# in5omnia/Image_Segmentation

Measured on AMD Instinct MI355X. Metric: images/sec (fwd+bwd) U-Net 3-class 256x256; IoU parity vs CPU ref, higher is better.
Workload: dtype bf16; 1 GPU; unet(3,3) train step (fwd + ce + bwd + grad all-reduce + AdamW), B=32/GPU 3x256x256, BASELINE config 2; global_batch=32, parallelism=dp1, rccl_ranks=0, rehearsal=False

## Files before the change

### image_segmentation_amd/_lib.py

```python
import ctypes as C
import os

_HERE = os.path.dirname(os.path.abspath(__file__))
LIB_PATH = os.path.join(_HERE, "csrc", "libsegk.so")

F32, BF16 = 0, 1
ABI_VERSION = 312
MAX_CLASSES = 8
MSE_PART_FLOATS = 1024

_vp, _fp, _i, _l, _f, _d = C.c_void_p, C.c_void_p, C.c_int, C.c_long, C.c_float, C.c_double

SIGNATURES = {
    "segk_version": (_i, []),
    "segk_entry_count": (_i, []),
    "segk_clock_probe": (_i, [_vp, _i, _i, _i, _vp]),
    "segk_debug_poison_tickets": (_i, [C.c_uint64, _vp]),
    "segk_build_id": (C.c_char_p, []),
    "segk_last_error": (C.c_char_p, []),
    "segk_nchw_to_nhwc": (_i, [_fp, _vp, _i, _i, _i, _i, _i, _i, _vp]),
    "segk_nhwc_to_nchw": (_i, [_vp, _fp, _i, _i, _i, _i, _i, _i, _vp]),
    "segk_pack_conv_weight": (_i, [_fp, _vp, _i, _i, _i, _i, _i, _i, _i, _i, _i, _vp]),
    "segk_pack_conv3x3_both": (_i, [_fp, _vp, _vp, _i, _i, _i, _i, _i, _i, _i, _vp]),
    "segk_pack_multi": (_i, [_vp, _i, _i, _i, _vp]),
    "segk_pack_convt_chunk": (_i, []),
    "segk_pack_convt_weight": (_i, [_fp, _vp, _i, _i, _i, _i, _i, _i, _vp]),
    "segk_conv_tiles": (_i, [_i, _i, _i, _i, _i, _i]),
    "segk_bn_stats_floats": (_i, [_i, _i]),
    "segk_conv3x3": (_i, [_vp, _vp, _vp, _fp, _fp, _fp, _vp, _vp, _fp, _i, _i, _i, _i, _i, _i, _i, _i, _vp]),
    "segk_conv_writes_act_q": (_i, [_i, _i, _i]),
    "segk_conv3x3_act": (_i, [_vp, _vp, _fp, _fp, _vp, _vp, _fp, _i, _i, _i, _i, _i, _i, _vp]),
    "segk_stem3x3_rows": (_i, [_i, _i, _i, _i, _i, _i]),
    "segk_stem3x3": (_i, [_fp, _fp, _vp, _vp, _fp, _i, _i, _i, _i, _i, _i, _vp]),
    "segk_stem3x3_wgrad_slabs": (_i, [_i, _i, _i, _i, _i, _i]),
    "segk_stem3x3_wgrad": (_i, [_fp, _vp, _fp, _i, _i, _i, _i, _i, _i, _vp]),
    "segk_conv1x1": (_i, [_vp, _vp, _fp, _vp, _i, _i, _i, _i, _i, _i, _vp]),
    "segk_convt2x2_fwd": (_i, [_vp, _vp, _fp, _vp, _i, _i, _i, _i, _i, _i, _vp]),
    "segk_convt2x2_dgrad": (_i, [_vp, _vp, _vp, _i, _i, _i, _i, _i, _i, _vp]),
    "segk_wgrad_tiles": (_i, [_i, _i, _i, _i, _i]),
    "segk_wgrad_split": (_i, [_i, _i, _i, _i, _i, _i]),
    "segk_wgrad": (_i, [_vp, _vp, _vp, _fp, _fp, _fp, _vp, _i, _i, _i, _i, _i, _i, _i, _i, _i, _vp]),
    "segk_wgrad_reduce": (_i, [_fp, _i, _fp, _i, _i, _i, _i, _i, _i, _i, _vp]),
    "segk_wgrad_reduce_multi": (_i, [_vp, _i, _vp]),
    "segk_bn_finalize": (_i, [_fp, _i, _i, _i, _d, _fp, _fp, _fp, _fp, _fp, _f, _f, _i, _fp, _fp, _fp, _fp, _vp]),
    "segk_bn_relu_apply": (_i, [_vp, _vp, _fp, _fp, _l, _i, _i, _vp]),
    "segk_bn_relu_apply_pool": (_i, [_vp, _vp, _vp, _fp, _fp, _i, _i, _i, _i, _i, _vp]),
    "segk_bn_bwd_blocks": (_i, [_l, _i, _i]),
    "segk_bn_relu_bwd": (_i, [_vp, _vp, _vp, _fp, _fp, _fp, _fp, _l, _i, _i, _fp, _fp, _fp, _fp, _i, _vp]),
    "segk_channel_sum": (_i, [_vp, _l, _i, _i, _fp, _fp, _i, _vp]),
    "segk_maxpool2x2_fwd": (_i, [_vp, _vp, _i, _i, _i, _i, _i, _vp]),
    "segk_maxpool2x2_bwd": (_i, [_vp, _vp, _vp, _i, _i, _i, _i, _i, _i, _vp]),
    "segk_maxpool_bwd_stat_blocks": (_i, [_i, _i, _i, _i, _i]),
    "segk_maxpool2x2_bwd_bnstat": (_i, [_vp, _vp, _vp, _i, _i, _i, _i, _i, _fp, _fp, _fp, _fp, _fp, _vp, _i, _vp]),
    "segk_bn_relu_bwd_from_part": (_i, [_vp, _vp, _vp, _fp, _fp, _fp, _fp, _l, _i, _i, _fp, _i, _fp, _fp, _fp, _i, _vp]),
    "segk_bilinear_fwd": (_i, [_vp, _vp, _i, _i, _i, _i, _i, _i, _i, _vp]),
    "segk_bilinear_bwd": (_i, [_vp, _vp, _fp, _i, _i, _i, _i, _i, _i, _i, _vp]),
    "segk_linear": (_i, [_vp, _vp, _fp, _vp, _l, _i, _i, _i, _i, _vp]),
    "segk_vit_patchify": (_i, [_fp, _vp, _i, _i, _i, _i, _i, _i, _i, _vp]),
    "segk_vit_embed_ln": (_i, [_vp, _fp, _fp, _fp, _fp, _f, _fp, _i, _i, _i, _i, _i, _vp]),
    "segk_add_layernorm": (_i, [_fp, _vp, _fp, _fp, _f, _vp, _l, _i, _i, _i, _vp]),
    "segk_linear_splitk": (_i, [_vp, _vp, _fp, _vp, _l, _i, _i, _i, _i, _vp]),
    "segk_add_layernorm_parts": (_i, [_fp, _vp, _i, _l, _fp, _fp, _f, _vp, _l, _i, _i, _i, _vp]),
    "segk_attention": (_i, [_vp, _vp, _i, _i, _i, _i, _i, _i, _f, _i, _vp]),
    "segk_vit_tokens_to_grid": (_i, [_fp, _vp, _i, _i, _i, _i, _i, _vp]),
    "segk_resize_pad": (_i, [_vp, _vp, _i, _i, _i, _i, _i, _i, _i, _i, _i, _i, _vp]),
    "segk_crop_resize": (_i, [_fp, _fp, _i, _i, _i, _i, _i, _i, _i, _i, _i, _vp]),
    "segk_resize_pad_u8": (_i, [_vp, _fp, _i, _i, _i, _i, _i, _i, _i, _i, _i, _vp]),
    "segk_predict_mask": (_i, [_vp, _vp, _vp, _vp, _vp, _vp, _vp, _i, _i, _i, _i, _i, _i, _i, _i, _i, _vp]),
    "segk_head_fwd": (_i, [_vp, _fp, _fp, _fp, _i, _i, _i, _i, _i, _i, _i, _vp]),
    "segk_head_fwd_bn": (_i, [_vp, _fp, _fp, _fp, _fp, _fp, _i, _i, _i, _i, _i, _i, _i, _vp]),
    "segk_head_bwd_bn": (_i, [_fp, _vp, _fp, _vp, _fp, _fp, _fp, _i, _i, _i, _i, _i, _i, _fp, _fp, _fp, _fp, _fp, _i, _vp]),
    "segk_head_part_floats": (_i, [_l, _i]),
    "segk_head_bwd": (_i, [_fp, _vp, _fp, _vp, _fp, _fp, _fp, _i, _i, _i, _i, _i, _i, _i, _vp]),
    "segk_head_bwd_blocks": (_i, [_l]),
    "segk_head_bwd_bnstat": (_i, [_fp, _vp, _fp, _vp, _fp, _fp, _fp, _i, _i, _i, _i, _i, _i, _fp, _fp, _fp, _fp, _fp, _i, _vp]),
    "segk_loss_part_floats": (_i, [_l]),
    "segk_loss_state_floats": (_i, []),
    "segk_loss_fwd": (_i, [_fp, _vp, _fp, _i, _i, _l, _i, _f, _f, _f, _fp, _fp, _fp, _vp]),
    "segk_loss_bwd": (_i, [_fp, _vp, _fp, _fp, _fp, _i, _i, _l, _i, _f, _f, _fp, _vp]),
    "segk_prompt_mix_fwd": (_i, [_fp, _fp, _fp, _i, _l, _vp]),
    "segk_prompt_mix_bwd": (_i, [_fp, _fp, _fp, _fp, _i, _l, _vp]),
    "segk_prob_loss_fwd": (_i, [_fp, _vp, _fp, _i, _i, _l, _i, _f, _f, _f, _i, _f, _fp, _fp, _fp, _vp]),
    "segk_prob_loss_bwd": (_i, [_fp, _vp, _fp, _fp, _fp, _i, _i, _l, _i, _f, _f, _i, _f, _fp, _vp]),
    "segk_confusion": (_i, [_fp, _vp, _i, _i, _l, _vp, _vp]),
    "segk_recon_head_fwd": (_i, [_vp, _fp, _fp, _fp, _i, _i, _i, _i, _i, _i, _i, _vp]),
    "segk_recon_sigmoid_bwd": (_i, [_fp, _fp, _vp, _i, _i, _i, _i, _i, _i, _vp]),
    "segk_mse_fwd": (_i, [_fp, _fp, _fp, _i, _fp, _l, _i, _vp]),
    "segk_mse_bwd": (_i, [_fp, _fp, _fp, _fp, _fp, _l, _i, _vp]),
}



class ReduceJob(C.Structure):
    _fields_ = [("src", C.c_void_p), ("dst", C.c_void_p), ("kind", C.c_int), ("S", C.c_int), ("N", C.c_int), ("CA", C.c_int),
                ("CB", C.c_int), ("Np", C.c_int), ("CAp", C.c_int), ("CBp", C.c_int), ("taps", C.c_int), ("pad_", C.c_int)]


_lib = None


def load():
    global _lib, LIB_PATH
    if _lib is None:
        if os.environ.get("SEGK_LIB"):
            LIB_PATH = os.path.abspath(os.environ["SEGK_LIB"])
        if not os.path.exists(LIB_PATH):
            raise RuntimeError(
                f"{LIB_PATH} not found: the HIP extension is required (no CPU/eager fallback exists). "
                "Build it with `python -m image_segmentation_amd.build`.")
        lib = C.CDLL(LIB_PATH)
        for name, (res, args) in SIGNATURES.items():
            try:
                fn = getattr(lib, name)
            except AttributeError:
                raise RuntimeError(f"{LIB_PATH} does not export {name}: it was built from another include/segk.h than "
                                   "this binding (rebuild with `python -m image_segmentation_amd.build`)") from None
            fn.restype = res
            fn.argtypes = args
        ver, nent = lib.segk_version(), lib.segk_entry_count()
        if ver != ABI_VERSION or nent != len(SIGNATURES):
            raise RuntimeError(f"{LIB_PATH}: ABI version {ver} with {nent} entries, this binding expects version "
                               f"{ABI_VERSION} with {len(SIGNATURES)} entries -- refusing to drive a library built from "
                               "another include/segk.h")
        _lib = lib
    return _lib


def call(name, *args):
    lib = load()
    rc = getattr(lib, name)(*args)
    if rc != 0:
        raise RuntimeError(f"{name} failed ({rc}): {lib.segk_last_error().decode()}")


def build_id():
    return load().segk_build_id().decode()


def query(name, *args):
    return getattr(load(), name)(*args)
```

### image_segmentation_amd/csrc/api.hip

```cpp
#include "common.hpp"
#include "segk_internal.h"
#include "../../include/segk.h"

thread_local char g_segk_err[512] = "";

int segk_bn_finalize_impl(const float*, int, int, int, double, const float*, const float*, const float*, float*, float*,
                          float, float, int, float*, float*, float*, float*, hipStream_t);
int segk_bn_relu_apply_impl(const void*, void*, const float*, const float*, long, int, int, hipStream_t);
int segk_bn_relu_apply_pool_impl(const void*, void*, void*, const float*, const float*, int, int, int, int, int, hipStream_t);
int segk_bn_bwd_impl(const void*, const void*, void*, const float*, const float*, const float*, const float*, long, int,
                     int, float*, float*, float*, float*, int, hipStream_t);
int segk_channel_sum_impl(const void*, long, int, int, float*, float*, int, hipStream_t);
int segk_maxpool_fwd_impl(const void*, void*, int, int, int, int, int, hipStream_t);
int segk_maxpool_bwd_impl(const void*, const void*, void*, int, int, int, int, int, int, hipStream_t);
int segk_maxpool_bwd_bnstat_impl(const void*, const void*, void*, int, int, int, int, int, const float*, const float*,
                                 const float*, const float*, float*, const void*, int, hipStream_t);
int segk_bn_bwd_from_part_impl(const void*, const void*, void*, const float*, const float*, const float*, const float*, long,
                               int, int, const float*, int, float*, float*, float*, int, hipStream_t);
int segk_nchw_to_nhwc_impl(const float*, void*, int, int, int, int, int, int, hipStream_t);
int segk_nhwc_to_nchw_impl(const void*, float*, int, int, int, int, int, int, hipStream_t);
int segk_pack_conv_weight_impl(const float*, void*, int, int, int, int, int, int, int, int, int, hipStream_t);
int segk_pack_convt_weight_impl(const float*, void*, int, int, int, int, int, int, hipStream_t);
int segk_pack_conv3x3_both_impl(const float*, void*, void*, int, int, int, int, int, int, int, hipStream_t);
int segk_pack_multi_impl(const void*, int, int, int, hipStream_t);
int segk_pack_convt_chunk_impl();
int segk_wgrad_reduce_impl(const float*, int, float*, int, int, int, int, int, int, int, hipStream_t);
int segk_wgrad_reduce_multi_impl(const segk_reduce_job*, int, hipStream_t);
int segk_head_fwd_impl(const void*, const float*, const float*, float*, int, int, int, int, int, int, const float*, const float*,
                       int, hipStream_t);
int segk_head_bwd_impl(const float*, const void*, const float*, void*, float*, float*, float*, int, int, int, int, int,
                       int, const float*, const float*, const float*, const float*, float*, int, int, hipStream_t);
int segk_head_blocks_q(long);
int segk_loss_fwd_impl(const float*, const long long*, const float*, int, int, long, int, float, float, float, float*,
                       float*, float*, int, int, float, hipStream_t);
int segk_loss_bwd_impl(const float*, const long long*, const float*, const float*, const float*, int, int, long, int,
                       float, float, float*, int, int, float, hipStream_t);
int segk_prompt_mix_impl(const float*, const float*, const float*, float*, int, long, hipStream_t);
int segk_confusion_impl(const float*, const long long*, int, int, long, unsigned long long*, hipStream_t);

int segk_recon_head_fwd_impl(const void*, const float*, const float*, float*, int, int, int, int, int, int, int, hipStream_t);
int segk_recon_sigmoid_bwd_impl(const float*, const float*, void*, int, int, int, int, int, int, hipStream_t);
int segk_mse_fwd_impl(const float*, const float*, float*, int, float*, long, int, hipStream_t);
int segk_mse_bwd_impl(const float*, const float*, const float*, float*, float*, long, int, hipStream_t);

int segk_clock_probe_impl(unsigned long long*, int, int, int, hipStream_t);
int segk_debug_poison_tickets_impl(unsigned long long, hipStream_t);

int segk_device_index() {
  int dev = 0;
  if (hipGetDevice(&dev) != hipSuccess || dev < 0) dev = 0;
  return dev < SEGK_MAX_DEVICES ? dev : SEGK_MAX_DEVICES - 1;
}
int segk_num_cus() {
  static int n[SEGK_MAX_DEVICES] = {};
  const int dev = segk_device_index();
  if (n[dev] == 0) {
    hipDeviceProp_t p;
    int v = 0;
    if (hipGetDeviceProperties(&p, dev) == hipSuccess) v = p.multiProcessorCount;
    n[dev] = v >= 8 ? v : 256;
  }
  return n[dev];
}

static void fill_tiles(ConvArgs&) {}

extern "C" {

#ifndef SEGK_BUILD_ID
#define SEGK_BUILD_ID "unknown"
#endif
int segk_version(void) { return SEGK_ABI_VERSION; }
int segk_entry_count(void) { return SEGK_ENTRY_COUNT; }
int segk_debug_poison_tickets(uint64_t pattern, segk_stream_t s) {
  return segk_debug_poison_tickets_impl((unsigned long long)pattern, (hipStream_t)s);
}
int segk_clock_probe(uint64_t* out, int blocks, int iters, int shape, segk_stream_t s) {
  return segk_clock_probe_impl((unsigned long long*)out, blocks, iters, shape, (hipStream_t)s);
}
const char* segk_build_id(void) { return SEGK_BUILD_ID; }
const char* segk_last_error(void) { return g_segk_err; }

int segk_nchw_to_nhwc(const float* src, void* dst, int B, int C, int H, int W, int Cp, int dtype, segk_stream_t s) {
  SEGK_REQUIRE(dtype == SEGK_DT_F32 || dtype == SEGK_DT_BF16, "nchw_to_nhwc: bad dtype %d", dtype);
  return segk_nchw_to_nhwc_impl(src, dst, B, C, H, W, Cp, dtype, (hipStream_t)s);
}
int segk_nhwc_to_nchw(const void* src, float* dst, int B, int C, int H, int W, int Cp, int dtype, segk_stream_t s) {
  SEGK_REQUIRE(dtype == SEGK_DT_F32 || dtype == SEGK_DT_BF16, "nhwc_to_nchw: bad dtype %d", dtype);
  return segk_nhwc_to_nchw_impl(src, dst, B, C, H, W, Cp, dtype, (hipStream_t)s);
}
int segk_pack_conv_weight(const float* w, void* dst, int Cout, int CA, int CB, int Coutp, int CAp, int CBp, int taps,
                          int mode, int dtype, segk_stream_t s) {
  SEGK_REQUIRE(dtype == SEGK_DT_F32 || dtype == SEGK_DT_BF16, "pack_conv_weight: bad dtype %d", dtype);
  return segk_pack_conv_weight_impl(w, dst, Cout, CA, CB, Coutp, CAp, CBp, taps, mode, dtype, (hipStream_t)s);
}
int segk_pack_conv3x3_both(const float* w, void* dst_fwd, void* dst_dgrad, int Cout, int CA, int CB, int Coutp, int CAp,
                            int CBp, int dtype, segk_stream_t s) {
  SEGK_REQUIRE(dtype == SEGK_DT_F32 || dtype == SEGK_DT_BF16, "pack_conv3x3_both: bad dtype %d", dtype);
  return segk_pack_conv3x3_both_impl(w, dst_fwd, dst_dgrad, Cout, CA, CB, Coutp, CAp, CBp, dtype, (hipStream_t)s);
}
int segk_pack_convt_chunk(void) { return segk_pack_convt_chunk_impl(); }
int segk_pack_multi(const void* table, int n, int total_blocks, int dtype, segk_stream_t s) {
  return segk_pack_multi_impl(table, n, total_blocks, dtype, (hipStream_t)s);
}
int segk_pack_convt_weight(const float* w, void* dst, int Cin, int Cout, int Cinp, int Coutp, int mode, int dtype,
                           segk_stream_t s) {
  SEGK_REQUIRE(dtype == SEGK_DT_F32 || dtype == SEGK_DT_BF16, "pack_convt_weight: bad dtype %d", dtype);
  return segk_pack_convt_weight_impl(w, dst, Cin, Cout, Cinp, Coutp, mode, dtype, (hipStream_t)s);
}

int segk_conv_tiles(int B, int H, int W, int Cin, int Cout, int dtype) {
  if (B <= 0 || H <= 0 || W <= 0 || Cin <= 0 || Cout <= 0 || (long long)B * H * W > 0x1fffffffLL) return 0;
  if (segk_conv_use_rs(Cin, Cout, dtype, W)) return segk_conv_rs_rows(B, H, W, Cout);
  const int pk = segk_conv_use_pipe(Cin, Cout, dtype);
  const int bm = segk_conv_use_ws(Cin, Cout, dtype) ? 256 : pk ? 32768 / pk : segk_conv_bm(0, Cout);
  const int twl = segk_conv_twl(bm, W);
  return B * cdiv(W, 1 << twl) * cdiv(H, bm >> twl);
}

int segk_conv3x3(const void* srcA, const void* srcB, const void* wpacked, const float* bias, const float* scale,
                 const float* shift, void* out, void* out2, float* stats, int B, int H, int W, int CA, int CB, int CO1,
                 int CO2, int dtype, segk_stream_t s) {
  SEGK_REQUIRE(dtype == SEGK_DT_F32 || dtype == SEGK_DT_BF16, "conv3x3: bad dtype %d", dtype);
  ConvArgs a{};
  a.srcA = srcA; a.srcB = srcB; a.w = wpacked; a.bias = bias; a.scale = scale; a.shift = shift;
  a.out = out; a.out2 = out2; a.stats = stats;
  a.B = B; a.H = H; a.W = W; a.CA = CA; a.CB = CB; a.Ntot = CO1 + CO2; a.CO1 = CO1; a.CO2 = CO2;
  fill_tiles(a);
  return segk_conv_igemm_launch(a, 0, dtype, (hipStream_t)s);
}

int segk_conv_writes_act_q(int Cin, int Cout, int dtype) { return segk_conv_writes_act(Cin, Cout, dtype); }

int segk_stem3x3_rows(int B, int H, int W, int Cin, int Cout, int dtype) { return segk_stem_rows(B, H, W, Cin, Cout, dtype); }
int segk_stem3x3_wgrad_slabs(int B, int H, int W, int Cin, int Cout, int dtype) {
  return segk_stem_wgrad_slabs(B, H, W, Cin, Cout, dtype);
}
int segk_stem3x3_wgrad(const float* x_nchw, const void* dz, float* slabs, int B, int H, int W, int Cin, int Cout, int dtype,
                       segk_stream_t s) {
  SEGK_REQUIRE(dtype == SEGK_DT_BF16, "stem3x3_wgrad: bf16 only (dtype %d)", dtype);
  return segk_stem_wgrad_launch(x_nchw, dz, slabs, B, H, W, Cin, Cout, (hipStream_t)s);
}
int segk_stem3x3(const float* x_nchw, const float* w_oihw, void* z, void* x_nhwc, float* stats, int B, int H, int W, int Cin,
                 int Cout, int dtype, segk_stream_t s) {
  SEGK_REQUIRE(dtype == SEGK_DT_BF16, "stem3x3: bf16 only (dtype %d)", dtype);
  return segk_stem_launch(x_nchw, w_oihw, z, x_nhwc, stats, B, H, W, Cin, Cout, (hipStream_t)s);
}

int segk_conv3x3_act(const void* srcA, const void* wpacked, const float* scale, const float* shift, void* out,
                     void* act_out, float* stats, int B, int H, int W, int CA, int CO, int dtype, segk_stream_t s) {
  SEGK_REQUIRE(dtype == SEGK_DT_F32 || dtype == SEGK_DT_BF16, "conv3x3_act: bad dtype %d", dtype);
  ConvArgs a{};
  a.srcA = srcA; a.w = wpacked; a.scale = scale; a.shift = shift; a.out = out; a.act_out = act_out; a.stats = stats;
  a.B = B; a.H = H; a.W = W; a.CA = CA; a.Ntot = CO; a.CO1 = CO;
  fill_tiles(a);
  return segk_conv_igemm_launch(a, 0, dtype, (hipStream_t)s);
}

int segk_conv1x1(const void* srcA, const void* wpacked, const float* bias, void* out, int B, int H, int W, int CA,
                 int CO, int dtype, segk_stream_t s) {
  SEGK_REQUIRE(dtype == SEGK_DT_F32 || dtype == SEGK_DT_BF16, "conv1x1: bad dtype %d", dtype);
  ConvArgs a{};
  a.srcA = srcA; a.w = wpacked; a.bias = bias; a.out = out;
  a.B = B; a.H = H; a.W = W; a.CA = CA; a.Ntot = CO; a.CO1 = CO;
  fill_tiles(a);
  return segk_conv_igemm_launch(a, 1, dtype, (hipStream_t)s);
}

int segk_linear(const void* rows, const void* wpacked, const float* bias, void* out, long M, int K, int N, int act,
                int dtype, segk_stream_t s) {
  SEGK_REQUIRE(dtype == SEGK_DT_F32 || dtype == SEGK_DT_BF16, "linear: bad dtype %d", dtype);
  SEGK_REQUIRE(M > 0 && M % 16 == 0 && M / 16 < (1 << 24), "linear: M=%ld must be a positive multiple of 16", M);
  SEGK_REQUIRE(act == 0 || act == 1, "linear: bad activation %d", act);
  ConvArgs a{};
  a.srcA = rows; a.w = wpacked; a.bias = bias; a.out = out;
  a.B = 1; a.H = (int)(M / 16); a.W = 16; a.CA = K; a.Ntot = N; a.CO1 = N; a.act = act;
  fill_tiles(a);
  return segk_conv_igemm_launch(a, 1, dtype, (hipStream_t)s);
}

int segk_linear_splitk(const void* rows, const void* wpacked, const float* bias, void* out_parts, long M, int K, int N,
                       int ksplit, int dtype, segk_stream_t s) {
  SEGK_REQUIRE(dtype == SEGK_DT_F32 || dtype == SEGK_DT_BF16, "linear_splitk: bad dtype %d", dtype);
  SEGK_REQUIRE(dtype == SEGK_DT_BF16, "linear_splitk: bf16 only");
  SEGK_REQUIRE(M > 0 && M % 16 == 0 && K > 0 && K % 64 == 0 && N > 0 && ksplit >= 1, "linear_splitk: bad shape");
  SEGK_REQUIRE(segk_gemm_dma_ok(M, K / 32, K / 32, N, N, K, 0) && (K / 64) % ksplit == 0 && K / 64 / ksplit >= 1,
               "linear_splitk: K=%d does not split %d ways into 64-element stages (or the shape is not served)", K, ksplit);
  GemmArgs g{};
  g.A = rows; g.w = (const char*)wpacked; g.bias = bias; g.out = out_parts;
  g.M = M; g.N = N; g.nchunks = K / 32; g.nchA = K / 32; g.lda = K; g.H = 1; g.W = 1; g.Cout = N;
  g.ksplit = ksplit; g.split_stride = M * (long)N;
  return segk_gemm_dma_launch(g, 0, (hipStream_t)s);
}

int segk_convt2x2_fwd(const void* in, const void* wpacked, const float* bias4, void* out, int B, int H, int W, int Cin,
                      int Cout, int dtype, segk_stream_t s) {
  SEGK_REQUIRE(dtype == SEGK_DT_F32 || dtype == SEGK_DT_BF16, "convt2x2_fwd: bad dtype %d", dtype);
  SEGK_REQUIRE(in && wpacked && out && B > 0 && H > 0 && W > 0 && Cin > 0 && Cout > 0, "convt2x2_fwd: bad arguments");
  if (segk_convt_stream_ok(B, H, W, Cin, Cout, dtype))
    return segk_convt_stream_launch(in, wpacked, bias4, out, B, H, W, Cin, Cout, (hipStream_t)s);
  ConvArgs a{};
  a.srcA = in; a.w = wpacked; a.bias = bias4; a.out = out;
  a.B = B; a.H = H; a.W = W; a.CA = Cin; a.Ntot = 4 * Cout; a.CO1 = Cout; a.shuffle = 1;
  fill_tiles(a);
  return segk_conv_igemm_launch(a, 1, dtype, (hipStream_t)s);
}

int segk_convt2x2_dgrad(const void* dout, const void* wpacked, void* din, int B, int H, int W, int Cin, int Cout,
                        int dtype, segk_stream_t s) {
  SEGK_REQUIRE(dtype == SEGK_DT_F32 || dtype == SEGK_DT_BF16, "convt2x2_dgrad: bad dtype %d", dtype);
  SEGK_REQUIRE(dout && wpacked && din && B > 0 && H > 0 && W > 0 && Cin > 0 && Cout > 0, "convt2x2_dgrad: bad arguments");
  if (segk_convt_stream_dgrad_ok(B, H, W, Cin, Cout, dtype))
    return segk_convt_stream_dgrad_launch(dout, wpacked, din, B, H, W, Cin, Cout, (hipStream_t)s);
  ConvArgs a{};
  a.srcA = dout; a.w = wpacked; a.out = din;
  a.B = B; a.H = H; a.W = W; a.CA = Cout; a.Ntot = Cin; a.CO1 = Cin; a.unshuf = 1;
  fill_tiles(a);
  return segk_conv_igemm_launch(a, 1, dtype, (hipStream_t)s);
}

int segk_wgrad(const void* dz, const void* srcA, const void* srcB, const float* scale, const float* shift, float* slabs,
               const void* zeros, int S, int B, int H, int W, int CD, int CA, int CB, int geo, int dtype,
               segk_stream_t s) {
  SEGK_REQUIRE(dtype == SEGK_DT_F32 || dtype == SEGK_DT_BF16, "wgrad: bad dtype %d", dtype);
  WgradArgs a{};
  a.dz = dz; a.srcA = srcA; a.srcB = srcB; a.scale = scale; a.shift = shift; a.slabs = slabs; a.zeros = zeros;
  a.B = B; a.H = H; a.W = W; a.CD = CD; a.CA = CA; a.CB = CB; a.S = S;
  return segk_wgrad_launch(a, geo, dtype, (hipStream_t)s);
}
int segk_wgrad_reduce(const float* slabs, int S, float* grad, int N, int CA, int CB, int Np, int CAp, int CBp, int taps,
                      segk_stream_t s) {
  return segk_wgrad_reduce_impl(slabs, S, grad, N, CA, CB, Np, CAp, CBp, taps, (hipStream_t)s);
}
int segk_wgrad_reduce_multi(const segk_reduce_job* jobs, int n, segk_stream_t s) {
  return segk_wgrad_reduce_multi_impl(jobs, n, (hipStream_t)s);
}

int segk_bn_finalize(const float* stats, int tiles, int Cp, int C, double count, const float* conv_bias,
                     const float* gamma, const float* beta, float* running_mean, float* running_var, float momentum,
                     float eps, int training, float* scale, float* shift, float* mean, float* rstd, segk_stream_t s) {
  return segk_bn_finalize_impl(stats, tiles, Cp, C, count, conv_bias, gamma, beta, running_mean, running_var, momentum,
                               eps, training, scale, shift, mean, rstd, (hipStream_t)s);
}
int segk_bn_relu_apply(const void* z, void* y, const float* scale, const float* shift, long P, int Cp, int dtype,
                       segk_stream_t s) {
  SEGK_REQUIRE(dtype == SEGK_DT_F32 || dtype == SEGK_DT_BF16, "bn_relu_apply: bad dtype %d", dtype);
  return segk_bn_relu_apply_impl(z, y, scale, shift, P, Cp, dtype, (hipStream_t)s);
}
int segk_bn_relu_apply_pool(const void* z, void* y, void* pooled, const float* scale, const float* shift, int B, int H, int W,
                            int Cp, int dtype, segk_stream_t s) {
  SEGK_REQUIRE(dtype == SEGK_DT_F32 || dtype == SEGK_DT_BF16, "bn_relu_apply_pool: bad dtype %d", dtype);
  return segk_bn_relu_apply_pool_impl(z, y, pooled, scale, shift, B, H, W, Cp, dtype, (hipStream_t)s);
}
int segk_bn_relu_bwd(const void* dy, const void* z, void* dz, const float* scale, const float* shift, const float* mean,
                     const float* rstd, long P, int Cp, int C, float* part, float* dgamma, float* dbeta, float* coef,
                     int dtype, segk_stream_t s) {
  SEGK_REQUIRE(dtype == SEGK_DT_F32 || dtype == SEGK_DT_BF16, "bn_relu_bwd: bad dtype %d", dtype);
  return segk_bn_bwd_impl(dy, z, dz, scale, shift, mean, rstd, P, Cp, C, part, dgamma, dbeta, coef, dtype,
                          (hipStream_t)s);
}
int segk_channel_sum(const void* x, long P, int Cp, int C, float* part, float* out, int dtype, segk_stream_t s) {
  SEGK_REQUIRE(dtype == SEGK_DT_F32 || dtype == SEGK_DT_BF16, "channel_sum: bad dtype %d", dtype);
  return segk_channel_sum_impl(x, P, Cp, C, part, out, dtype, (hipStream_t)s);
}
int segk_maxpool2x2_fwd(const void* x, void* y, int B, int H, int W, int Cp, int dtype, segk_stream_t s) {
  SEGK_REQUIRE(dtype == SEGK_DT_F32 || dtype == SEGK_DT_BF16, "maxpool2x2_fwd: bad dtype %d", dtype);
  return segk_maxpool_fwd_impl(x, y, B, H, W, Cp, dtype, (hipStream_t)s);
}
int segk_maxpool2x2_bwd(const void* x, const void* dy, void* dx, int B, int H, int W, int Cp, int accumulate, int dtype,
                        segk_stream_t s) {
  SEGK_REQUIRE(dtype == SEGK_DT_F32 || dtype == SEGK_DT_BF16, "maxpool2x2_bwd: bad dtype %d", dtype);
  return segk_maxpool_bwd_impl(x, dy, dx, B, H, W, Cp, accumulate, dtype, (hipStream_t)s);
}
int segk_maxpool2x2_bwd_bnstat(const void* x, const void* dy, void* dx, int B, int H, int W, int Cp, int accumulate,
                               const float* scale, const float* shift, const float* mean, const float* rstd, float* part,
                               const void* z, int dtype, segk_stream_t s) {
  SEGK_REQUIRE(dtype == SEGK_DT_F32 || dtype == SEGK_DT_BF16, "maxpool2x2_bwd_bnstat: bad dtype %d", dtype);
  return segk_maxpool_bwd_bnstat_impl(x, dy, dx, B, H, W, Cp, accumulate, scale, shift, mean, rstd, part, z, dtype,
                                      (hipStream_t)s);
}
int segk_bn_relu_bwd_from_part(const void* dy, const void* z, void* dz, const float* scale, const float* shift,
                               const float* mean, const float* rstd, long P, int Cp, int C, const float* part, int nb,
                               float* dgamma, float* dbeta, float* coef, int dtype, segk_stream_t s) {
  SEGK_REQUIRE(dtype == SEGK_DT_F32 || dtype == SEGK_DT_BF16, "bn_relu_bwd_from_part: bad dtype %d", dtype);
  return segk_bn_bwd_from_part_impl(dy, z, dz, scale, shift, mean, rstd, P, Cp, C, part, nb, dgamma, dbeta, coef, dtype,
                                    (hipStream_t)s);
}
int segk_head_fwd(const void* y, const float* w, const float* bias, float* logits, int B, int H, int W, int Cp, int C,
                  int ncls, int dtype, segk_stream_t s) {
  SEGK_REQUIRE(dtype == SEGK_DT_F32 || dtype == SEGK_DT_BF16, "head_fwd: bad dtype %d", dtype);
  return segk_head_fwd_impl(y, w, bias, logits, B, H, W, Cp, C, ncls, nullptr, nullptr, dtype, (hipStream_t)s);
}
int segk_head_fwd_bn(const void* z, const float* scale, const float* shift, const float* w, const float* bias, float* logits,
                     int B, int H, int W, int Cp, int C, int ncls, int dtype, segk_stream_t s) {
  SEGK_REQUIRE(scale && shift, "head_fwd_bn: null scale/shift");
  return segk_head_fwd_impl(z, w, bias, logits, B, H, W, Cp, C, ncls, scale, shift, dtype, (hipStream_t)s);
}
int segk_head_bwd(const float* dlogits, const void* y, const float* w, void* dy, float* part, float* dw, float* db,
                  int B, int H, int W, int Cp, int C, int ncls, int dtype, segk_stream_t s) {
  SEGK_REQUIRE(dtype == SEGK_DT_F32 || dtype == SEGK_DT_BF16, "head_bwd: bad dtype %d", dtype);
  return segk_head_bwd_impl(dlogits, y, w, dy, part, dw, db, B, H, W, Cp, C, ncls, nullptr, nullptr, nullptr, nullptr, nullptr,
                            0, dtype, (hipStream_t)s);
}
int segk_head_bwd_blocks(long P) { return segk_head_blocks_q(P); }
int segk_head_bwd_bnstat(const float* dlogits, const void* y, const float* w, void* dy, float* part, float* dw, float* db,
                         int B, int H, int W, int Cp, int C, int ncls, const float* scale, const float* shift,
                         const float* mean, const float* rstd, float* bnpart, int dtype, segk_stream_t s) {
  SEGK_REQUIRE(dtype == SEGK_DT_F32 || dtype == SEGK_DT_BF16, "head_bwd_bnstat: bad dtype %d", dtype);
  SEGK_REQUIRE(bnpart, "head_bwd_bnstat: null partials");
  return segk_head_bwd_impl(dlogits, y, w, dy, part, dw, db, B, H, W, Cp, C, ncls, scale, shift, mean, rstd, bnpart, 0, dtype,
                            (hipStream_t)s);
}
int segk_head_bwd_bn(const float* dlogits, const void* z, const float* w, void* dy, float* part, float* dw, float* db,
                     int B, int H, int W, int Cp, int C, int ncls, const float* scale, const float* shift,
                     const float* mean, const float* rstd, float* bnpart, int dtype, segk_stream_t s) {
  SEGK_REQUIRE(scale && shift && mean && rstd, "head_bwd_bn: null BatchNorm vectors");
  return segk_head_bwd_impl(dlogits, z, w, dy, part, dw, db, B, H, W, Cp, C, ncls, scale, shift, mean, rstd, bnpart, 1, dtype,
                            (hipStream_t)s);
}
int segk_loss_fwd(const float* logits, const int64_t* labels, const float* cw, int N, int C, long HW, int ignore_index,
                  float smooth, float dice_weight, float ce_weight, float* part, float* state, float* loss_out,
                  segk_stream_t s) {
  return segk_loss_fwd_impl(logits, (const long long*)labels, cw, N, C, HW, ignore_index, smooth, dice_weight, ce_weight,
                            part, state, loss_out, 0, 0, 0.f, (hipStream_t)s);
}
int segk_prob_loss_fwd(const float* probs, const int64_t* labels, const float* cw, int N, int C, long HW, int ignore_index,
                       float smooth, float dice_weight, float nll_weight, int nll_log, float eps, float* part, float* state,
                       float* loss_out, segk_stream_t s) {
  return segk_loss_fwd_impl(probs, (const long long*)labels, cw, N, C, HW, ignore_index, smooth, dice_weight, nll_weight,
                            part, state, loss_out, 1, nll_log, eps, (hipStream_t)s);
}
int segk_prob_loss_bwd(const float* probs, const int64_t* labels, const float* cw, const float* state, const float* gout,
                       int N, int C, long HW, int ignore_index, float dice_weight, float nll_weight, int nll_log, float eps,
                       float* dprobs, segk_stream_t s) {
  return segk_loss_bwd_impl(probs, (const long long*)labels, cw, state, gout, N, C, HW, ignore_index, dice_weight,
                            nll_weight, dprobs, 1, nll_log, eps, (hipStream_t)s);
}
int segk_prompt_mix_fwd(const float* clip_logits, const float* mask_logit, float* final_probs, int N, long HW,
                        segk_stream_t s) {
  return segk_prompt_mix_impl(clip_logits, mask_logit, nullptr, final_probs, N, HW, (hipStream_t)s);
}
int segk_prompt_mix_bwd(const float* clip_logits, const float* mask_logit, const float* dfinal, float* dmask_logit, int N,
                        long HW, segk_stream_t s) {
  SEGK_REQUIRE(dfinal, "prompt_mix_bwd: null gradient");
  return segk_prompt_mix_impl(clip_logits, mask_logit, dfinal, dmask_logit, N, HW, (hipStream_t)s);
}
int segk_loss_bwd(const float* logits, const int64_t* labels, const float* cw, const float* state, const float* gout,
                  int N, int C, long HW, int ignore_index, float dice_weight, float ce_weight, float* dlogits,
                  segk_stream_t s) {
  return segk_loss_bwd_impl(logits, (const long long*)labels, cw, state, gout, N, C, HW, ignore_index, dice_weight,
                            ce_weight, dlogits, 0, 0, 0.f, (hipStream_t)s);
}
int segk_recon_head_fwd(const void* x, const float* w, const float* bias, float* rec, int B, int H, int W, int Cp, int Cin,
                        int Cout, int dtype, segk_stream_t s) {
  return segk_recon_head_fwd_impl(x, w, bias, rec, B, H, W, Cp, Cin, Cout, dtype, (hipStream_t)s);
}
int segk_recon_sigmoid_bwd(const float* drec, const float* rec, void* dz, int B, int H, int W, int C, int Cp, int dtype,
                           segk_stream_t s) {
  return segk_recon_sigmoid_bwd_impl(drec, rec, dz, B, H, W, C, Cp, dtype, (hipStream_t)s);
}
int segk_mse_fwd(const float* a, const float* b, float* part, int part_floats, float* out, long n, int mean, segk_stream_t s) {
  return segk_mse_fwd_impl(a, b, part, part_floats, out, n, mean, (hipStream_t)s);
}
int segk_mse_bwd(const float* a, const float* b, const float* grad_out, float* da, float* db, long n, int mean,
                 segk_stream_t s) {
  return segk_mse_bwd_impl(a, b, grad_out, da, db, n, mean, (hipStream_t)s);
}
int segk_confusion(const float* logits, const int64_t* labels, int N, int C, long HW, uint64_t* M, segk_stream_t s) {
  return segk_confusion_impl(logits, (const long long*)labels, N, C, HW, (unsigned long long*)M, (hipStream_t)s);
}

}
```

### image_segmentation_amd/csrc/bn_pool.hip

```cpp
#include <atomic>
#include "common.hpp"
#include "segk_internal.h"
#include "ticket.hpp"
#include "../../include/segk.h"

namespace {
__device__ unsigned g_tickets[TICKET_SLOTS * TICKET_GROUPS];

struct Lanes {
  int cx, ry, cv;
  bool active;
};
__device__ __forceinline__ Lanes lanes(int cvb, int cvec) {
  Lanes l;
  l.cx = threadIdx.x % cvb;
  l.ry = threadIdx.x / cvb;
  l.cv = blockIdx.y * cvb + l.cx;
  l.active = l.cv < cvec;
  return l;
}

constexpr int NCH = 32;
__device__ __forceinline__ void stats_chunk(const float* __restrict__ part, int MT, int C, double* __restrict__ out,
                                            double (&sh)[8][32][2]) {
  const int cx = threadIdx.x & 31, ry = threadIdx.x >> 5;
  const int c = blockIdx.x * 32 + cx;
  const int chunk = (MT + NCH - 1) / NCH;
  const int m0 = blockIdx.y * chunk, m1 = min(MT, m0 + chunk);
  double s1 = 0.0, s2 = 0.0;
  for (int m = m0 + ry; m < m1; m += 8) {
    const float2 v = ((const float2*)part)[(size_t)m * C + c];
    s1 += (double)v.x;
    s2 += (double)v.y;
  }
  sh[ry][cx][0] = s1;
  sh[ry][cx][1] = s2;
  __syncthreads();
  if (ry == 0) {
    s1 = 0.0; s2 = 0.0;
    for (int r = 0; r < 8; ++r) { s1 += sh[r][cx][0]; s2 += sh[r][cx][1]; }
    out[((size_t)blockIdx.y * C + c) * 2 + 0] = s1;
    out[((size_t)blockIdx.y * C + c) * 2 + 1] = s2;
  }
}

__device__ __forceinline__ void finalize_channels(const double* __restrict__ part, int MT, int C, int C_real,
                                                  double count, const float* conv_bias,
                                                  const float* gamma, const float* beta, float* rmean,
                                                  float* rvar, float momentum, float eps, int training,
                                                  float* scale, float* shift, float* mean_out,
                                                  float* rstd_out, double (&sh)[8][32][2]) {
  const int cx = threadIdx.x & 31, ry = threadIdx.x >> 5;
  const int c = blockIdx.x * 32 + cx;
  double s1 = 0.0, s2 = 0.0;
  if (training && c < C)
    for (int m = ry; m < MT; m += 8) {
      s1 += part[((size_t)m * C + c) * 2 + 0];
      s2 += part[((size_t)m * C + c) * 2 + 1];
    }
  sh[ry][cx][0] = s1;
  sh[ry][cx][1] = s2;
  __syncthreads();
  if (ry != 0 || c >= C) return;
  if (c >= C_real) {
    scale[c] = 0.f; shift[c] = 0.f;
    if (mean_out) { mean_out[c] = 0.f; rstd_out[c] = 0.f; }
    return;
  }
  const float g = gamma[c], be = beta[c];
  const float cb = conv_bias ? conv_bias[c] : 0.f;
  if (training) {
    s1 = 0.0; s2 = 0.0;
    for (int r = 0; r < 8; ++r) { s1 += sh[r][cx][0]; s2 += sh[r][cx][1]; }
    const double mean = s1 / count;
    double var = s2 / count - mean * mean;
    if (var < 0.0) var = 0.0;
    const float rstd = (float)(1.0 / sqrt(var + (double)eps));
    const float sc = g * rstd;
    scale[c] = sc;
    shift[c] = be - (float)mean * sc;
    mean_out[c] = (float)mean;
    rstd_out[c] = rstd;
    if (rmean) {
      const double unb = count > 1.0 ? var * count / (count - 1.0) : var;
      rmean[c] = (1.f - momentum) * rmean[c] + momentum * ((float)mean + cb);
      rvar[c] = (1.f - momentum) * rvar[c] + momentum * (float)unb;
    }
  } else {
    const float rstd = 1.f / sqrtf(rvar[c] + eps);
    const float sc = g * rstd;
    scale[c] = sc;
    shift[c] = be + (cb - rmean[c]) * sc;
    if (mean_out) { mean_out[c] = rmean[c] - cb; rstd_out[c] = rstd; }
  }
}

__global__ __launch_bounds__(256) void bn_finalize_kernel(const double* __restrict__ part, int MT, int C, int C_real,
                                                          double count, const float* conv_bias,
                                                          const float* gamma, const float* beta, float* rmean,
                                                          float* rvar, float momentum, float eps, int training,
                                                          float* scale, float* shift, float* mean_out,
                                                          float* rstd_out) {
  __shared__ double sh[8][32][2];
  finalize_channels(part, MT, C, C_real, count, conv_bias, gamma, beta, rmean, rvar, momentum, eps, training, scale, shift,
                    mean_out, rstd_out, sh);
}

__global__ __launch_bounds__(1024) void bn_stats_finalize_small_kernel(const float* __restrict__ part, int MT, int C,
                                                                       int C_real, double count, const float* conv_bias,
                                                                       const float* gamma, const float* beta, float* rmean,
                                                                       float* rvar, float momentum, float eps, float* scale,
                                                                       float* shift, float* mean_out, float* rstd_out) {
  __shared__ double sh[32][32][2];
  const int cx = threadIdx.x & 31, ry = threadIdx.x >> 5;
  const int c = blockIdx.x * 32 + cx;
  double s1 = 0.0, s2 = 0.0;
#pragma unroll 1
  for (int m = ry; m < MT; m += 512) {
    float2 v[16];
#pragma unroll
    for (int u = 0; u < 16; ++u) {
      const int r = m + 32 * u < MT ? m + 32 * u : MT - 1;
      v[u] = ((const float2*)part)[(unsigned)r * (unsigned)C + (unsigned)c];
    }
#pragma unroll
    for (int u = 0; u < 16; ++u) {
      const bool ok = m + 32 * u < MT;
      s1 += ok ? (double)v[u].x : 0.0;
      s2 += ok ? (double)v[u].y : 0.0;
    }
  }
  sh[ry][cx][0] = s1;
  sh[ry][cx][1] = s2;
  __syncthreads();
  if (ry != 0) return;
  s1 = 0.0; s2 = 0.0;
#pragma unroll 8
  for (int r = 0; r < 32; ++r) { s1 += sh[r][cx][0]; s2 += sh[r][cx][1]; }
  if (c >= C_real) {
    scale[c] = 0.f; shift[c] = 0.f; mean_out[c] = 0.f; rstd_out[c] = 0.f;
    return;
  }
  const float g = gamma[c], be = beta[c];
  const float cb = conv_bias ? conv_bias[c] : 0.f;
  const double mean = s1 / count;
  double var = s2 / count - mean * mean;
  if (var < 0.0) var = 0.0;
  const float rstd = (float)(1.0 / sqrt(var + (double)eps));
  const float sc = g * rstd;
  scale[c] = sc;
  shift[c] = be - (float)mean * sc;
  mean_out[c] = (float)mean;
  rstd_out[c] = rstd;
  if (rmean) {
    const double unb = count > 1.0 ? var * count / (count - 1.0) : var;
    rmean[c] = (1.f - momentum) * rmean[c] + momentum * ((float)mean + cb);
    rvar[c] = (1.f - momentum) * rvar[c] + momentum * (float)unb;
  }
}

__global__ __launch_bounds__(256) void bn_stats_finalize_kernel(const float* __restrict__ part, int MT, int C, int C_real,
                                                                double count, const float* conv_bias,
                                                                const float* gamma, const float* beta, float* rmean,
                                                                float* rvar, float momentum, float eps,
                                                                float* scale, float* shift, float* mean_out,
                                                                float* rstd_out, double* __restrict__ scratch,
                                                                unsigned* __restrict__ tickets) {
  __shared__ double sh[8][32][2];
  __shared__ int last;
  stats_chunk(part, MT, C, scratch, sh);
  if (!last_arriver(tickets + blockIdx.x, gridDim.y, &last)) return;
  finalize_channels(scratch, (int)gridDim.y, C, C_real, count, conv_bias, gamma, beta, rmean, rvar, momentum, eps, 1, scale,
                    shift, mean_out, rstd_out, sh);
}

template <typename T>
__global__ __launch_bounds__(256) void bn_relu_apply_kernel(const T* __restrict__ z, T* __restrict__ y,
                                                            const float* scale, const float* shift, long P, int C,
                                                            int cvb, int rows) {
  using E = ET<T>;
  const Lanes l = lanes(cvb, C / E::VEC);
  if (!l.active || l.ry >= rows) return;
  float sc[E::VEC], sh[E::VEC];
#pragma unroll
  for (int j = 0; j < E::VEC; ++j) { sc[j] = scale[l.cv * E::VEC + j]; sh[j] = shift[l.cv * E::VEC + j]; }
  auto one = [&](const uint4 raw, const size_t off) {
    float f[E::VEC];
    unpack16<T>(raw, f);
#pragma unroll
    for (int j = 0; j < E::VEC; ++j) f[j] = fmaxf(fmaf(f[j], sc[j], sh[j]), 0.f);
    *(uint4*)(y + off) = pack16<T>(f);
  };
  for (long p = (long)blockIdx.x * rows + l.ry; p < P; p += (long)gridDim.x * rows) {
    const size_t off = (size_t)p * C + (size_t)l.cv * E::VEC;
    one(*(const uint4*)(z + off), off);
  }
}

template <typename T>
__global__ __launch_bounds__(256) void bn_bwd_reduce_kernel(const T* __restrict__ dy, const T* __restrict__ z,
                                                            const float* scale, const float* shift,
                                                            const float* mean, const float* rstd, long P, int C,
                                                            int cvb, int rows, float* part) {
  using E = ET<T>;
  extern __shared__ __attribute__((aligned(16))) char smem[];
  float* red = (float*)smem;
  const Lanes l = lanes(cvb, C / E::VEC);
  float sg[E::VEC], sgx[E::VEC];
#pragma unroll
  for (int j = 0; j < E::VEC; ++j) { sg[j] = 0.f; sgx[j] = 0.f; }
  if (l.active && l.ry < rows) {
    float sc[E::VEC], sh[E::VEC], mu[E::VEC], rs[E::VEC];
#pragma unroll
    for (int j = 0; j < E::VEC; ++j) {
      const int c = l.cv * E::VEC + j;
      sc[j] = scale[c]; sh[j] = shift[c]; mu[j] = mean[c]; rs[j] = rstd[c];
    }
    auto one = [&](const uint4 rz, const uint4 rd) {
      float fz[E::VEC], fd[E::VEC];
      unpack16<T>(rz, fz);
      unpack16<T>(rd, fd);
#pragma unroll
      for (int j = 0; j < E::VEC; ++j) {
        const float g = (fmaf(fz[j], sc[j], sh[j]) > 0.f) ? fd[j] : 0.f;
        sg[j] += g;
        sgx[j] = fmaf(g, (fz[j] - mu[j]) * rs[j], sgx[j]);
      }
    };
    const long step = (long)gridDim.x * rows;
    const size_t cofs = (size_t)l.cv * E::VEC;
    long p = (long)blockIdx.x * rows + l.ry;
    for (; p + 3 * step < P; p += 4 * step) {
      uint4 rz[4], rd[4];
#pragma unroll
      for (int u = 0; u < 4; ++u) {
        const size_t off = (size_t)(p + u * step) * C + cofs;
        rz[u] = *(const uint4*)(z + off);
        rd[u] = *(const uint4*)(dy + off);
      }
      __builtin_amdgcn_sched_barrier(0);
#pragma unroll
      for (int u = 0; u < 4; ++u) one(rz[u], rd[u]);
    }
    for (; p < P; p += step) {
      const size_t off = (size_t)p * C + cofs;
      one(*(const uint4*)(z + off), *(const uint4*)(dy + off));
    }
  }
  if (l.ry < rows) {
    float* r = red + ((size_t)l.ry * cvb + l.cx) * (2 * E::VEC);
#pragma unroll
    for (int j = 0; j < E::VEC; ++j) { r[j] = sg[j]; r[E::VEC + j] = sgx[j]; }
  }
  __syncthreads();
  if (l.ry == 0 && l.active) {
#pragma unroll
    for (int j = 0; j < E::VEC; ++j) {
      float a = 0.f, b = 0.f;
      for (int r = 0; r < rows; ++r) {
        const float* q = red + ((size_t)r * cvb + l.cx) * (2 * E::VEC);
        a += q[j];
        b += q[E::VEC + j];
      }
      float2* dst = (float2*)part + (size_t)blockIdx.x * C + l.cv * E::VEC + j;
      *dst = make_float2(a, b);
    }
  }
}

__global__ __launch_bounds__(1024) void bn_bwd_finalize_kernel(const float* __restrict__ part, int NB, int C,
                                                               int C_real, double count, float* dgamma, float* dbeta,
                                                               float* coef) {
  __shared__ double sh[32][32][2];
  const int cx = threadIdx.x & 31, ry = threadIdx.x >> 5;
  const int c = blockIdx.x * 32 + cx;
  double s1 = 0.0, s2 = 0.0;
  if (c < C) {
    for (int m = ry; m < NB; m += 512) {
      float2 v[16];
#pragma unroll
      for (int u = 0; u < 16; ++u) {
        const int r = m + 32 * u < NB ? m + 32 * u : NB - 1;
        v[u] = ((const float2*)part)[(unsigned)r * (unsigned)C + (unsigned)c];
      }
#pragma unroll
      for (int u = 0; u < 16; ++u) {
        const bool ok = m + 32 * u < NB;
        s1 += ok ? (double)v[u].x : 0.0;
        s2 += ok ? (double)v[u].y : 0.0;
      }
    }
  }
  sh[ry][cx][0] = s1;
  sh[ry][cx][1] = s2;
  __syncthreads();
  if (ry != 0 || c >= C) return;
  s1 = 0.0; s2 = 0.0;
  for (int r = 0; r < 32; ++r) { s1 += sh[r][cx][0]; s2 += sh[r][cx][1]; }
  if (c < C_real) { dbeta[c] = (float)s1; dgamma[c] = (float)s2; }
  coef[2 * c] = (float)(s1 / count);
  coef[2 * c + 1] = (float)(s2 / count);
}

template <typename T>
__global__ __launch_bounds__(256) void bn_bwd_apply_kernel(const T* __restrict__ dy, const T* __restrict__ z,
                                                           T* __restrict__ dz, const float* scale,
                                                           const float* shift, const float* mean, const float* rstd,
                                                           const float* coef, long P, int C, int cvb, int rows) {
  using E = ET<T>;
  const Lanes l = lanes(cvb, C / E::VEC);
  if (!l.active || l.ry >= rows) return;
  float sc[E::VEC], sh[E::VEC], mu[E::VEC], rs[E::VEC], c1[E::VEC], c2[E::VEC];
#pragma unroll
  for (int j = 0; j < E::VEC; ++j) {
    const int c = l.cv * E::VEC + j;
    sc[j] = scale[c]; sh[j] = shift[c]; mu[j] = mean[c]; rs[j] = rstd[c];
    c1[j] = coef[2 * c]; c2[j] = coef[2 * c + 1];
  }
  auto one = [&](const uint4 rz, const uint4 rd, const size_t off) {
    float fz[E::VEC], fd[E::VEC];
    unpack16<T>(rz, fz);
    unpack16<T>(rd, fd);
#pragma unroll
    for (int j = 0; j < E::VEC; ++j) {
      const float g = (fmaf(fz[j], sc[j], sh[j]) > 0.f) ? fd[j] : 0.f;
      const float xh = (fz[j] - mu[j]) * rs[j];
      fd[j] = sc[j] * (g - c1[j] - xh * c2[j]);
    }
    *(uint4*)(dz + off) = pack16<T>(fd);
  };
#ifndef SEGK_BN_APPLY_FLIGHT
#define SEGK_BN_APPLY_FLIGHT 1
#endif
  constexpr int APF = SEGK_BN_APPLY_FLIGHT;
  const long step = (long)gridDim.x * rows;
  const size_t cofs = (size_t)l.cv * E::VEC;
  long p = (long)blockIdx.x * rows + l.ry;
  for (; p + (APF - 1) * step < P; p += APF * step) {
    size_t o[APF];
    uint4 rz[APF], rd[APF];
#pragma unroll
    for (int u = 0; u < APF; ++u) {
      o[u] = (size_t)(p + u * step) * C + cofs;
      rz[u] = *(const uint4*)(z + o[u]);
      rd[u] = *(const uint4*)(dy + o[u]);
    }
#pragma unroll
    for (int u = 0; u < APF; ++u) one(rz[u], rd[u], o[u]);
  }
  for (; p < P; p += step) {
    const size_t o0 = (size_t)p * C + cofs;
    one(*(const uint4*)(z + o0), *(const uint4*)(dy + o0), o0);
  }
}

template <typename T>
__global__ __launch_bounds__(256) void bn_relu_apply_pool_kernel(const T* __restrict__ z, T* __restrict__ y,
                                                                 T* __restrict__ pooled, const float* __restrict__ scale,
                                                                 const float* __restrict__ shift, int B, int H, int W, int C) {
  using E = ET<T>;
  const int Ho = H >> 1, Wo = W >> 1, CV = C / E::VEC;
  const int Hc = (H + 1) >> 1, Wc = (W + 1) >> 1;
  const long total = (long)B * Hc * Wc * CV;
  for (unsigned i = blockIdx.x * 256u + threadIdx.x; i < (unsigned)total; i += gridDim.x * 256u) {
    const Idx4 ix = split4(i, (unsigned)CV, (unsigned)Wc, (unsigned)Hc);
    const int cv = ix.cv, xo = ix.x, yo = ix.y, b = ix.b;
    float sc[E::VEC], sh[E::VEC], mx[E::VEC];
#pragma unroll
    for (int j = 0; j < E::VEC; ++j) { sc[j] = scale[cv * E::VEC + j]; sh[j] = shift[cv * E::VEC + j]; mx[j] = 0.f; }
    size_t offs[4];
    uint4 raw[4];
#pragma unroll
    for (int k = 0; k < 4; ++k) {
      const int yy = 2 * yo + (k >> 1), xx = 2 * xo + (k & 1);
      offs[k] = (((size_t)(b * H + (yy < H ? yy : H - 1))) * W + (xx < W ? xx : W - 1)) * C + cv * E::VEC;
      raw[k] = *(const uint4*)(z + offs[k]);
    }
#pragma unroll
    for (int k = 0; k < 4; ++k) {
      const int yy = 2 * yo + (k >> 1), xx = 2 * xo + (k & 1);
      if (yy >= H || xx >= W) continue;
      const size_t off = offs[k];
      float f[E::VEC];
      unpack16<T>(raw[k], f);
#pragma unroll
      for (int j = 0; j < E::VEC; ++j) f[j] = fmaxf(fmaf(f[j], sc[j], sh[j]), 0.f);
      const uint4 pk = pack16<T>(f);
      *(uint4*)(y + off) = pk;
      unpack16<T>(pk, f);
#pragma unroll
      for (int j = 0; j < E::VEC; ++j) mx[j] = fmaxf(mx[j], f[j]);
    }
    if (yo < Ho && xo < Wo) *(uint4*)(pooled + (((size_t)(b * Ho + yo)) * Wo + xo) * C + cv * E::VEC) = pack16<T>(mx);
  }
}

template <typename T>
__global__ __launch_bounds__(256) void maxpool_fwd_kernel(const T* __restrict__ x, T* __restrict__ y, int B, int H,
                                                          int W, int C) {
  using E = ET<T>;
  const int Ho = H >> 1, Wo = W >> 1, CV = C / E::VEC;
  const long total = (long)B * Ho * Wo * CV;
  for (unsigned i = blockIdx.x * 256u + threadIdx.x; i < (unsigned)total; i += gridDim.x * 256u) {
    const Idx4 ix = split4(i, (unsigned)CV, (unsigned)Wo, (unsigned)Ho);
    const int cv = ix.cv, xo = ix.x, yo = ix.y, b = ix.b;
    const T* src = x + (((size_t)(b * H + 2 * yo)) * W + 2 * xo) * C + cv * E::VEC;
    float f0[E::VEC], f1[E::VEC], f2[E::VEC], f3[E::VEC];
    unpack16<T>(*(const uint4*)src, f0);
    unpack16<T>(*(const uint4*)(src + C), f1);
    unpack16<T>(*(const uint4*)(src + (size_t)W * C), f2);
    unpack16<T>(*(const uint4*)(src + (size_t)W * C + C), f3);
#pragma unroll
    for (int j = 0; j < E::VEC; ++j) f0[j] = fmaxf(fmaxf(f0[j], f1[j]), fmaxf(f2[j], f3[j]));
    *(uint4*)(y + (((size_t)(b * Ho + yo)) * Wo + xo) * C + cv * E::VEC) = pack16<T>(f0);
  }
}

template <typename T, bool STAT>
__global__ __launch_bounds__(256) void maxpool_bwd_kernel(const T* __restrict__ x, const T* __restrict__ dy,
                                                          T* __restrict__ dx, int B, int H, int W, int C,
                                                          int accumulate, const float* __restrict__ scale,
                                                          const float* __restrict__ shift, const float* __restrict__ mean,
                                                          const float* __restrict__ rstd, float* __restrict__ part,
                                                          const T* __restrict__ z) {
  using E = ET<T>;
  const int Ho = H >> 1, Wo = W >> 1, CV = C / E::VEC;
  const int Hc = (H + 1) >> 1, Wc = (W + 1) >> 1;
  const long total = (long)B * Hc * Wc * CV;
  float xa[E::VEC], xb[E::VEC], sg[E::VEC], sgx[E::VEC];
  bool from_z = false;
  if (STAT) {
    const int cv0 = threadIdx.x % CV;
#pragma unroll
    for (int j = 0; j < E::VEC; ++j) {
      const int c = cv0 * E::VEC + j;
      const float sc = scale[c], rs = rstd[c], sh = shift[c];
      from_z = from_z || (z != nullptr && (sc == 0.f || fabsf(sc) * 16.f < fabsf(sh)));
      xa[j] = sc != 0.f ? rs / sc : 0.f;
      xb[j] = -sh * xa[j] - mean[c] * rs;
      sg[j] = 0.f; sgx[j] = 0.f;
    }
  }
  for (unsigned i = blockIdx.x * 256u + threadIdx.x; i < (unsigned)total; i += gridDim.x * 256u) {
    const Idx4 ix = split4(i, (unsigned)CV, (unsigned)Wc, (unsigned)Hc);
    const int cv = ix.cv, xo = ix.x, yo = ix.y, b = ix.b;
    const bool inwin = (yo < Ho) && (xo < Wo);
    const int yoc = yo < Ho ? yo : Ho - 1, xoc = xo < Wo ? xo : Wo - 1;
    const uint4 rg = *(const uint4*)(dy + (((size_t)(b * Ho + yoc)) * Wo + xoc) * C + cv * E::VEC);
    uint4 rv[4], ro[4];
    size_t off[4];
#pragma unroll
    for (int k = 0; k < 4; ++k) {
      const int yy = 2 * yo + (k >> 1), xx = 2 * xo + (k & 1);
      off[k] = (((size_t)(b * H + (yy < H ? yy : H - 1))) * W + (xx < W ? xx : W - 1)) * C + cv * E::VEC;
      rv[k] = *(const uint4*)(x + off[k]);
    }
    if (accumulate) {
#pragma unroll
      for (int k = 0; k < 4; ++k) ro[k] = *(const uint4*)(dx + off[k]);
    }
    float g[E::VEC];
    float v[4][E::VEC];
    unpack16<T>(rg, g);
#pragma unroll
    for (int k = 0; k < 4; ++k) unpack16<T>(rv[k], v[k]);
    int sel[E::VEC];
#pragma unroll
    for (int j = 0; j < E::VEC; ++j) {
      sel[j] = 0;
      float m = v[0][j];
#pragma unroll
      for (int k = 1; k < 4; ++k)
        if (v[k][j] > m) { m = v[k][j]; sel[j] = k; }
    }
#pragma unroll
    for (int k = 0; k < 4; ++k) {
      const int yy = 2 * yo + (k >> 1), xx = 2 * xo + (k & 1);
      if (yy >= H || xx >= W) continue;
      float o[E::VEC];
      if (accumulate) unpack16<T>(ro[k], o);
#pragma unroll
      for (int j = 0; j < E::VEC; ++j) {
        const float r = (inwin && sel[j] == k) ? g[j] : 0.f;
        o[j] = accumulate ? o[j] + r : r;
        if (STAT) {
          const float gg = v[k][j] > 0.f ? o[j] : 0.f;
          sg[j] += gg;
          sgx[j] = fmaf(gg, fmaf(v[k][j], xa[j], xb[j]), sgx[j]);
        }
      }
      *(uint4*)(dx + off[k]) = pack16<T>(o);
    }
  }
  if (STAT) {
    __shared__ float red[256][2 * E::VEC + 1];
    if (from_z) {
#pragma unroll
      for (int j = 0; j < E::VEC; ++j) sgx[j] = 0.f;
      for (unsigned i = blockIdx.x * 256u + threadIdx.x; i < (unsigned)total; i += gridDim.x * 256u) {
        const Idx4 ix = split4(i, (unsigned)CV, (unsigned)Wc, (unsigned)Hc);
        const int cv = ix.cv, xo = ix.x, yo = ix.y, b = ix.b;
        for (int k = 0; k < 4; ++k) {
          const int yy = 2 * yo + (k >> 1), xx = 2 * xo + (k & 1);
          if (yy >= H || xx >= W) continue;
          const size_t off = (((size_t)(b * H + yy)) * W + xx) * C + cv * E::VEC;
          float fy[E::VEC], fd[E::VEC], fz[E::VEC];
          unpack16<T>(*(const uint4*)(x + off), fy);
          unpack16<T>(*(const uint4*)(dx + off), fd);
          unpack16<T>(*(const uint4*)(z + off), fz);
#pragma unroll
          for (int j = 0; j < E::VEC; ++j) {
            const int c = cv * E::VEC + j;
            const float gg = fy[j] > 0.f ? fd[j] : 0.f;
            sgx[j] = fmaf(gg, (fz[j] - mean[c]) * rstd[c], sgx[j]);
          }
        }
      }
    }
#pragma unroll
    for (int j = 0; j < E::VEC; ++j) { red[threadIdx.x][j] = sg[j]; red[threadIdx.x][E::VEC + j] = sgx[j]; }
    __syncthreads();
    for (int q = threadIdx.x; q < CV * E::VEC; q += 256) {
      const int cv = q / E::VEC, j = q - cv * E::VEC;
      float a = 0.f, bsum = 0.f;
      for (int t = cv; t < 256; t += CV) {
        a += red[t][j];
        bsum += red[t][E::VEC + j];
      }
      ((float2*)part)[(size_t)blockIdx.x * C + q] = make_float2(a, bsum);
    }
  }
}

template <typename T>
__global__ __launch_bounds__(256) void channel_sum_kernel(const T* __restrict__ x, long P, int C, int cvb, int rows,
                                                          float* part) {
  using E = ET<T>;
  extern __shared__ __attribute__((aligned(16))) char smem[];
  float* red = (float*)smem;
  const Lanes l = lanes(cvb, C / E::VEC);
  float s[E::VEC];
#pragma unroll
  for (int j = 0; j < E::VEC; ++j) s[j] = 0.f;
  if (l.active && l.ry < rows) {
    auto one = [&](const uint4 raw) {
      float f[E::VEC];
      unpack16<T>(raw, f);
#pragma unroll
      for (int j = 0; j < E::VEC; ++j) s[j] += f[j];
    };
    const long step = (long)gridDim.x * rows;
    const size_t cofs = (size_t)l.cv * E::VEC;
    long p = (long)blockIdx.x * rows + l.ry;
    for (; p + 3 * step < P; p += 4 * step) {
      uint4 r[4];
#pragma unroll
      for (int u = 0; u < 4; ++u) r[u] = *(const uint4*)(x + (size_t)(p + u * step) * C + cofs);
      __builtin_amdgcn_sched_barrier(0);
#pragma unroll
      for (int u = 0; u < 4; ++u) one(r[u]);
    }
    for (; p < P; p += step) one(*(const uint4*)(x + (size_t)p * C + cofs));
  }
  if (l.ry < rows) {
    float* r = red + ((size_t)l.ry * cvb + l.cx) * E::VEC;
#pragma unroll
    for (int j = 0; j < E::VEC; ++j) r[j] = s[j];
  }
  __syncthreads();
  if (l.ry == 0 && l.active)
#pragma unroll
    for (int j = 0; j < E::VEC; ++j) {
      float a = 0.f;
      for (int r = 0; r < rows; ++r) a += red[((size_t)r * cvb + l.cx) * E::VEC + j];
      part[(size_t)blockIdx.x * C + l.cv * E::VEC + j] = a;
    }
}
__global__ __launch_bounds__(1024) void channel_sum_finalize_kernel(const float* __restrict__ part, int NB, int C,
                                                                    int C_real, float* out) {
  __shared__ double sh[32][32];
  const int cx = threadIdx.x & 31, ry = threadIdx.x >> 5;
  const int c = blockIdx.x * 32 + cx;
  double s = 0.0;
  if (c < C) {
    for (int m = ry; m < NB; m += 512) {
      float v[16];
#pragma unroll
      for (int u = 0; u < 16; ++u) {
        const int r = m + 32 * u < NB ? m + 32 * u : NB - 1;
        v[u] = part[(unsigned)r * (unsigned)C + (unsigned)c];
      }
#pragma unroll
      for (int u = 0; u < 16; ++u) s += (m + 32 * u < NB) ? (double)v[u] : 0.0;
    }
  }
  sh[ry][cx] = s;
  __syncthreads();
  if (ry != 0 || c >= C_real) return;
  s = 0.0;
#pragma unroll 8
  for (int r = 0; r < 32; ++r) s += sh[r][cx];
  out[c] = (float)s;
}

static inline void lane_geometry(int C, int vec, int* cvb, int* rows, int* gy) {
  const int cvec = C / vec;
  *cvb = cvec < 128 ? cvec : 128;
  *rows = 256 / *cvb;
  *gy = cdiv(cvec, *cvb);
}

}

unsigned* segk_ticket_slot(int groups, hipStream_t st) {
  static std::atomic<unsigned> n{0};
  static unsigned* base[SEGK_MAX_DEVICES] = {};
  const int dev = segk_device_index();
  if (groups < 1 || groups > TICKET_GROUPS) return nullptr;
  if (!base[dev] && hipGetSymbolAddress((void**)&base[dev], HIP_SYMBOL(g_tickets)) != hipSuccess) return nullptr;
  unsigned* const p = base[dev] + (size_t)(n.fetch_add(1, std::memory_order_relaxed) % TICKET_SLOTS) * TICKET_GROUPS;
  if (hipMemsetAsync(p, 0, (size_t)groups * sizeof(unsigned), st) != hipSuccess) return nullptr;
  return p;
}

int segk_debug_poison_tickets_impl(unsigned long long pattern, hipStream_t st) {
  unsigned* base = nullptr;
  SEGK_REQUIRE(hipGetSymbolAddress((void**)&base, HIP_SYMBOL(g_tickets)) == hipSuccess, "poison_tickets: no ticket array");
  static unsigned host[TICKET_SLOTS * TICKET_GROUPS];
  for (int i = 0; i < TICKET_SLOTS * TICKET_GROUPS; ++i) host[i] = (unsigned)pattern;
  SEGK_REQUIRE(hipMemcpyAsync(base, host, sizeof(host), hipMemcpyHostToDevice, st) == hipSuccess, "poison_tickets: copy failed");
  SEGK_REQUIRE(hipStreamSynchronize(st) == hipSuccess, "poison_tickets: sync failed");
  return 0;
}

int segk_bn_finalize_impl(const float* part, int MT, int C, int C_real, double count, const float* conv_bias,
                          const float* gamma, const float* beta, float* rmean, float* rvar, float momentum, float eps,
                          int training, float* scale, float* shift, float* mean, float* rstd, hipStream_t st) {
  SEGK_REQUIRE(C > 0 && C % 32 == 0 && C_real > 0 && C_real <= C, "bn_finalize: bad channels C=%d real=%d", C, C_real);
  SEGK_REQUIRE(gamma && beta && scale && shift, "bn_finalize: null pointer");
  if (training) SEGK_REQUIRE(part && MT > 0 && count > 0 && mean && rstd, "bn_finalize: training needs partials");
  else SEGK_REQUIRE(rmean && rvar, "bn_finalize: eval needs running statistics");
  double* scratch = part ? (double*)(const_cast<float*>(part) + (size_t)MT * C * 2) : nullptr;
  if (training && MT <= 1024) {
    hipLaunchKernelGGL(bn_stats_finalize_small_kernel, dim3(C / 32), dim3(1024), 0, st, part, MT, C, C_real, count, conv_bias,
                       gamma, beta, rmean, rvar, momentum, eps, scale, shift, mean, rstd);
    SEGK_CHECK_LAUNCH("bn_stats_finalize_small");
    return 0;
  }
  if (training) {
    SEGK_REQUIRE(C / 32 <= TICKET_GROUPS, "bn_finalize: at most %d channels", 32 * TICKET_GROUPS);
    unsigned* const tickets = segk_ticket_slot(C / 32, st);
    SEGK_REQUIRE(tickets != nullptr, "bn_finalize: no ticket array");
    hipLaunchKernelGGL(bn_stats_finalize_kernel, dim3(C / 32, NCH), dim3(256), 0, st, part, MT, C, C_real, count, conv_bias,
                       gamma, beta, rmean, rvar, momentum, eps, scale, shift, mean, rstd, scratch, tickets);
    SEGK_CHECK_LAUNCH("bn_stats_finalize");
    return 0;
  }
  hipLaunchKernelGGL(bn_finalize_kernel, dim3(C / 32), dim3(256), 0, st, scratch, NCH, C, C_real, count, conv_bias,
                     gamma, beta, rmean, rvar, momentum, eps, training, scale, shift, mean, rstd);
  SEGK_CHECK_LAUNCH("bn_finalize");
  return 0;
}
int segk_bn_stats_floats(int tiles, int Cp) {
  if (tiles <= 0 || Cp <= 0) return 0;
  const long long n = (long long)tiles * Cp * 2 + (long long)NCH * Cp * 4;
  return n > 0x7fffffffLL ? 0 : (int)n;
}

template <typename T>
static int bn_relu_apply_t(const void* z, void* y, const float* scale, const float* shift, long P, int C, hipStream_t st) {
  int cvb, rows, gy;
  lane_geometry(C, ET<T>::VEC, &cvb, &rows, &gy);
  long gx = (P + rows - 1) / rows;
  if (gx > 4096) gx = 4096;
  hipLaunchKernelGGL(bn_relu_apply_kernel<T>, dim3((int)gx, gy), dim3(256), 0, st, (const T*)z, (T*)y, scale, shift, P,
                     C, cvb, rows);
  SEGK_CHECK_LAUNCH("bn_relu_apply");
  return 0;
}
int segk_bn_relu_apply_impl(const void* z, void* y, const float* scale, const float* shift, long P, int C, int dtype,
                            hipStream_t st) {
  SEGK_REQUIRE(z && y && scale && shift && P > 0 && C > 0 && C % 32 == 0, "bn_relu_apply: bad arguments");
  return dtype == SEGK_DT_BF16 ? bn_relu_apply_t<bf16_t>(z, y, scale, shift, P, C, st)
                               : bn_relu_apply_t<float>(z, y, scale, shift, P, C, st);
}

int segk_bn_relu_apply_pool_impl(const void* z, void* y, void* pooled, const float* scale, const float* shift, int B, int H,
                                  int W, int C, int dtype, hipStream_t st) {
  SEGK_REQUIRE(z && y && pooled && scale && shift && B > 0 && H >= 2 && W >= 2 && C > 0 && C % 32 == 0,
               "bn_relu_apply_pool: bad arguments");
  const int vec = dtype == SEGK_DT_BF16 ? 8 : 4;
  long total = (long)B * ((H + 1) / 2) * ((W + 1) / 2) * (C / vec);
  SEGK_REQUIRE(total < (1L << 31), "bn_relu_apply_pool: more than 2^31 windows x channel vectors");
  long g = (total + 255) / 256;
  if (g > 8192) g = 8192;
  if (dtype == SEGK_DT_BF16)
    hipLaunchKernelGGL(bn_relu_apply_pool_kernel<bf16_t>, dim3((int)g), dim3(256), 0, st, (const bf16_t*)z, (bf16_t*)y,
                       (bf16_t*)pooled, scale, shift, B, H, W, C);
  else
    hipLaunchKernelGGL(bn_relu_apply_pool_kernel<float>, dim3((int)g), dim3(256), 0, st, (const float*)z, (float*)y,
                       (float*)pooled, scale, shift, B, H, W, C);
  SEGK_CHECK_LAUNCH("bn_relu_apply_pool");
  return 0;
}

int segk_bn_bwd_blocks(long P, int C, int dtype) {
  if (P <= 0 || C <= 0 || C % 32 != 0) return 0;
  const int vec = dtype == SEGK_DT_BF16 ? 8 : 4;
  int cvb, rows, gy;
  lane_geometry(C, vec, &cvb, &rows, &gy);
  long gx = (P + rows - 1) / rows;
  if (gx > 512) gx = 512;
  return (int)gx;
}

template <typename T>
static int bn_bwd_t(const void* dy, const void* z, void* dz, const float* scale, const float* shift, const float* mean,
                    const float* rstd, long P, int C, int C_real, float* part, float* dgamma, float* dbeta,
                    float* coef, hipStream_t st) {
  using E = ET<T>;
  int cvb, rows, gy;
  lane_geometry(C, E::VEC, &cvb, &rows, &gy);
  const int gx = segk_bn_bwd_blocks(P, C, sizeof(T) == 2 ? SEGK_DT_BF16 : SEGK_DT_F32);
  const size_t lds = (size_t)rows * cvb * 2 * E::VEC * sizeof(float);
  hipLaunchKernelGGL(bn_bwd_reduce_kernel<T>, dim3(gx, gy), dim3(256), lds, st, (const T*)dy, (const T*)z, scale, shift,
                     mean, rstd, P, C, cvb, rows, part);
  SEGK_CHECK_LAUNCH("bn_bwd_reduce");
  hipLaunchKernelGGL(bn_bwd_finalize_kernel, dim3(C / 32), dim3(1024), 0, st, part, gx, C, C_real, (double)P, dgamma,
                     dbeta, coef);
  SEGK_CHECK_LAUNCH("bn_bwd_finalize");
  long ga = (P + rows - 1) / rows;
  if (ga > 4096) ga = 4096;
  hipLaunchKernelGGL(bn_bwd_apply_kernel<T>, dim3((int)ga, gy), dim3(256), 0, st, (const T*)dy, (const T*)z, (T*)dz,
                     scale, shift, mean, rstd, coef, P, C, cvb, rows);
  SEGK_CHECK_LAUNCH("bn_bwd_apply");
  return 0;
}
template <typename T>
static int bn_bwd_from_part_t(const void* dy, const void* z, void* dz, const float* scale, const float* shift, const float* mean,
                              const float* rstd, long P, int C, int C_real, const float* part, int nb, float* dgamma,
                              float* dbeta, float* coef, hipStream_t st) {
  using E = ET<T>;
  int cvb, rows, gy;
  lane_geometry(C, E::VEC, &cvb, &rows, &gy);
  hipLaunchKernelGGL(bn_bwd_finalize_kernel, dim3(C / 32), dim3(1024), 0, st, part, nb, C, C_real, (double)P, dgamma,
                     dbeta, coef);
  SEGK_CHECK_LAUNCH("bn_bwd_finalize");
  long ga = (P + rows - 1) / rows;
  if (ga > 4096) ga = 4096;
  hipLaunchKernelGGL(bn_bwd_apply_kernel<T>, dim3((int)ga, gy), dim3(256), 0, st, (const T*)dy, (const T*)z, (T*)dz,
                     scale, shift, mean, rstd, coef, P, C, cvb, rows);
  SEGK_CHECK_LAUNCH("bn_bwd_apply");
  return 0;
}
int segk_bn_bwd_from_part_impl(const void* dy, const void* z, void* dz, const float* scale, const float* shift,
                               const float* mean, const float* rstd, long P, int C, int C_real, const float* part, int nb,
                               float* dgamma, float* dbeta, float* coef, int dtype, hipStream_t st) {
  SEGK_REQUIRE(dy && z && dz && scale && shift && mean && rstd && part && dgamma && dbeta && coef && nb > 0,
               "bn_bwd_from_part: bad arguments");
  SEGK_REQUIRE(P > 0 && C > 0 && C % 32 == 0 && C_real > 0 && C_real <= C, "bn_bwd_from_part: bad shape");
  return dtype == SEGK_DT_BF16
             ? bn_bwd_from_part_t<bf16_t>(dy, z, dz, scale, shift, mean, rstd, P, C, C_real, part, nb, dgamma, dbeta, coef, st)
             : bn_bwd_from_part_t<float>(dy, z, dz, scale, shift, mean, rstd, P, C, C_real, part, nb, dgamma, dbeta, coef, st);
}

int segk_bn_bwd_impl(const void* dy, const void* z, void* dz, const float* scale, const float* shift, const float* mean,
                     const float* rstd, long P, int C, int C_real, float* part, float* dgamma, float* dbeta, float* coef,
                     int dtype, hipStream_t st) {
  SEGK_REQUIRE(dy && z && dz && scale && shift && mean && rstd && part && dgamma && dbeta && coef,
               "bn_bwd: null pointer");
  SEGK_REQUIRE(P > 0 && C > 0 && C % 32 == 0 && C_real > 0 && C_real <= C, "bn_bwd: bad shape");
  return dtype == SEGK_DT_BF16
             ? bn_bwd_t<bf16_t>(dy, z, dz, scale, shift, mean, rstd, P, C, C_real, part, dgamma, dbeta, coef, st)
             : bn_bwd_t<float>(dy, z, dz, scale, shift, mean, rstd, P, C, C_real, part, dgamma, dbeta, coef, st);
}

int segk_maxpool_fwd_impl(const void* x, void* y, int B, int H, int W, int C, int dtype, hipStream_t st) {
  SEGK_REQUIRE(x && y && B > 0 && H >= 2 && W >= 2 && C > 0 && C % 32 == 0, "maxpool_fwd: bad arguments");
  const int vec = dtype == SEGK_DT_BF16 ? 8 : 4;
  long total = (long)B * (H / 2) * (W / 2) * (C / vec);
  SEGK_REQUIRE(total < (1L << 31), "maxpool_fwd: more than 2^31 windows x channel vectors");
  long g = (total + 255) / 256;
  if (g > 8192) g = 8192;
  if (dtype == SEGK_DT_BF16)
    hipLaunchKernelGGL(maxpool_fwd_kernel<bf16_t>, dim3((int)g), dim3(256), 0, st, (const bf16_t*)x, (bf16_t*)y, B, H, W, C);
  else
    hipLaunchKernelGGL(maxpool_fwd_kernel<float>, dim3((int)g), dim3(256), 0, st, (const float*)x, (float*)y, B, H, W, C);
  SEGK_CHECK_LAUNCH("maxpool_fwd");
  return 0;
}

int segk_maxpool_bwd_impl(const void* x, const void* dy, void* dx, int B, int H, int W, int C, int accumulate, int dtype,
                          hipStream_t st) {
  SEGK_REQUIRE(x && dy && dx && B > 0 && H >= 2 && W >= 2 && C > 0 && C % 32 == 0, "maxpool_bwd: bad arguments");
  const int vec = dtype == SEGK_DT_BF16 ? 8 : 4;
  long total = (long)B * ((H + 1) / 2) * ((W + 1) / 2) * (C / vec);
  SEGK_REQUIRE(total < (1L << 31), "maxpool_bwd: more than 2^31 windows x channel vectors");
  long g = (total + 255) / 256;
  if (g > 8192) g = 8192;
  if (dtype == SEGK_DT_BF16)
    hipLaunchKernelGGL((maxpool_bwd_kernel<bf16_t, false>), dim3((int)g), dim3(256), 0, st, (const bf16_t*)x, (const bf16_t*)dy,
                       (bf16_t*)dx, B, H, W, C, accumulate, nullptr, nullptr, nullptr, nullptr, nullptr, nullptr);
  else
    hipLaunchKernelGGL((maxpool_bwd_kernel<float, false>), dim3((int)g), dim3(256), 0, st, (const float*)x, (const float*)dy,
                       (float*)dx, B, H, W, C, accumulate, nullptr, nullptr, nullptr, nullptr, nullptr, nullptr);
  SEGK_CHECK_LAUNCH("maxpool_bwd");
  return 0;
}

int segk_maxpool_bwd_stat_blocks(int B, int H, int W, int C, int dtype) {
  const int vec = dtype == SEGK_DT_BF16 ? 8 : 4;
  if (B <= 0 || H < 2 || W < 2 || C <= 0 || C % 32 != 0) return 0;
  const int cv = C / vec;
  if ((cv & (cv - 1)) != 0 || cv > 256) return 0;
  long total = (long)B * ((H + 1) / 2) * ((W + 1) / 2) * cv;
  if (total >= (1L << 31)) return 0;
  long g = (total + 255) / 256;
  return (int)(g > 1024 ? 1024 : g);
}

int segk_maxpool_bwd_bnstat_impl(const void* x, const void* dy, void* dx, int B, int H, int W, int C, int accumulate,
                                 const float* scale, const float* shift, const float* mean, const float* rstd, float* part,
                                 const void* z, int dtype, hipStream_t st) {
  SEGK_REQUIRE(x && dy && dx && scale && shift && mean && rstd && part, "maxpool_bwd_bnstat: null pointer");
  const int g = segk_maxpool_bwd_stat_blocks(B, H, W, C, dtype);
  SEGK_REQUIRE(g > 0, "maxpool_bwd_bnstat: shape not served (channel vectors must be a power of two)");
  if (dtype == SEGK_DT_BF16)
    hipLaunchKernelGGL((maxpool_bwd_kernel<bf16_t, true>), dim3(g), dim3(256), 0, st, (const bf16_t*)x, (const bf16_t*)dy,
                       (bf16_t*)dx, B, H, W, C, accumulate, scale, shift, mean, rstd, part, (const bf16_t*)z);
  else
    hipLaunchKernelGGL((maxpool_bwd_kernel<float, true>), dim3(g), dim3(256), 0, st, (const float*)x, (const float*)dy,
                       (float*)dx, B, H, W, C, accumulate, scale, shift, mean, rstd, part, (const float*)z);
  SEGK_CHECK_LAUNCH("maxpool_bwd_bnstat");
  return 0;
}

int segk_channel_sum_impl(const void* x, long P, int C, int C_real, float* part, float* out, int dtype, hipStream_t st) {
  SEGK_REQUIRE(x && part && out && P > 0 && C > 0 && C % 32 == 0 && C_real > 0 && C_real <= C, "channel_sum: bad arguments");
  const int vec = dtype == SEGK_DT_BF16 ? 8 : 4;
  int cvb, rows, gy;
  lane_geometry(C, vec, &cvb, &rows, &gy);
  const int gx = segk_bn_bwd_blocks(P, C, dtype);
  const size_t lds = (size_t)rows * cvb * vec * sizeof(float);
  if (dtype == SEGK_DT_BF16)
    hipLaunchKernelGGL(channel_sum_kernel<bf16_t>, dim3(gx, gy), dim3(256), lds, st, (const bf16_t*)x, P, C, cvb, rows, part);
  else
    hipLaunchKernelGGL(channel_sum_kernel<float>, dim3(gx, gy), dim3(256), lds, st, (const float*)x, P, C, cvb, rows, part);
  SEGK_CHECK_LAUNCH("channel_sum");
  hipLaunchKernelGGL(channel_sum_finalize_kernel, dim3(C / 32), dim3(1024), 0, st, part, gx, C, C_real, out);
  SEGK_CHECK_LAUNCH("channel_sum_finalize");
  return 0;
}
```

### image_segmentation_amd/csrc/common.hpp

```cpp
#pragma once
#include <hip/hip_runtime.h>
#include <stdint.h>
#include <stdio.h>
#include <string.h>

typedef __bf16 bf16_t;
typedef __attribute__((ext_vector_type(8))) __bf16 bf16x8;
typedef __attribute__((ext_vector_type(4))) __bf16 bf16x4;
typedef __attribute__((ext_vector_type(4))) short s16x4;
typedef __attribute__((ext_vector_type(4))) float f32x4;
typedef __attribute__((ext_vector_type(16))) float f32x16;

#define SEGK_DT_F32 0
#define SEGK_DT_BF16 1

extern thread_local char g_segk_err[512];
#define SEGK_FAIL(code, ...)                                   \
  do {                                                         \
    snprintf(g_segk_err, sizeof(g_segk_err), __VA_ARGS__);     \
    return (code);                                             \
  } while (0)
#define SEGK_REQUIRE(cond, ...)                                \
  do {                                                         \
    if (!(cond)) SEGK_FAIL(-2, __VA_ARGS__);                   \
  } while (0)
#define SEGK_CHECK_LAUNCH(name)                                                        \
  do {                                                                                 \
    hipError_t e_ = hipGetLastError();                                                 \
    if (e_ != hipSuccess) SEGK_FAIL(-3, "%s: launch failed: %s", name, hipGetErrorString(e_)); \
  } while (0)

template <typename T> struct ET;
template <> struct ET<float> {
  static constexpr int VEC = 4;
  static constexpr int ES = 4;
  static constexpr int CH = 16;
};
template <> struct ET<bf16_t> {
  static constexpr int VEC = 8;
  static constexpr int ES = 2;
  static constexpr int CH = 32;
};

__device__ __forceinline__ float bf2f(uint32_t lo16) { return __uint_as_float(lo16 << 16); }

template <typename T> __device__ __forceinline__ void unpack16(const uint4& v, float* f);
template <> __device__ __forceinline__ void unpack16<float>(const uint4& v, float* f) {
  f[0] = __uint_as_float(v.x); f[1] = __uint_as_float(v.y);
  f[2] = __uint_as_float(v.z); f[3] = __uint_as_float(v.w);
}
template <> __device__ __forceinline__ void unpack16<bf16_t>(const uint4& v, float* f) {
  f[0] = bf2f(v.x & 0xffffu); f[1] = __uint_as_float(v.x & 0xffff0000u);
  f[2] = bf2f(v.y & 0xffffu); f[3] = __uint_as_float(v.y & 0xffff0000u);
  f[4] = bf2f(v.z & 0xffffu); f[5] = __uint_as_float(v.z & 0xffff0000u);
  f[6] = bf2f(v.w & 0xffffu); f[7] = __uint_as_float(v.w & 0xffff0000u);
}
typedef float f32x2v __attribute__((ext_vector_type(2)));
typedef __bf16 bf16x2v __attribute__((ext_vector_type(2)));
__device__ __forceinline__ uint32_t cvt_pk_bf16(float lo, float hi) {
  return __builtin_bit_cast(uint32_t, __builtin_convertvector((f32x2v){lo, hi}, bf16x2v));
}
__device__ __forceinline__ uint32_t pack_bf16x2(float lo, float hi) { return cvt_pk_bf16(lo, hi); }
template <typename T> __device__ __forceinline__ uint4 pack16(const float* f);
template <> __device__ __forceinline__ uint4 pack16<float>(const float* f) {
  return make_uint4(__float_as_uint(f[0]), __float_as_uint(f[1]), __float_as_uint(f[2]), __float_as_uint(f[3]));
}
template <> __device__ __forceinline__ uint4 pack16<bf16_t>(const float* f) {
  return make_uint4(pack_bf16x2(f[0], f[1]), pack_bf16x2(f[2], f[3]), pack_bf16x2(f[4], f[5]),
                    pack_bf16x2(f[6], f[7]));
}
template <typename T> __device__ __forceinline__ T from_float(float f);
template <> __device__ __forceinline__ float from_float<float>(float f) { return f; }
template <> __device__ __forceinline__ bf16_t from_float<bf16_t>(float f) { return (bf16_t)f; }
template <typename T> __device__ __forceinline__ float to_float(T v);
template <> __device__ __forceinline__ float to_float<float>(float v) { return v; }
template <> __device__ __forceinline__ float to_float<bf16_t>(bf16_t v) { return (float)v; }

typedef float f32x2_t __attribute__((ext_vector_type(2)));
template <typename T>
__device__ __forceinline__ void stage_frag(const float (&v)[16], char* obase, int OP, float& s1, float& s2) {
  f32x2_t p1 = {0.f, 0.f}, p2 = {0.f, 0.f};
#pragma unroll
  for (int r = 0; r < 16; r += 2) {
    const int dm = (r & 3) + 8 * (r >> 2);
    const f32x2_t x = {v[r], v[r + 1]};
    p1 += x;
    p2 = __builtin_elementwise_fma(x, x, p2);
    if constexpr (sizeof(T) == 2) {
      const uint32_t pk = cvt_pk_bf16(x.x, x.y);
      *(uint16_t*)(obase + dm * OP) = (uint16_t)(pk & 0xffffu);
      *(uint16_t*)(obase + (dm + 1) * OP) = (uint16_t)(pk >> 16);
    } else {
      *(float*)(obase + dm * OP) = x.x;
      *(float*)(obase + (dm + 1) * OP) = x.y;
    }
  }
  s1 += p1.x + p1.y;
  s2 += p2.x + p2.y;
}

__device__ __forceinline__ int xcd_remap(int bid, int nblk) {
  const int q = nblk >> 3, r = nblk & 7, x = bid & 7, i = bid >> 3;
  return (x < r ? x * (q + 1) : r * (q + 1) + (x - r) * q) + i;
}

struct Idx4 { int cv, x, y, b; };
__device__ __forceinline__ Idx4 split4(unsigned i, unsigned CV, unsigned Wc, unsigned Hc) {
  const unsigned p = i / CV, q = p / Wc, b = q / Hc;
  Idx4 r;
  r.cv = (int)(i - p * CV); r.x = (int)(p - q * Wc); r.y = (int)(q - b * Hc); r.b = (int)b;
  return r;
}
static inline int cdiv(int a, int b) { return (a + b - 1) / b; }
```

### image_segmentation_amd/csrc/segk_internal.h

```cpp
#pragma once
#include <hip/hip_runtime.h>
#include <stdint.h>

struct ConvArgs {
  const void* srcA;
  const void* srcB;
  const void* w;
  const float* bias;
  const float* scale;
  const float* shift;
  void* out;
  void* out2;
  float* stats;
  void* act_out;
  int B, H, W;
  int CA, CB;
  int Ntot, CO1, CO2;
  int twl, tiles_x, tiles_y;
  int unshuf, shuffle;
  int persistent;
  int act;
};
int segk_conv_igemm_launch(const ConvArgs& a, int geo, int dtype, hipStream_t st);

#define SEGK_MAX_DEVICES 64
int segk_device_index();
int segk_num_cus();

int segk_conv_use_rs(int cin_p, int n_p, int dtype, int W);
int segk_conv_rs_rows(int B, int H, int W, int n_p);
void segk_conv_rs_grid(int B, int H, int W, int NT, int* gw_out, int* GW_out);
int segk_conv_rs_launch(const ConvArgs& a, hipStream_t st);
int segk_stem_rows(int B, int H, int W, int Cin, int Cout, int dtype);
int segk_stem_launch(const float* x, const float* w, void* z, void* xn, float* stats, int B, int H, int W, int Cin, int Cout,
                     hipStream_t st);
int segk_stem_wgrad_slabs(int B, int H, int W, int Cin, int Cout, int dtype);
int segk_stem_wgrad_launch(const float* x, const void* dz, float* slabs, int B, int H, int W, int Cin, int Cout,
                           hipStream_t st);
int segk_convt_stream_ok(int B, int H, int W, int Cin, int Cout, int dtype);
int segk_convt_stream_launch(const void* x, const void* wp, const float* bias4, void* out, int B, int H, int W, int Cin,
                             int Cout, hipStream_t st);
int segk_convt_stream_dgrad_ok(int B, int H, int W, int Cin, int Cout, int dtype);
int segk_convt_stream_dgrad_launch(const void* dout, const void* wd, void* din, int B, int H, int W, int Cin, int Cout,
                                   hipStream_t st);
int segk_conv_use_ws(int cin_p, int n_p, int dtype);
int segk_conv_use_pipe(int cin_p, int n_p, int dtype);
int segk_conv_writes_act(int cin_p, int n_p, int dtype);
int segk_conv_bm(int geo, int unit);
int segk_conv_twl(int bm, int W);

struct SegkPackEntry {
  const float* w;
  void* dst_fwd;
  void* dst_dgrad;
  int Cout, CA, CB, Coutp, CAp, CBp;
  int block0;
  int kind;
  int pad_[2];
};
static_assert(sizeof(SegkPackEntry) == 64, "SegkPackEntry is 64 bytes");

struct WgradArgs {
  const void* dz;
  const void* srcA;
  const void* srcB;
  const float* scale;
  const float* shift;
  float* slabs;
  const void* zeros;
  int B, H, W;
  int CD, CA, CB;
  int S;
};
int segk_wgrad_launch(const WgradArgs& a, int geo, int dtype, hipStream_t st);
int segk_wgrad_wc(int CD, int CA, int CB, int geo, int dtype);

struct GemmArgs {
  const void* A;
  const char* w;
  const float* bias;
  void* out;
  long M;
  int N;
  int nchunks;
  int nchA;
  int lda;
  int H, W;
  int Cout;
  int act;
  int ksplit;
  long split_stride;
};
int segk_gemm_dma_ok(long M, int nchunks, int nchA, int N, int cout_shuffle, int lda, int mode);
int segk_gemm_dma_launch(const GemmArgs& g, int mode, hipStream_t st);
```

### image_segmentation_amd/csrc/stem.hip

```cpp
#include "common.hpp"
#include "segk_internal.h"

namespace {

typedef unsigned u32x4 __attribute__((ext_vector_type(4)));

template <int CTRL> __device__ __forceinline__ float dpp_add(float v) {
  const int x = __builtin_amdgcn_update_dpp(0, __float_as_int(v), CTRL, 0xf, 0xf, true);
  return v + __int_as_float(x);
}
__device__ __forceinline__ float row16_sum(float v) {
  v = dpp_add<0xB1>(v);
  v = dpp_add<0x4E>(v);
  v = dpp_add<0x141>(v);
  v = dpp_add<0x140>(v);
  return v;
}
__device__ __forceinline__ unsigned pk_bf16(float a, float b) {
  return cvt_pk_bf16(a, b);
}

constexpr int STEM_WAVES = 8;
#ifndef STEM_WG_PER_CU
#define STEM_WG_PER_CU 2
#endif

__global__ __launch_bounds__(STEM_WAVES * 64, 4) void stem_stream_kernel(const float* __restrict__ x, const float* __restrict__ w,
                                                                         bf16_t* __restrict__ z, bf16_t* __restrict__ xn,
                                                                         float* __restrict__ stats, int B, int H, int W,
                                                                         int Cin, long nblk) {
  __shared__ float red[STEM_WAVES][64][2];
  const int lane = threadIdx.x & 63, lc = lane & 15, lq = lane >> 4;
  const int wave = __builtin_amdgcn_readfirstlane(threadIdx.x >> 6);
  const int K = Cin * 9;
  const long HW = (long)H * W;

  u32x4 wf[4];
#pragma unroll
  for (int g = 0; g < 4; ++g) {
    const int p = g >> 1, half = g & 1;
    const int n_row = p * 32 + 8 * (lc >> 2) + 4 * half + (lc & 3);
    float f[8];
#pragma unroll
    for (int e = 0; e < 8; ++e) {
      const int k = lq * 8 + e;
      f[e] = k < K ? w[(size_t)n_row * K + k] : 0.f;
    }
    wf[g] = (u32x4){pk_bf16(f[0], f[1]), pk_bf16(f[2], f[3]), pk_bf16(f[4], f[5]), pk_bf16(f[6], f[7])};
  }
  unsigned gpk[2] = {0u, 0u};
#pragma unroll
  for (int e = 0; e < 8; ++e) {
    const int k = lq * 8 + e;
    const int ci = k / 9, tap = k - ci * 9;
    const int dy = tap / 3 - 1, dx = tap % 3 - 1;
    const unsigned bits = k < K ? (unsigned)((dy + 1) | ((dx + 1) << 2) | (ci << 4) | (1 << 6)) : 0x05u;
    gpk[e >> 2] |= bits << (8 * (e & 3));
  }

  float s1[2][8], s2[2][8];
#pragma unroll
  for (int p = 0; p < 2; ++p)
#pragma unroll
    for (int j = 0; j < 8; ++j) { s1[p][j] = 0.f; s2[p][j] = 0.f; }

  const int W16 = W / 16;
  const unsigned step = gridDim.x * STEM_WAVES;
  struct Blk { unsigned row; int xx; unsigned ok; float g[8]; };
  auto fetch = [&](unsigned blk, Blk& k) {
    k.row = blk / (unsigned)W16;
    k.xx = (int)(blk - k.row * W16) * 16 + lc;
    const unsigned b = k.row / (unsigned)H;
    const int y = (int)(k.row - b * H);
    const unsigned base = (b * (unsigned)Cin) * (unsigned)HW + (unsigned)y * (unsigned)W + (unsigned)k.xx;
    unsigned ok = 0;
#pragma unroll
    for (int e = 0; e < 8; ++e) {
      const unsigned bits = gpk[e >> 2] >> (8 * (e & 3));
      const int dy = (int)(bits & 3u) - 1, dx = (int)((bits >> 2) & 3u) - 1, ci = (int)((bits >> 4) & 3u);
      const bool v = ((bits >> 6) & 1u) & ((unsigned)(y + dy) < (unsigned)H) & ((unsigned)(k.xx + dx) < (unsigned)W);
      ok |= (v ? 1u : 0u) << e;
      const int off = ci * (int)HW + dy * W + dx;
      k.g[e] = x[base + (unsigned)(v ? off : 0)];
    }
    k.ok = ok;
  };
  auto work = [&](const Blk& k) {
    float v[8];
#pragma unroll
    for (int e = 0; e < 8; ++e) v[e] = ((k.ok >> e) & 1u) ? k.g[e] : 0.f;
    const u32x4 bf = {pk_bf16(v[0], v[1]), pk_bf16(v[2], v[3]), pk_bf16(v[4], v[5]), pk_bf16(v[6], v[7])};
    f32x4 acc[4];
#pragma unroll
    for (int g = 0; g < 4; ++g)
      acc[g] = __builtin_amdgcn_mfma_f32_16x16x32_bf16(__builtin_bit_cast(bf16x8, wf[g]), __builtin_bit_cast(bf16x8, bf),
                                                       (f32x4){0.f, 0.f, 0.f, 0.f}, 0, 0, 0);
    const size_t opix = (size_t)k.row * W + k.xx;
#pragma unroll
    for (int p = 0; p < 2; ++p) {
      const f32x4 a0 = acc[2 * p], a1 = acc[2 * p + 1];
      const float o[8] = {a0[0], a0[1], a0[2], a0[3], a1[0], a1[1], a1[2], a1[3]};
#pragma unroll
      for (int j = 0; j < 8; ++j) { s1[p][j] += o[j]; s2[p][j] = fmaf(o[j], o[j], s2[p][j]); }
      const u32x4 ov = {pk_bf16(o[0], o[1]), pk_bf16(o[2], o[3]), pk_bf16(o[4], o[5]), pk_bf16(o[6], o[7])};
      *(u32x4*)(z + opix * 64 + p * 32 + lq * 8) = ov;
    }
    if (xn != nullptr) {
      u32x4 c = {0u, 0u, 0u, 0u};
      if (lq == 0) {
        const unsigned b = k.row / (unsigned)H;
        const float* px = x + (size_t)b * Cin * HW + (size_t)(k.row - b * H) * W + k.xx;
        const float c0 = px[0], c1 = Cin > 1 ? px[HW] : 0.f, c2 = Cin > 2 ? px[2 * HW] : 0.f;
        c.x = pk_bf16(c0, c1);
        c.y = pk_bf16(c2, 0.f);
      }
      *(u32x4*)(xn + opix * 32 + lq * 8) = c;
    }
  };
  {
    const unsigned nb = (unsigned)nblk;
    unsigned blk = blockIdx.x * STEM_WAVES + wave;
    for (; blk < nb; blk += 2 * step) {
      const bool two = blk + step < nb;
      Blk ka, kb;
      fetch(blk, ka);
      fetch(two ? blk + step : blk, kb);
      __builtin_amdgcn_sched_barrier(0);
      work(ka);
      if (two) work(kb);
    }
  }
  if (stats == nullptr) return;
#pragma unroll
  for (int p = 0; p < 2; ++p)
#pragma unroll
    for (int j = 0; j < 8; ++j) {
      const float a = row16_sum(s1[p][j]), q = row16_sum(s2[p][j]);
      if (lc == 0) {
        red[wave][p * 32 + lq * 8 + j][0] = a;
        red[wave][p * 32 + lq * 8 + j][1] = q;
      }
    }
  __syncthreads();
  if (threadIdx.x < 64) {
    float a = 0.f, q = 0.f;
#pragma unroll
    for (int wv = 0; wv < STEM_WAVES; ++wv) { a += red[wv][threadIdx.x][0]; q += red[wv][threadIdx.x][1]; }
    ((float2*)stats)[(size_t)blockIdx.x * 64 + threadIdx.x] = make_float2(a, q);
  }
}

struct __attribute__((packed, aligned(4))) F4U { float v[4]; };

__global__ __launch_bounds__(STEM_WAVES * 64, 2) void stem_wgrad_kernel(const float* __restrict__ x, const bf16_t* __restrict__ dz,
                                                                        float* __restrict__ slabs, int B, int H, int W, int Cin,
                                                                        long nblk) {
  __shared__ __attribute__((aligned(16))) char lds[4 * 64 * 32 * 4];
  typedef __attribute__((address_space(3))) s16x4* lds_v4;
  const int lane = threadIdx.x & 63;
  const int wave = __builtin_amdgcn_readfirstlane(threadIdx.x >> 6);
  const int K = Cin * 9;
  const long HW = (long)H * W;
  char* const slot = lds + wave * 2048;

  const int j = lane & 31, hh = lane >> 5;
  const int ci = j / 9, tap = j - ci * 9;
  const int dy = tap / 3 - 1, dx = tap % 3 - 1;
  const bool jok = j < K;
  const int g = lane >> 4, i16 = lane & 15, q = i16 >> 2, p = i16 & 3;
  const int coff = (16 * (g & 1) + 4 * p) * 2, xa = 8 * (g >> 1) + q;
  const int lp = lane >> 2, lc4 = lane & 3;

  f32x16 acc[2];
#pragma unroll
  for (int nh = 0; nh < 2; ++nh)
#pragma unroll
    for (int r = 0; r < 16; ++r) acc[nh][r] = 0.f;

  const int W16 = W / 16;
  const long step = (long)gridDim.x * STEM_WAVES;
  for (long blk = (long)blockIdx.x * STEM_WAVES + wave; blk < nblk; blk += step) {
    const long row = blk / W16;
    const int x0 = (int)(blk - row * W16) * 16;
    const long b = row / H;
    const int y = (int)(row - b * H);
    const bf16_t* dp = dz + ((size_t)row * W + x0 + lp) * 64 + lc4 * 8;
    const uint4 d0 = *(const uint4*)dp, d1 = *(const uint4*)(dp + 32);
    float v[8];
    const int xs = x0 + 8 * hh + dx;
    const bool rok = jok & ((unsigned)(y + dy) < (unsigned)H);
    const float* src = x + ((size_t)(b * Cin + ci) * H + (y + dy)) * W + xs;
    if (rok && xs >= 0 && xs + 8 <= W) {
      const F4U a = *(const F4U*)src, c = *(const F4U*)(src + 4);
#pragma unroll
      for (int e = 0; e < 4; ++e) { v[e] = a.v[e]; v[4 + e] = c.v[e]; }
    } else {
#pragma unroll
      for (int e = 0; e < 8; ++e) v[e] = (rok && (unsigned)(xs + e) < (unsigned)W) ? src[e] : 0.f;
    }
    *(uint4*)(slot + lp * 64 + lc4 * 16) = d0;
    *(uint4*)(slot + 1024 + lp * 64 + lc4 * 16) = d1;
    const u32x4 fbv = {pk_bf16(v[0], v[1]), pk_bf16(v[2], v[3]), pk_bf16(v[4], v[5]), pk_bf16(v[6], v[7])};
    const bf16x8 fb = __builtin_bit_cast(bf16x8, fbv);
    __builtin_amdgcn_fence(__ATOMIC_RELEASE, "wavefront");
#pragma unroll
    for (int nh = 0; nh < 2; ++nh) {
      const s16x4 a0 = __builtin_amdgcn_ds_read_tr16_b64_v4i16((lds_v4)(slot + nh * 1024 + xa * 64 + coff));
      const s16x4 a1 = __builtin_amdgcn_ds_read_tr16_b64_v4i16((lds_v4)(slot + nh * 1024 + (xa + 4) * 64 + coff));
      const bf16x8 fa = __builtin_bit_cast(bf16x8, __builtin_shufflevector(a0, a1, 0, 1, 2, 3, 4, 5, 6, 7));
      acc[nh] = __builtin_amdgcn_mfma_f32_32x32x16_bf16(fa, fb, acc[nh], 0, 0, 0);
    }
  }

  float* const red = (float*)lds;
  const int col = lane & 31, lh = lane >> 5;
  auto put = [&](int slot_i) {
#pragma unroll
    for (int nh = 0; nh < 2; ++nh)
#pragma unroll
      for (int r = 0; r < 16; ++r) {
        const int n = 32 * nh + (r & 3) + 8 * (r >> 2) + 4 * lh;
        red[(slot_i * 64 + n) * 32 + col] = acc[nh][r];
      }
  };
  auto add = [&](int slot_i) {
#pragma unroll
    for (int nh = 0; nh < 2; ++nh)
#pragma unroll
      for (int r = 0; r < 16; ++r) {
        const int n = 32 * nh + (r & 3) + 8 * (r >> 2) + 4 * lh;
        acc[nh][r] += red[(slot_i * 64 + n) * 32 + col];
      }
  };
  __syncthreads();
  if (wave >= 4) put(wave - 4);
  __syncthreads();
  if (wave < 4) add(wave);
  __syncthreads();
  if (wave == 2 || wave == 3) put(wave - 2);
  __syncthreads();
  if (wave < 2) add(wave);
  __syncthreads();
  if (wave == 1) put(0);
  __syncthreads();
  if (wave == 0) {
    add(0);
    float* const slab = slabs + (size_t)blockIdx.x * 64 * 32;
#pragma unroll
    for (int nh = 0; nh < 2; ++nh)
#pragma unroll
      for (int r = 0; r < 16; ++r) {
        const int n = 32 * nh + (r & 3) + 8 * (r >> 2) + 4 * lh;
        slab[n * 32 + col] = acc[nh][r];
      }
  }
}

}

int segk_stem_wgrad_slabs(int B, int H, int W, int Cin, int Cout, int dtype) {
  const int rows = segk_stem_rows(B, H, W, Cin, Cout, dtype);
  if (rows <= 0) return 0;
  const long nblk = (long)B * H * (W / 16);
  long g = (nblk + STEM_WAVES - 1) / STEM_WAVES;
  const long cap = (long)segk_num_cus() * 2;
  if (g > cap) g = cap;
  return (int)g;
}

int segk_stem_wgrad_launch(const float* x, const void* dz, float* slabs, int B, int H, int W, int Cin, int Cout,
                           hipStream_t st) {
  SEGK_REQUIRE(x && dz && slabs, "stem_wgrad: null pointer");
  const int g = segk_stem_wgrad_slabs(B, H, W, Cin, Cout, SEGK_DT_BF16);
  SEGK_REQUIRE(g > 0, "stem_wgrad: shape not served (bf16, 1..3 input channels, 64 output channels, W a multiple of 16)");
  const long nblk = (long)B * H * (W / 16);
  hipLaunchKernelGGL(stem_wgrad_kernel, dim3(g), dim3(STEM_WAVES * 64), 0, st, x, (const bf16_t*)dz, slabs, B, H, W, Cin, nblk);
  SEGK_CHECK_LAUNCH("stem_wgrad");
  return 0;
}

int segk_stem_rows(int B, int H, int W, int Cin, int Cout, int dtype) {
  if (dtype != SEGK_DT_BF16 || B <= 0 || H <= 0 || W <= 0 || W % 16 != 0 || Cin < 1 || Cin > 3 || Cout != 64) return 0;
  if ((long long)B * H * W * 64 >= 2147483647LL * 16 || (long long)B * Cin * H * W >= 2147483647LL) return 0;
  const long nblk = (long)B * H * (W / 16);
  long g = (nblk + STEM_WAVES - 1) / STEM_WAVES;
  const long cap = (long)segk_num_cus() * STEM_WG_PER_CU;
  if (g > cap) g = cap;
  return (int)(g > 1024 ? 1024 : g);
}

int segk_stem_launch(const float* x, const float* w, void* z, void* xn, float* stats, int B, int H, int W, int Cin, int Cout,
                     hipStream_t st) {
  SEGK_REQUIRE(x && w && z, "stem3x3: null pointer");
  const int g = segk_stem_rows(B, H, W, Cin, Cout, SEGK_DT_BF16);
  SEGK_REQUIRE(g > 0, "stem3x3: shape not served (bf16, 1..3 input channels, 64 output channels, W a multiple of 16)");
  const long nblk = (long)B * H * (W / 16);
  hipLaunchKernelGGL(stem_stream_kernel, dim3(g), dim3(STEM_WAVES * 64), 0, st, x, w, (bf16_t*)z, (bf16_t*)xn, stats, B, H, W, Cin,
                     nblk);
  SEGK_CHECK_LAUNCH("stem3x3");
  return 0;
}
```

### image_segmentation_amd/ops.py

```python
import os
import sys
import weakref

import torch

from . import _lib

_DT = {torch.float32: _lib.F32, torch.bfloat16: _lib.BF16}
_compute_dtype = torch.bfloat16


def set_compute_dtype(dtype):
    global _compute_dtype
    if dtype not in _DT:
        raise ValueError("compute dtype must be torch.float32 or torch.bfloat16")
    _compute_dtype = dtype


def get_compute_dtype():
    return _compute_dtype


def pad32(c):
    return (c + 31) // 32 * 32


_raw_stream = getattr(torch._C, "_cuda_getCurrentRawStream", None)
_raw_device = getattr(torch._C, "_cuda_getDevice", None)


def _stream():
    if _raw_stream is not None and _raw_device is not None:
        return _raw_stream(_raw_device())
    return torch.cuda.current_stream().cuda_stream


def _require_cuda(t, what):
    if not t.is_cuda:
        raise RuntimeError(f"{what}: expected a CUDA/HIP tensor -- image_segmentation_amd has no CPU path "
                           "(the CPU oracle lives in oracle/ and is test infrastructure only)")


def _p(t):
    return 0 if t is None else t.data_ptr()


def new_act(B, C, H, W, dtype, device):
    Cp = pad32(C)
    buf = torch.empty((B, H, W, Cp), dtype=dtype, device=device)
    if Cp != C:
        buf[..., C:].zero_()
    return buf.permute(0, 3, 1, 2)[:, :C]


def act_view(buf, C):
    return buf.permute(0, 3, 1, 2)[:, :C]


def act_info(t, dtype):
    if t.dim() != 4 or t.dtype != dtype or not t.is_cuda:
        return None
    B, C, H, W = t.shape
    sb, sc, sh, sw = t.stride()
    Cp = sw if W > 1 else (sh if H > 1 else pad32(C))
    if sc != 1 or Cp < C or Cp % 32 != 0 or Cp != pad32(C):
        return None
    if (W > 1 and sw != Cp) or (H > 1 and sh != W * Cp) or (B > 1 and sb != H * W * Cp):
        return None
    if (t.storage_offset() * t.element_size()) % 16 != 0:
        return None
    return t.data_ptr(), Cp


def to_act(x, dtype):
    _require_cuda(x, "to_act")
    if act_info(x, dtype) is not None:
        return x
    B, C, H, W = x.shape
    src = x.detach()
    if C % 32 == 0 and src.stride(1) == 1 and src.permute(0, 2, 3, 1).is_contiguous():
        return act_view(src.permute(0, 2, 3, 1).to(dtype), C)
    if src.dtype != torch.float32 or not src.is_contiguous():
        src = src.float().contiguous()
    out = torch.empty((B, H, W, pad32(C)), dtype=dtype, device=x.device)
    _lib.call("segk_nchw_to_nhwc", src.data_ptr(), out.data_ptr(), B, C, H, W, pad32(C), _DT[dtype], _stream())
    return act_view(out, C)


def act_to_nchw(t):
    info = act_info(t, t.dtype)
    if info is None:
        return t.float().contiguous()
    B, C, H, W = t.shape
    out = torch.empty((B, C, H, W), dtype=torch.float32, device=t.device)
    _lib.call("segk_nhwc_to_nchw", info[0], out.data_ptr(), B, C, H, W, info[1], _DT[t.dtype], _stream())
    return out


def _private_act_copy(t, dtype):
    ptr, Cp = act_info(t, dtype)
    B, C, H, W = t.shape
    n = B * H * W * Cp
    out = torch.empty((B, H, W, Cp), dtype=dtype, device=t.device)
    out.view(-1).copy_(torch.as_strided(t, (n,), (1,), t.storage_offset()))
    return out


def _raw(t, dtype):
    t = to_act(t, dtype)
    ptr, Cp = act_info(t, dtype)
    return t, ptr, Cp


INPLACE_SKIP_GRAD = True
FUSE_BN_REDUCE = True
HEAD_ON_Z = os.environ.get("SEGK_HEAD_ON_Z", "1") != "0"
_OPT_EPOCH = [0]


def _on_optimizer_step(optimizer, args, kwargs):
    _OPT_EPOCH[0] += 1


from torch.optim.optimizer import register_optimizer_step_post_hook as _register_step_hook

_register_step_hook(_on_optimizer_step)


def invalidate_packed_weights():
    _OPT_EPOCH[0] += 1


class PackCache:

    def __init__(self):
        self._c = {}
        self.multi = {}

    def get_pair(self, key_a, key_b, param, builder, meta=None):
        ver = (param._version, param.data_ptr(), param.device, _OPT_EPOCH[0] if param.requires_grad else -1)
        hit = self._c.get(key_a)
        if hit is None or hit[0] != ver:
            a, b = builder()
            hit = (ver, a)
            self._c[key_a] = hit
            self._c[key_b] = (ver, b)
            if meta is not None:
                self.multi[key_a] = (meta[0], key_b, param) + tuple(meta[1:])
        return hit[1]

    def get_registered(self, key, param, builder, meta):
        self.multi[key] = (meta[0], None, param) + tuple(meta[1:])
        return self.get(key, param, builder)

    def get(self, key, param, builder):
        ver = (param._version, param.data_ptr(), param.device, _OPT_EPOCH[0] if param.requires_grad else -1)
        hit = self._c.get(key)
        if hit is None or hit[0] != ver:
            hit = (ver, builder())
            self._c[key] = hit
        return hit[1]


def pack_conv(w, CA, CB, dtype, mode, taps=9):
    Cout = w.shape[0]
    Coutp, CAp, CBp = pad32(Cout), pad32(CA), (pad32(CB) if CB else 0)
    dst = torch.empty(((CAp + CBp) * taps * Coutp,), dtype=dtype, device=w.device)
    wf = w.detach()
    if wf.dtype != torch.float32 or not wf.is_contiguous():
        wf = wf.float().contiguous()
    _lib.call("segk_pack_conv_weight", wf.data_ptr(), dst.data_ptr(), Cout, CA, CB, Coutp, CAp, CBp, taps, mode,
              _DT[dtype], _stream())
    return dst


def pack_conv_both(w, CA, CB, dtype):
    Cout = w.shape[0]
    Coutp, CAp, CBp = pad32(Cout), pad32(CA), (pad32(CB) if CB else 0)
    n = (CAp + CBp) * 9 * Coutp
    both = torch.empty((2 * n,), dtype=dtype, device=w.device)
    wf = w.detach()
    if wf.dtype != torch.float32 or not wf.is_contiguous():
        wf = wf.float().contiguous()
    _lib.call("segk_pack_conv3x3_both", wf.data_ptr(), both.data_ptr(), both[n:].data_ptr(), Cout, CA, CB, Coutp, CAp, CBp,
              _DT[dtype], _stream())
    return both[:n], both[n:]


_PACK_CONVT_CHUNK = [0]


def _entry_geometry(kind, param, d0, d1):
    if kind == 0:
        Cout = param.shape[0]
        Coutp, CAp, CBp = pad32(Cout), pad32(d0), (pad32(d1) if d1 else 0)
        return (CAp + CBp) * 9 * Coutp, (Cout, d0, d1, Coutp, CAp, CBp), (CAp + CBp) // 32 * (Coutp // 32)
    if kind == 1:
        Cin, Cout = param.shape[0], param.shape[1]
        Cinp, Coutp = pad32(Cin), pad32(Cout)
        if not _PACK_CONVT_CHUNK[0]:
            _PACK_CONVT_CHUNK[0] = _lib.query("segk_pack_convt_chunk")
        n = Cinp * 4 * Coutp
        return n, (Cout, Cin, 0, Coutp, Cinp, 0), (n + _PACK_CONVT_CHUNK[0] - 1) // _PACK_CONVT_CHUNK[0]
    if kind == 3:
        Cout = param.shape[0]
        Coutp, CAp = pad32(Cout), pad32(d0)
        if not _PACK_CONVT_CHUNK[0]:
            _PACK_CONVT_CHUNK[0] = _lib.query("segk_pack_convt_chunk")
        n = CAp * Coutp
        return n, (Cout, d0, 0, Coutp, CAp, 0), (n + _PACK_CONVT_CHUNK[0] - 1) // _PACK_CONVT_CHUNK[0]
    Cout = param.shape[0]
    reps = d0 if d0 > 0 else 4
    return reps * pad32(Cout), (Cout, d0, 0, pad32(Cout), 0, 0), 1


def _pack_caches(model):
    seen, out, stack = set(), [], list(model.modules())
    while stack:
        m = stack.pop()
        if id(m) in seen:
            continue
        seen.add(id(m))
        c = getattr(m, "cache", None)
        if isinstance(c, PackCache):
            out.append(c)
        for v in vars(m).values():
            if isinstance(v, torch.nn.Module) and id(v) not in seen:
                stack.extend(v.modules())
    return out


def repack_stale(model):
    st = model.__dict__.get("_segk_pack_state")
    if st is None:
        st = model.__dict__["_segk_pack_state"] = {"epoch": _OPT_EPOCH[0], "caches": None, "tables": {}}
        return
    if st["epoch"] == _OPT_EPOCH[0]:
        return
    st["epoch"] = _OPT_EPOCH[0]
    if st["caches"] is None:
        st["caches"] = _pack_caches(model)
    groups = {}
    for cache in st["caches"]:
        for key_a, (kind, key_b, param, d0, d1, dtype) in cache.multi.items():
            ha = cache._c.get(key_a)
            hb = cache._c.get(key_b) if key_b is not None else None
            if ha is None or (key_b is not None and hb is None):
                continue
            if not param.is_cuda or param.dtype != torch.float32 or not param.is_contiguous():
                continue
            ver = (param._version, param.data_ptr(), param.device, _OPT_EPOCH[0] if param.requires_grad else -1)
            if ha[0] == ver and (hb is None or hb[0] == ver):
                continue
            n, _, _ = _entry_geometry(kind, param, d0, d1)
            want = torch.float32 if kind == 2 else dtype
            if ha[1].numel() != n or ha[1].dtype != want or not ha[1].is_contiguous():
                continue
            if hb is not None and (hb[1].numel() != n or hb[1].dtype != want or not hb[1].is_contiguous()):
                continue
            groups.setdefault((dtype, param.device), []).append(
                (cache, key_a, key_b, ver, param, ha[1], None if hb is None else hb[1], kind, d0, d1))
    for (dtype, dev), items in groups.items():
        if len(items) < 2:
            continue
        for c0 in range(0, len(items), 64):
            chunk = items[c0:c0 + 64]
            sig = tuple((it[4].data_ptr(), it[5].data_ptr(), 0 if it[6] is None else it[6].data_ptr(), it[7], it[8], it[9])
                        for it in chunk)
            tab = st["tables"].get((dtype, dev, c0))
            if tab is None or tab[0] != sig:
                import numpy as np
                words = np.zeros((len(chunk), 8), dtype=np.int64)
                ints = words.view(np.int32).reshape(len(chunk), 16)
                blk = 0
                for i, (_, _, _, _, param, a, b, kind, d0, d1) in enumerate(chunk):
                    _, dims, nblk = _entry_geometry(kind, param, d0, d1)
                    words[i, 0], words[i, 1], words[i, 2] = param.data_ptr(), a.data_ptr(), 0 if b is None else b.data_ptr()
                    ints[i, 6:12] = dims
                    ints[i, 12], ints[i, 13] = blk, kind
                    blk += nblk
                tab = (sig, torch.from_numpy(words).to(dev), blk)
                st["tables"][(dtype, dev, c0)] = tab
            with torch.cuda.device(dev):
                _lib.call("segk_pack_multi", tab[1].data_ptr(), len(chunk), tab[2], _DT[dtype], _stream())
            for cache, key_a, key_b, ver, _, a, b, _, _, _ in chunk:
                cache._c[key_a] = (ver, a)
                if key_b is not None:
                    cache._c[key_b] = (ver, b)


def pack_convt(w, dtype, mode):
    Cin, Cout = w.shape[0], w.shape[1]
    dst = torch.empty((pad32(Cin) * 4 * pad32(Cout),), dtype=dtype, device=w.device)
    wf = w.detach()
    if wf.dtype != torch.float32 or not wf.is_contiguous():
        wf = wf.float().contiguous()
    _lib.call("segk_pack_convt_weight", wf.data_ptr(), dst.data_ptr(), Cin, Cout, pad32(Cin), pad32(Cout), mode,
              _DT[dtype], _stream())
    return dst


class KernelTimer:

    def __init__(self):
        self.rows = {}
        self.levels = {}

    def span(self, tag, flops=0.0, nbytes=0.0):
        return _Span(self, tag, flops, nbytes)

    @staticmethod
    def _sum(rows):
        out = {}
        for key, r in rows.items():
            ms = sum(a.elapsed_time(b) for a, b in r["ev"])
            out[key] = {"launches": len(r["ev"]), "ms": ms, "flops": r["flops"], "bytes": r["bytes"]}
        return out

    def summary(self):
        torch.cuda.synchronize()
        return self._sum(self.rows)

    def level_summary(self):
        torch.cuda.synchronize()
        return self._sum(self.levels)


class _Span:
    def __init__(self, timer, tag, flops, nbytes):
        self.t, self.tag, self.flops, self.nbytes = timer, tag, flops, nbytes

    def __enter__(self):
        self.a = torch.cuda.Event(enable_timing=True)
        self.a.record()

    def __exit__(self, *exc):
        b = torch.cuda.Event(enable_timing=True)
        b.record()
        r = self.t.rows.setdefault(self.tag, {"ev": [], "flops": 0.0, "bytes": 0.0})
        r["ev"].append((self.a, b))
        r["flops"] += self.flops
        r["bytes"] += self.nbytes
        if _LEVEL is not None:
            phase = {"conv3x3_igemm": "dgrad" if _LEVEL[1] else "fwd", "wgrad3x3": "wgrad"}.get(self.tag, "other")
            r = self.t.levels.setdefault((_LEVEL[0], phase), {"ev": [], "flops": 0.0, "bytes": 0.0})
            r["ev"].append((self.a, b))
            r["flops"] += self.flops
            r["bytes"] += self.nbytes


class _NoSpan:
    def __enter__(self):
        return None

    def __exit__(self, *exc):
        return False


_NOSPAN = _NoSpan()
TIMER = None
_LEVEL = None


def name_levels(model):
    for name, m in model.named_modules():
        if hasattr(m, "bn_modules") and hasattr(m, "cache"):
            m.__dict__["_segk_level"] = name or "block"


class _level_scope:
    def __init__(self, mod, backward):
        self.v = (mod.__dict__.get("_segk_level"), backward) if TIMER is not None else None

    def __enter__(self):
        global _LEVEL
        self.prev = _LEVEL
        if self.v is not None and self.v[0] is not None:
            _LEVEL = self.v

    def __exit__(self, *exc):
        global _LEVEL
        _LEVEL = self.prev
        return False


def clock_probe(launches=4, blocks=256, iters=20000, device=None):
    dev = torch.device("cuda", torch.cuda.current_device()) if device is None else torch.device(device)
    res = {"method": f"s_memtime / s_memrealtime (100 MHz) around {iters} rounds of 16 v_mfma_f32_32x32x16_bf16 (or 32 "
                     f"v_mfma_f32_16x16x32_bf16: the same matrix work) per wave, one wave per SIMD on {blocks} workgroups, "
                     f"launch {launches} of {launches} back to back; pseudo-random register operands"}
    for shape, name in ((0, "mfma_32x32x16"), (1, "mfma_16x16x32")):
        out = torch.zeros((blocks * 4 * 2,), dtype=torch.int64, device=dev)
        with torch.cuda.device(dev):
            for _ in range(launches):
                _lib.call("segk_clock_probe", out.data_ptr(), blocks, iters, shape, _stream())
            torch.cuda.synchronize(dev)
        t = out.view(-1, 2).double().cpu()
        ghz = (t[:, 0] / t[:, 1].clamp(min=1.0)) * 0.1
        ms = float(t[:, 1].median()) / 1e5
        res[name] = {"median_ghz": round(float(ghz.median()), 4), "min_ghz": round(float(ghz.min()), 4),
                     "max_ghz": round(float(ghz.max()), 4), "probe_ms": round(ms, 3),
                     "probe_pflops": round(blocks * 4 * iters * 16 * 32768.0 / (ms * 1e-3) / 1e15, 3)}
    res["median_ghz"] = res["mfma_32x32x16"]["median_ghz"]
    return res


def _span(tag, flops=0.0, nbytes=0.0):
    return _NOSPAN if TIMER is None else TIMER.span(tag, flops, nbytes)


def _es(dtype):
    return 2 if dtype == torch.bfloat16 else 4


def _f32(n, dev):
    return torch.empty((n,), dtype=torch.float32, device=dev)


_ZERO_PAGES = {}


def _zero_page(dev):
    key = torch.device(dev)
    if key.type == "cuda" and key.index is None:
        key = torch.device("cuda", torch.cuda.current_device())
    z = _ZERO_PAGES.get(key)
    if z is None:
        z = torch.zeros(256, dtype=torch.uint8, device=key)
        _ZERO_PAGES[key] = z
    return z


def conv3x3(srcA, ptrA, CAp, ptrB, CBp, wpacked, out_ptr, CO1p, out2_ptr, CO2p, B, H, W, dtype, scale=None,
            shift=None, stats=None, alg=None, tag="conv3x3_igemm"):
    cin, cout = alg if alg else (CAp + CBp, CO1p + CO2p)
    P, e = B * H * W, _es(dtype)
    with _span(tag, 2.0 * P * 9 * cin * cout, P * (cin + cout) * e + 9.0 * cin * cout * e):
        _lib.call("segk_conv3x3", ptrA, ptrB, wpacked.data_ptr(), 0, _p(scale), _p(shift), out_ptr, out2_ptr,
                  _p(stats), B, H, W, CAp, CBp, CO1p, CO2p, _DT[dtype], _stream())


def wgrad(dz_ptr, CDp, ptrA, CAp, ptrB, CBp, B, H, W, geo, dtype, dev, scale=None, shift=None, alg=None):
    taps = {0: 9, 1: 1, 2: 4}[geo]
    cd, ck = alg if alg else (CDp, CAp + CBp)
    P, e = B * H * W, _es(dtype)
    pk = P * (4 if geo == 2 else 1)
    tiles = _lib.query("segk_wgrad_tiles", B, H, W, geo, _DT[dtype])
    S = _lib.query("segk_wgrad_split", tiles, CDp, CAp, CBp, geo, _DT[dtype])
    slabs = _f32(S * CDp * taps * (CAp + CBp), dev)
    tag = {0: "wgrad3x3", 1: "wgrad1x1", 2: "wgrad_convt"}[geo]
    with _span(tag, 2.0 * P * taps * cd * ck, (P * cd + pk * ck) * e + 4.0 * taps * cd * ck):
        _lib.call("segk_wgrad", dz_ptr, ptrA, ptrB, _p(scale), _p(shift), slabs.data_ptr(), _zero_page(dev).data_ptr(),
                  S, B, H, W, CDp, CAp, CBp, geo, _DT[dtype], _stream())
    return slabs, S


_GRAD_DEST = None
_GRAD_DEST_USED = set()


def grad_destination_begin(callback):
    global _GRAD_DEST
    _GRAD_DEST = callback
    _GRAD_DEST_USED.clear()


def grad_destination_end():
    global _GRAD_DEST
    _GRAD_DEST = None
    _GRAD_DEST_USED.clear()


def _grad_buffer(param, shape, dev):
    if _GRAD_DEST is not None and param is not None and param.data_ptr() not in _GRAD_DEST_USED:
        d = _GRAD_DEST(param)
        if d is not None and tuple(d.shape) == tuple(shape) and d.dtype == torch.float32:
            _GRAD_DEST_USED.add(param.data_ptr())
            return d
    return torch.empty(shape, dtype=torch.float32, device=dev)


def wgrad_to_param(slabs, S, shape, N, CA, CB, taps, dev, param=None):
    grad = _grad_buffer(param, shape, dev)
    with _span("wgrad_reduce", 0.0, 4.0 * (S + 1) * grad.numel()):
        _lib.call("segk_wgrad_reduce", slabs.data_ptr(), S, grad.data_ptr(), N, CA, CB, pad32(N), pad32(CA),
                  pad32(CB) if CB else 0, taps, _stream())
    return grad


class ReduceBatch:

    def __init__(self, dev):
        self.dev, self.jobs, self.keep, self.nbytes = dev, [], [], 0.0

    def add_weight(self, slabs, S, shape, N, CA, CB, taps, param=None):
        grad = _grad_buffer(param, shape, self.dev)
        self.jobs.append(_lib.ReduceJob(slabs.data_ptr(), grad.data_ptr(), 0, S, N, CA, CB, pad32(N), pad32(CA),
                                        pad32(CB) if CB else 0, taps, 0))
        self.keep.append(slabs)
        self.nbytes += 4.0 * (S + 1) * grad.numel()
        return grad

    def add_colsum(self, part, rows, ntot, col0, ncols):
        out = _f32(ncols, self.dev)
        self.jobs.append(_lib.ReduceJob(part.data_ptr(), out.data_ptr(), 1, rows, ntot, col0, ncols, 0, 0, 0, 0, 0))
        self.keep.append(part)
        self.nbytes += 8.0 * rows * ncols
        return out

    def flush(self):
        for i in range(0, len(self.jobs), 4):
            chunk = self.jobs[i:i + 4]
            arr = (_lib.ReduceJob * len(chunk))(*chunk)
            with _span("wgrad_reduce", 0.0, self.nbytes * len(chunk) / len(self.jobs)):
                _lib.call("segk_wgrad_reduce_multi", arr, len(chunk), _stream())
        self.jobs, self.keep, self.nbytes = [], [], 0.0


def bn_finalize(stats, tiles, C, count, conv_bias, bn_w, bn_b, rmean, rvar, momentum, eps, training, dev):
    Cp = pad32(C)
    scale, shift = _f32(Cp, dev), _f32(Cp, dev)
    mean, rstd = _f32(Cp, dev), _f32(Cp, dev)
    with _span("bn_finalize", 0.0, 8.0 * tiles * Cp if training else 0.0):
        _lib.call("segk_bn_finalize", _p(stats), tiles, Cp, C, float(count), _p(conv_bias), bn_w.data_ptr(),
                  bn_b.data_ptr(), _p(rmean), _p(rvar), float(momentum), float(eps), int(training), scale.data_ptr(),
                  shift.data_ptr(), mean.data_ptr(), rstd.data_ptr(), _stream())
    return scale, shift, mean, rstd


def bn_relu_bwd(dy_ptr, z_ptr, dz_ptr, scale, shift, mean, rstd, P, C, dtype, dev, ready=None, frozen=False):
    Cp = pad32(C)
    dgamma, dbeta = _f32(C, dev), _f32(C, dev)
    if frozen:
        nb = _lib.query("segk_bn_bwd_blocks", P, Cp, _DT[dtype])
        part, coef = _f32(nb * Cp * 2, dev), _f32(2 * Cp, dev)
        scratch = torch.empty((P * Cp,), dtype=dtype, device=dev)
        _lib.call("segk_bn_relu_bwd", dy_ptr, z_ptr, scratch.data_ptr(), scale.data_ptr(), shift.data_ptr(), mean.data_ptr(),
                  rstd.data_ptr(), P, Cp, C, part.data_ptr(), dgamma.data_ptr(), dbeta.data_ptr(), coef.data_ptr(),
                  _DT[dtype], _stream())
        zero_part = torch.zeros((Cp * 2,), dtype=torch.float32, device=dev)
        unused_g, unused_b = _f32(C, dev), _f32(C, dev)
        _lib.call("segk_bn_relu_bwd_from_part", dy_ptr, z_ptr, dz_ptr, scale.data_ptr(), shift.data_ptr(),
                  mean.data_ptr(), rstd.data_ptr(), P, Cp, C, zero_part.data_ptr(), 1, unused_g.data_ptr(), unused_b.data_ptr(),
                  coef.data_ptr(), _DT[dtype], _stream())
        return dgamma, dbeta
    if ready is not None:
        part, nb = ready
        coef = _f32(2 * Cp, dev)
        with _span("bn_relu_bwd", 0.0, 3.0 * P * C * _es(dtype)):
            _lib.call("segk_bn_relu_bwd_from_part", dy_ptr, z_ptr, dz_ptr, scale.data_ptr(), shift.data_ptr(),
                      mean.data_ptr(), rstd.data_ptr(), P, Cp, C, part.data_ptr(), nb, dgamma.data_ptr(), dbeta.data_ptr(),
                      coef.data_ptr(), _DT[dtype], _stream())
        return dgamma, dbeta
    nb = _lib.query("segk_bn_bwd_blocks", P, Cp, _DT[dtype])
    part, coef = _f32(nb * Cp * 2, dev), _f32(2 * Cp, dev)
    with _span("bn_relu_bwd", 0.0, 5.0 * P * C * _es(dtype)):
        _lib.call("segk_bn_relu_bwd", dy_ptr, z_ptr, dz_ptr, scale.data_ptr(), shift.data_ptr(), mean.data_ptr(),
                  rstd.data_ptr(), P, Cp, C, part.data_ptr(), dgamma.data_ptr(), dbeta.data_ptr(), coef.data_ptr(),
                  _DT[dtype], _stream())
    return dgamma, dbeta


def channel_sum(ptr, P, C, dtype, dev):
    Cp = pad32(C)
    nb = _lib.query("segk_bn_bwd_blocks", P, Cp, _DT[dtype])
    part, out = _f32(nb * Cp, dev), _f32(C, dev)
    _lib.call("segk_channel_sum", ptr, P, Cp, C, part.data_ptr(), out.data_ptr(), _DT[dtype], _stream())
    return out


_ZERO_POOL = {}


def _zero_grad_like(n, dev):
    key = torch.device(dev)
    if key.type == "cuda" and key.index is None:
        key = torch.device("cuda", torch.cuda.current_device())
    pool = _ZERO_POOL.get(key)
    if pool is None or pool[0] != _OPT_EPOCH[0] or pool[2] + n > pool[1].numel():
        pool = [_OPT_EPOCH[0], torch.zeros(max(16384, 4 * n), dtype=torch.float32, device=key), 0]
        _ZERO_POOL[key] = pool
    off = pool[2]
    pool[2] = off + (n + 3) // 4 * 4
    return pool[1][off:off + n]


_NBT_DEFER = None


class defer_batch_counters:

    def __enter__(self):
        global _NBT_DEFER
        self.prev, _NBT_DEFER = _NBT_DEFER, []
        return self

    def __exit__(self, *exc):
        global _NBT_DEFER
        pending, _NBT_DEFER = _NBT_DEFER, self.prev
        if pending and exc[0] is None:
            torch._foreach_add_(pending, 1)
        return False


def _bump_batch_counters(*bns):
    for bn in bns:
        if bn.num_batches_tracked is None:
            continue
        if _NBT_DEFER is not None:
            _NBT_DEFER.append(bn.num_batches_tracked)
        else:
            bn.num_batches_tracked.add_(1)


def _param_f32(p):
    t = p.detach()
    if t.dtype != torch.float32 or not t.is_contiguous():
        t = t.float().contiguous()
    return t


def _bn_momentum(bn):
    if bn.momentum is None:
        raise NotImplementedError("BatchNorm2d(momentum=None) (cumulative moving average) is not supported by the fused "
                                  "DoubleConv kernels; the reference uses the default momentum 0.1 (unet/unet.py:17,20)")
    return bn.momentum


def _convt_fwd(mod, x_t, px, w, b, B, H, W, Cin, Cout, dtype, dev, both=False):
    Cinp, Coutp = pad32(Cin), pad32(Cout)
    if both:
        wp = mod.cache.get_pair(("tf", dtype), ("td", dtype), w, lambda: (pack_convt(w, dtype, 0), pack_convt(w, dtype, 1)),
                                meta=(1, 0, 0, dtype))
    else:
        wp = mod.cache.get(("tf", dtype), w, lambda: pack_convt(w, dtype, 0))

    def bias4():
        t = torch.zeros((4, Coutp), dtype=torch.float32, device=dev)
        t[:, :Cout] = _param_f32(b)
        return t
    b4 = None if b is None else mod.cache.get_registered(("tb", dtype), b, bias4, meta=(2, 0, 0, dtype))
    out = torch.empty((B, 2 * H, 2 * W, Coutp), dtype=dtype, device=dev)
    with _span("convt_fwd", 2.0 * B * H * W * Cin * 4 * Cout, B * H * W * (Cin + 4 * Cout) * _es(dtype)):
        _lib.call("segk_convt2x2_fwd", px, wp.data_ptr(), _p(b4), out.data_ptr(), B, H, W, Cinp, Coutp, _DT[dtype],
                  _stream())
    return out


def _convt_bwd(mod, x_t, w, pd, B, H, W, Cin, Cout, dtype, dev, need_dx, has_bias, chan_sum=None, batch=None):
    Cinp, Coutp = pad32(Cin), pad32(Cout)
    px = act_info(x_t, dtype)[0]
    dx = None
    if need_dx:
        wd = mod.cache.get(("td", dtype), w, lambda: pack_convt(w, dtype, 1))
        dxb = torch.empty((B, H, W, Cinp), dtype=dtype, device=dev)
        with _span("convt_dgrad", 2.0 * B * H * W * Cin * 4 * Cout, B * H * W * (Cin + 4 * Cout) * _es(dtype)):
            _lib.call("segk_convt2x2_dgrad", pd, wd.data_ptr(), dxb.data_ptr(), B, H, W, Cinp, Coutp, _DT[dtype],
                      _stream())
        dx = act_view(dxb, Cin)
    slabs, S = wgrad(px, Cinp, pd, Coutp, 0, 0, B, H, W, 2, dtype, dev, alg=(Cin, Cout))
    if batch is not None:
        dw = batch.add_weight(slabs, S, w.shape, Cin, Cout, 0, 4, param=w)
    else:
        dw = wgrad_to_param(slabs, S, w.shape, Cin, Cout, 0, 4, dev, param=w)
    db = None
    if has_bias:
        db = chan_sum if chan_sum is not None else channel_sum(pd, B * 4 * H * W, Cout, dtype, dev)
    return dx, dw, db


def _head_fwd(px, Cp, w, b, B, C, H, W, dtype, dev, bn=None):
    ncls = w.shape[0]
    if ncls > _lib.MAX_CLASSES:
        raise RuntimeError(f"output head supports up to {_lib.MAX_CLASSES} classes, got {ncls}")
    w2 = _param_f32(w).reshape(ncls, C)
    logits = torch.empty((B, ncls, H, W), dtype=torch.float32, device=dev)
    with _span("head_fwd", 2.0 * B * H * W * C * ncls, B * H * W * (C * _es(dtype) + 4 * ncls)):
        if bn is not None:
            _lib.call("segk_head_fwd_bn", px, bn[0].data_ptr(), bn[1].data_ptr(), w2.data_ptr(), _param_f32(b).data_ptr(),
                      logits.data_ptr(), B, H, W, Cp, C, ncls, _DT[dtype], _stream())
        else:
            _lib.call("segk_head_fwd", px, w2.data_ptr(), _param_f32(b).data_ptr(), logits.data_ptr(), B, H, W, Cp, C,
                      ncls, _DT[dtype], _stream())
    return logits


def _head_bwd(dlogits, px, Cp, w, B, C, H, W, dtype, dev, bn=None, on_z=False):
    ncls = w.shape[0]
    dl = dlogits
    if dl.dtype != torch.float32 or not dl.is_contiguous():
        dl = dl.float().contiguous()
    w2 = _param_f32(w).reshape(ncls, C)
    dy = torch.empty((B, H, W, Cp), dtype=dtype, device=dev)
    part = _f32(_lib.query("segk_head_part_floats", B * H * W, Cp), dev)
    dw = _grad_buffer(w, w.shape, dev)
    db = _f32(ncls, dev)
    ready = None
    with _span("head_bwd", 4.0 * B * H * W * C * ncls, B * H * W * (2 * C * _es(dtype) + 4 * ncls)):
        if on_z:
            sc, sh, mu, rs = bn
            bnpart, nb = None, 0
            if FUSE_BN_REDUCE:
                nb = _lib.query("segk_head_bwd_blocks", B * H * W)
                bnpart = _f32(nb * Cp * 2, dev)
                ready = (bnpart, nb)
            _lib.call("segk_head_bwd_bn", dl.data_ptr(), px, w2.data_ptr(), dy.data_ptr(), part.data_ptr(),
                      dw.data_ptr(), db.data_ptr(), B, H, W, Cp, C, ncls, sc.data_ptr(), sh.data_ptr(), mu.data_ptr(),
                      rs.data_ptr(), _p(bnpart), _DT[dtype], _stream())
        elif bn is not None and FUSE_BN_REDUCE:
            sc, sh, mu, rs = bn
            nb = _lib.query("segk_head_bwd_blocks", B * H * W)
            bnpart = _f32(nb * Cp * 2, dev)
            _lib.call("segk_head_bwd_bnstat", dl.data_ptr(), px, w2.data_ptr(), dy.data_ptr(), part.data_ptr(),
                      dw.data_ptr(), db.data_ptr(), B, H, W, Cp, C, ncls, sc.data_ptr(), sh.data_ptr(), mu.data_ptr(),
                      rs.data_ptr(), bnpart.data_ptr(), _DT[dtype], _stream())
            ready = (bnpart, nb)
        else:
            _lib.call("segk_head_bwd", dl.data_ptr(), px, w2.data_ptr(), dy.data_ptr(), part.data_ptr(), dw.data_ptr(),
                      db.data_ptr(), B, H, W, Cp, C, ncls, _DT[dtype], _stream())
    return dy, dw, db, ready


class BlockCfg:
    __slots__ = ("mod", "up_mod", "emit_pool")

    def __init__(self, mod, up_mod=None, emit_pool=False):
        self.mod, self.up_mod, self.emit_pool = mod, up_mod, emit_pool


class DoubleConvFn(torch.autograd.Function):

    @staticmethod
    def forward(ctx, cfg, xa, xb, w1, b1, g1, be1, w2, b2, g2, be2, up_x, up_w, up_b, head_w, head_b):
        with _level_scope(cfg.mod, False):
            return DoubleConvFn._forward(ctx, cfg, xa, xb, w1, b1, g1, be1, w2, b2, g2, be2, up_x, up_w, up_b, head_w, head_b)

    @staticmethod
    def _forward(ctx, cfg, xa, xb, w1, b1, g1, be1, w2, b2, g2, be2, up_x, up_w, up_b, head_w, head_b):
        mod = cfg.mod
        dtype = mod.compute_dtype or _compute_dtype
        _require_cuda(xa, "DoubleConvReLU")
        dev = xa.device
        B, CA, H, W = xa.shape
        up_t, up_dims = None, None
        if up_x is not None:
            if xb is not None:
                raise ValueError("DoubleConvFn: give either xb or up_x")
            _require_cuda(up_x, "ConvTranspose2d")
            Bu, Cin_u, Hu, Wu = up_x.shape
            Cout_u = up_w.shape[1]
            if (2 * Hu, 2 * Wu) != (H, W):
                raise RuntimeError(f"Sizes of tensors must match except in dimension 1: {tuple(xa.shape)} vs "
                                   f"{(Bu, Cout_u, 2 * Hu, 2 * Wu)} (H and W must be multiples of 16)")
            up_t, pux, _ = _raw(up_x, dtype)
            ubuf = _convt_fwd(cfg.up_mod, up_t, pux, up_w, up_b, Bu, Hu, Wu, Cin_u, Cout_u, dtype, dev,
                              both=any(ctx.needs_input_grad))
            xb = act_view(ubuf, Cout_u)
            up_dims = (Bu, Hu, Wu, Cin_u, Cout_u)
        CB = 0 if xb is None else xb.shape[1]
        Cout = w1.shape[0]
        Coutp = pad32(Cout)
        training = mod.training
        bn1, bn2 = mod.bn_modules()
        want_grad = any(ctx.needs_input_grad)
        stem_rows = 0
        if (xb is None and act_info(xa, dtype) is None and xa.dtype == torch.float32 and xa.is_contiguous()
                and w1.dtype == torch.float32 and w1.is_contiguous()):
            stem_rows = _lib.query("segk_stem3x3_rows", B, H, W, CA, Cout, _DT[dtype])
        stem_raw = False
        if stem_rows:
            xa_t, pA, CAp = None, 0, pad32(CA)
            if want_grad and _lib.query("segk_stem3x3_wgrad_slabs", B, H, W, CA, Cout, _DT[dtype]):
                xa_t, stem_raw = xa.detach(), True
            elif want_grad:
                xbuf = torch.empty((B, H, W, CAp), dtype=dtype, device=dev)
                xa_t, pA = act_view(xbuf, CA), xbuf.data_ptr()
        else:
            xa_t, pA, CAp = _raw(xa, dtype)
        xb_t, pB, CBp = (None, 0, 0) if xb is None else _raw(xb, dtype)
        if training and want_grad:
            w1p = mod.cache.get_pair(("w1f", dtype), ("w1d", dtype), w1, lambda: pack_conv_both(w1, CA, CB, dtype),
                                     meta=(0, CA, CB, dtype))
            w2p = mod.cache.get_pair(("w2f", dtype), ("w2d", dtype), w2, lambda: pack_conv_both(w2, Cout, 0, dtype),
                                     meta=(0, Cout, 0, dtype))
        else:
            w1p = mod.cache.get(("w1f", dtype), w1, lambda: pack_conv(w1, CA, CB, dtype, 0))
            w2p = mod.cache.get(("w2f", dtype), w2, lambda: pack_conv(w2, Cout, 0, dtype, 0))
        tiles1 = stem_rows or _lib.query("segk_conv_tiles", B, H, W, CAp + CBp, Coutp, _DT[dtype])
        tiles2 = _lib.query("segk_conv_tiles", B, H, W, Coutp, Coutp, _DT[dtype])
        P = B * H * W

        z1 = torch.empty((B, H, W, Coutp), dtype=dtype, device=dev)
        st1 = _f32(_lib.query("segk_bn_stats_floats", tiles1, Coutp), dev) if training else None
        if stem_rows:
            e = _es(dtype)
            with _span("conv3x3_igemm", 2.0 * P * 9 * CA * Cout, P * (4 * CA + Cout * e) + 9.0 * CA * Cout * 4):
                _lib.call("segk_stem3x3", xa.data_ptr(), w1.data_ptr(), z1.data_ptr(), pA, _p(st1), B, H, W, CA, Cout,
                          _DT[dtype], _stream())
        else:
            conv3x3(xa_t, pA, CAp, pB, CBp, w1p, z1.data_ptr(), Coutp, 0, 0, B, H, W, dtype, stats=st1, alg=(CA + CB, Cout))
        sc1, sh1, mu1, rs1 = bn_finalize(st1, tiles1, Cout, P, None if b1 is None else _param_f32(b1), _param_f32(g1),
                                         _param_f32(be1), bn1.running_mean, bn1.running_var, _bn_momentum(bn1), bn1.eps,
                                         training, dev)
        z2 = torch.empty((B, H, W, Coutp), dtype=dtype, device=dev)
        st2 = _f32(_lib.query("segk_bn_stats_floats", tiles2, Coutp), dev) if training else None
        a1 = None
        if training and want_grad and _lib.query("segk_conv_writes_act_q", Coutp, Coutp, _DT[dtype]):
            a1 = torch.empty((B, H, W, Coutp), dtype=dtype, device=dev)
            with _span("conv3x3_igemm", 2.0 * P * 9 * Cout * Cout, (P * 2 * Cout + 9.0 * Cout * Cout) * _es(dtype)):
                _lib.call("segk_conv3x3_act", z1.data_ptr(), w2p.data_ptr(), sc1.data_ptr(), sh1.data_ptr(), z2.data_ptr(),
                          a1.data_ptr(), _p(st2), B, H, W, Coutp, Coutp, _DT[dtype], _stream())
        else:
            conv3x3(z1, z1.data_ptr(), Coutp, 0, 0, w2p, z2.data_ptr(), Coutp, 0, 0, B, H, W, dtype, scale=sc1,
                    shift=sh1, stats=st2, alg=(Cout, Cout))
        sc2, sh2, mu2, rs2 = bn_finalize(st2, tiles2, Cout, P, None if b2 is None else _param_f32(b2), _param_f32(g2),
                                         _param_f32(be2), bn2.running_mean, bn2.running_var, _bn_momentum(bn2), bn2.eps,
                                         training, dev)
        if training:
            _bump_batch_counters(bn1, bn2)
        head_on_z = head_w is not None and HEAD_ON_Z
        y = None if head_on_z else torch.empty((B, H, W, Coutp), dtype=dtype, device=dev)
        pooled = None
        if head_on_z:
            pass
        elif cfg.emit_pool:
            if H < 2 or W < 2:
                raise RuntimeError("MaxPool2d(2,2): input smaller than the window")
            pooled = torch.empty((B, H // 2, W // 2, Coutp), dtype=dtype, device=dev)
            with _span("bn_relu_apply", 0.0, 2.25 * P * Cout * _es(dtype)):
                _lib.call("segk_bn_relu_apply_pool", z2.data_ptr(), y.data_ptr(), pooled.data_ptr(), sc2.data_ptr(),
                          sh2.data_ptr(), B, H, W, Coutp, _DT[dtype], _stream())
        else:
            with _span("bn_relu_apply", 0.0, 2.0 * P * Cout * _es(dtype)):
                _lib.call("segk_bn_relu_apply", z2.data_ptr(), y.data_ptr(), sc2.data_ptr(), sh2.data_ptr(), P, Coutp,
                          _DT[dtype], _stream())
        logits = None
        if head_on_z:
            logits = _head_fwd(z2.data_ptr(), Coutp, head_w, head_b, B, Cout, H, W, dtype, dev, bn=(sc2, sh2))
        elif head_w is not None:
            logits = _head_fwd(y.data_ptr(), Coutp, head_w, head_b, B, Cout, H, W, dtype, dev)

        ctx.cfg, ctx.dtype, ctx.dims = cfg, dtype, (B, H, W, CA, CB, Cout)
        ctx.training = training
        ctx.has_bias = (b1 is not None, b2 is not None)
        ctx.up_dims = up_dims
        ctx.has_head = head_w is not None
        ctx.head_on_z = head_on_z
        ctx.stem_raw = stem_raw
        ctx.save_for_backward(xa_t, xb_t, z1, z2, sc1, sh1, mu1, rs1, sc2, sh2, mu2, rs2, w1, w2, a1,
                              y if (cfg.emit_pool or head_w is not None) else None, up_t, up_w, head_w)
        if logits is not None:
            return logits
        if pooled is not None:
            y_out = act_view(y, Cout)
            ctx.y_ref = weakref.ref(y_out)
            return y_out, act_view(pooled, Cout)
        return act_view(y, Cout)

    @staticmethod
    def backward(ctx, *grads):
        with _level_scope(ctx.cfg.mod, True):
            return DoubleConvFn._backward(ctx, *grads)

    @staticmethod
    def _backward(ctx, *grads):
        frozen = not ctx.training
        (xa_t, xb_t, z1, z2, sc1, sh1, mu1, rs1, sc2, sh2, mu2, rs2, w1, w2, a1, y, up_t, up_w, head_w) = ctx.saved_tensors
        cfg, dtype = ctx.cfg, ctx.dtype
        mod = cfg.mod
        B, H, W, CA, CB, Cout = ctx.dims
        dev = z1.device
        Coutp, CAp, CBp = pad32(Cout), pad32(CA), (pad32(CB) if CB else 0)
        P = B * H * W
        pA = 0 if ctx.stem_raw else act_info(xa_t, dtype)[0]
        pB = 0 if xb_t is None else act_info(xb_t, dtype)[0]
        need = ctx.needs_input_grad

        ready = None
        d_head_w = d_head_b = None
        keep = None
        if ctx.has_head:
            src = z2 if ctx.head_on_z else y
            dy_buf, d_head_w, d_head_b, ready = _head_bwd(grads[0], src.data_ptr(), Coutp, head_w, B, Cout, H, W, dtype, dev,
                                                          bn=(sc2, sh2, mu2, rs2), on_z=ctx.head_on_z)
            pdy, keep = dy_buf.data_ptr(), dy_buf
        elif cfg.emit_pool:
            dy, dpool = grads
            rc_skip, rc_pool = sys.getrefcount(dy), sys.getrefcount(dpool)
            if dpool is None:
                keep, pdy, _ = _raw(dy, dtype)
            else:
                dp_t, pdp, _ = _raw(dpool, dtype)
                if dy is None:
                    keep = torch.empty((B, H, W, Coutp), dtype=dtype, device=dev)
                    pdy, acc, nbytes = keep.data_ptr(), 0, 2.25
                else:
                    yo = getattr(ctx, "y_ref", lambda: None)()
                    uc = getattr(dy, "_use_count", None)
                    shared = uc is None or uc() > 2 or rc_skip > rc_pool
                    hooked = INPLACE_SKIP_GRAD is False or shared or (yo is not None and bool(yo._backward_hooks))
                    keep, pdy, _ = _raw(dy, dtype)
                    if hooked and keep.data_ptr() == dy.data_ptr():
                        keep = _private_act_copy(keep, dtype)
                        pdy = keep.data_ptr()
                    acc, nbytes = 1, 3.25
                nb = _lib.query("segk_maxpool_bwd_stat_blocks", B, H, W, Coutp, _DT[dtype]) if FUSE_BN_REDUCE else 0
                with _span("maxpool_bwd", 0.0, nbytes * P * Cout * _es(dtype)):
                    if nb > 0:
                        part = _f32(nb * Coutp * 2, dev)
                        _lib.call("segk_maxpool2x2_bwd_bnstat", y.data_ptr(), pdp, pdy, B, H, W, Coutp, acc,
                                  sc2.data_ptr(), sh2.data_ptr(), mu2.data_ptr(), rs2.data_ptr(), part.data_ptr(),
                                  z2.data_ptr(), _DT[dtype], _stream())
                        ready = (part, nb)
                    else:
                        _lib.call("segk_maxpool2x2_bwd", y.data_ptr(), pdp, pdy, B, H, W, Coutp, acc, _DT[dtype],
                                  _stream())
        else:
            keep, pdy, _ = _raw(grads[0], dtype)

        dz2 = torch.empty((B, H, W, Coutp), dtype=dtype, device=dev)
        dg2, dbe2 = bn_relu_bwd(pdy, z2.data_ptr(), dz2.data_ptr(), sc2, sh2, mu2, rs2, P, Cout, dtype, dev, ready=ready,
                                frozen=frozen)
        del keep
        w2d = mod.cache.get(("w2d", dtype), w2, lambda: pack_conv(w2, Cout, 0, dtype, 1))
        da1 = torch.empty((B, H, W, Coutp), dtype=dtype, device=dev)
        conv3x3(dz2, dz2.data_ptr(), Coutp, 0, 0, w2d, da1.data_ptr(), Coutp, 0, 0, B, H, W, dtype, alg=(Cout, Cout))
        if a1 is not None:
            slabs, S = wgrad(dz2.data_ptr(), Coutp, a1.data_ptr(), Coutp, 0, 0, B, H, W, 0, dtype, dev, alg=(Cout, Cout))
        else:
            slabs, S = wgrad(dz2.data_ptr(), Coutp, z1.data_ptr(), Coutp, 0, 0, B, H, W, 0, dtype, dev, scale=sc1,
                             shift=sh1, alg=(Cout, Cout))
        dw2 = wgrad_to_param(slabs, S, w2.shape, Cout, Cout, 0, 9, dev, param=w2)
        rb = ReduceBatch(dev)
        del slabs, dz2

        dg1, dbe1 = bn_relu_bwd(da1.data_ptr(), z1.data_ptr(), da1.data_ptr(), sc1, sh1, mu1, rs1, P, Cout, dtype, dev,
                                frozen=frozen)
        dz1 = da1
        dxa = dxb = None
        dxb_buf, chan_sum = None, None
        has_up = ctx.up_dims is not None
        if need[1] or need[2] or has_up:
            w1d = mod.cache.get(("w1d", dtype), w1, lambda: pack_conv(w1, CA, CB, dtype, 1))
            dxa_buf = torch.empty((B, H, W, CAp), dtype=dtype, device=dev)
            dxb_buf = torch.empty((B, H, W, CBp), dtype=dtype, device=dev) if CB else None
            std = None
            if has_up:
                tiles_d = _lib.query("segk_conv_tiles", B, H, W, Coutp, CAp + CBp, _DT[dtype])
                std = _f32(_lib.query("segk_bn_stats_floats", tiles_d, CAp + CBp), dev)
            conv3x3(dz1, dz1.data_ptr(), Coutp, 0, 0, w1d, dxa_buf.data_ptr(), CAp, _p(dxb_buf), CBp, B, H, W, dtype,
                    stats=std, alg=(Cout, CA + CB))
            dxa = act_view(dxa_buf, CA)
            dxb = act_view(dxb_buf, CB) if CB else None
            if has_up:
                chan_sum = rb.add_colsum(std, tiles_d, CAp + CBp, CAp, CB)
        if ctx.stem_raw:
            S = _lib.query("segk_stem3x3_wgrad_slabs", B, H, W, CA, Cout, _DT[dtype])
            slabs = _f32(S * 64 * 32, dev)
            with _span("wgrad3x3", 2.0 * P * 9 * CA * Cout, P * (Cout * _es(dtype) + 4 * CA) + 4.0 * 9 * CA * Cout):
                _lib.call("segk_stem3x3_wgrad", xa_t.data_ptr(), dz1.data_ptr(), slabs.data_ptr(), B, H, W, CA, Cout,
                          _DT[dtype], _stream())
            dw1 = wgrad_to_param(slabs, S, w1.shape, Cout, 9 * CA, 0, 1, dev, param=w1)
        else:
            slabs, S = wgrad(dz1.data_ptr(), Coutp, pA, CAp, pB, CBp, B, H, W, 0, dtype, dev, alg=(Cout, CA + CB))
            dw1 = wgrad_to_param(slabs, S, w1.shape, Cout, CA, CB, 9, dev, param=w1)
        del slabs
        if frozen:
            db1 = sc1[:Cout] * dbe1 if ctx.has_bias[0] else None
            db2 = sc2[:Cout] * dbe2 if ctx.has_bias[1] else None
        else:
            db1 = _zero_grad_like(Cout, dev) if ctx.has_bias[0] else None
            db2 = _zero_grad_like(Cout, dev) if ctx.has_bias[1] else None

        d_up_x = d_up_w = d_up_b = None
        if has_up:
            Bu, Hu, Wu, Cin_u, Cout_u = ctx.up_dims
            d_up_x, d_up_w, d_up_b = _convt_bwd(cfg.up_mod, up_t, up_w, dxb_buf.data_ptr(), Bu, Hu, Wu, Cin_u, Cout_u, dtype,
                                                dev, need[11], cfg.up_mod.upsample.bias is not None, chan_sum=chan_sum,
                                                batch=rb)
            dxb = None
        rb.flush()
        return (None, dxa, dxb, dw1, db1, dg1, dbe1, dw2, db2, dg2, dbe2, d_up_x, d_up_w, d_up_b, d_head_w, d_head_b)


def double_conv(mod, xa, xb, params, emit_pool=False, head=None, up_mod=None, up_x=None):
    cfg = BlockCfg(mod, up_mod, emit_pool and head is None)
    uw = ub = None
    if up_mod is not None:
        uw, ub = up_mod.upsample.weight, up_mod.upsample.bias
    hw = hb = None
    if head is not None:
        hw, hb = head.weight, head.bias
    return DoubleConvFn.apply(cfg, xa, xb, *params, up_x, uw, ub, hw, hb)


class MaxPoolFn(torch.autograd.Function):

    @staticmethod
    def forward(ctx, x, dtype):
        _require_cuda(x, "MaxPool2d")
        x_t, px, Cp = _raw(x, dtype)
        B, C, H, W = x.shape
        y = torch.empty((B, H // 2, W // 2, Cp), dtype=dtype, device=x.device)
        with _span("maxpool_fwd", 0.0, 1.25 * B * H * W * C * _es(dtype)):
            _lib.call("segk_maxpool2x2_fwd", px, y.data_ptr(), B, H, W, Cp, _DT[dtype], _stream())
        ctx.save_for_backward(x_t)
        ctx.dtype = dtype
        return act_view(y, C)

    @staticmethod
    def backward(ctx, dy):
        (x_t,) = ctx.saved_tensors
        dtype = ctx.dtype
        B, C, H, W = x_t.shape
        px, Cp = act_info(x_t, dtype)
        dy_t, pdy, _ = _raw(dy, dtype)
        dx = torch.empty((B, H, W, Cp), dtype=dtype, device=x_t.device)
        with _span("maxpool_bwd", 0.0, 2.25 * B * H * W * C * _es(dtype)):
            _lib.call("segk_maxpool2x2_bwd", px, pdy, dx.data_ptr(), B, H, W, Cp, 0, _DT[dtype], _stream())
        return act_view(dx, C), None


class ConvT2x2Fn(torch.autograd.Function):

    @staticmethod
    def forward(ctx, mod, x, w, b):
        dtype = mod.compute_dtype or _compute_dtype
        _require_cuda(x, "ConvTranspose2d")
        B, Cin, H, W = x.shape
        Cout = w.shape[1]
        x_t, px, _ = _raw(x, dtype)
        out = _convt_fwd(mod, x_t, px, w, b, B, H, W, Cin, Cout, dtype, x.device, both=any(ctx.needs_input_grad))
        ctx.mod, ctx.dtype, ctx.dims = mod, dtype, (B, H, W, Cin, Cout)
        ctx.has_bias = b is not None
        ctx.save_for_backward(x_t, w)
        return act_view(out, Cout)

    @staticmethod
    def backward(ctx, dout):
        x_t, w = ctx.saved_tensors
        B, H, W, Cin, Cout = ctx.dims
        d_t, pd, _ = _raw(dout, ctx.dtype)
        dx, dw, db = _convt_bwd(ctx.mod, x_t, w, pd, B, H, W, Cin, Cout, ctx.dtype, x_t.device, ctx.needs_input_grad[1],
                                ctx.has_bias)
        return None, dx, dw, db


class Conv1x1Fn(torch.autograd.Function):

    @staticmethod
    def forward(ctx, mod, x, w, b):
        dtype = mod.compute_dtype or _compute_dtype
        _require_cuda(x, "Conv2d 1x1")
        dev = x.device
        B, Cin, H, W = x.shape
        Cout = w.shape[0]
        Cinp, Coutp = pad32(Cin), pad32(Cout)
        x_t, px, _ = _raw(x, dtype)
        wp = mod.cache.get_registered(("cf", dtype), w, lambda: pack_conv(w, Cin, 0, dtype, 0, taps=1), meta=(3, Cin, 0, dtype))

        def biasp():
            t = torch.zeros((Coutp,), dtype=torch.float32, device=dev)
            t[:Cout] = _param_f32(b)
            return t
        bp = None if b is None else mod.cache.get_registered(("cb", dtype), b, biasp, meta=(2, 1, 0, dtype))
        out = torch.empty((B, H, W, Coutp), dtype=dtype, device=dev)
        _lib.call("segk_conv1x1", px, wp.data_ptr(), _p(bp), out.data_ptr(), B, H, W, Cinp, Coutp, _DT[dtype], _stream())
        ctx.mod, ctx.dtype, ctx.dims = mod, dtype, (B, H, W, Cin, Cout)
        ctx.has_bias = b is not None
        ctx.save_for_backward(x_t, w)
        return act_view(out, Cout)

    @staticmethod
    def backward(ctx, dout):
        x_t, w = ctx.saved_tensors
        mod, dtype = ctx.mod, ctx.dtype
        B, H, W, Cin, Cout = ctx.dims
        dev = x_t.device
        Cinp, Coutp = pad32(Cin), pad32(Cout)
        d_t, pd, _ = _raw(dout, dtype)
        px = act_info(x_t, dtype)[0]
        dx = None
        if ctx.needs_input_grad[1]:
            wd = mod.cache.get(("cd", dtype), w, lambda: pack_conv(w, Cin, 0, dtype, 1, taps=1))
            dxb = torch.empty((B, H, W, Cinp), dtype=dtype, device=dev)
            _lib.call("segk_conv1x1", pd, wd.data_ptr(), 0, dxb.data_ptr(), B, H, W, Coutp, Cinp, _DT[dtype], _stream())
            dx = act_view(dxb, Cin)
        slabs, S = wgrad(pd, Coutp, px, Cinp, 0, 0, B, H, W, 1, dtype, dev)
        dw = wgrad_to_param(slabs, S, w.shape, Cout, Cin, 0, 1, dev, param=w)
        db = channel_sum(pd, B * H * W, Cout, dtype, dev) if ctx.has_bias else None
        return None, dx, dw, db


class ReconHeadFn(torch.autograd.Function):

    @staticmethod
    def forward(ctx, mod, x, w, b):
        dtype = mod.compute_dtype or _compute_dtype
        _require_cuda(x, "reconstruction head")
        dev = x.device
        B, Cin, H, W = x.shape
        Cout = w.shape[0]
        x_t, px, Cp = _raw(x, dtype)
        rec = torch.empty((B, Cout, H, W), dtype=torch.float32, device=dev)
        P = B * H * W
        with _span("recon_head_fwd", 2.0 * P * 9 * Cin * Cout, P * (Cin * _es(dtype) + 4 * Cout)):
            _lib.call("segk_recon_head_fwd", px, _param_f32(w).data_ptr(), 0 if b is None else _param_f32(b).data_ptr(),
                      rec.data_ptr(), B, H, W, Cp, Cin, Cout, _DT[dtype], _stream())
        ctx.mod, ctx.dtype, ctx.dims = mod, dtype, (B, H, W, Cin, Cout)
        ctx.has_bias = b is not None
        ctx.save_for_backward(x_t, w, rec)
        return rec

    @staticmethod
    def backward(ctx, drec):
        x_t, w, rec = ctx.saved_tensors
        mod, dtype = ctx.mod, ctx.dtype
        B, H, W, Cin, Cout = ctx.dims
        dev = x_t.device
        Cinp, Coutp = pad32(Cin), pad32(Cout)
        g = drec.detach()
        if g.dtype != torch.float32 or not g.is_contiguous():
            g = g.float().contiguous()
        dzb = torch.empty((B, H, W, Coutp), dtype=dtype, device=dev)
        P = B * H * W
        with _span("recon_sigmoid_bwd", 0.0, P * (8.0 * Cout + Coutp * _es(dtype))):
            _lib.call("segk_recon_sigmoid_bwd", g.data_ptr(), rec.data_ptr(), dzb.data_ptr(), B, H, W, Cout, Coutp,
                      _DT[dtype], _stream())
        pd = dzb.data_ptr()
        px = act_info(x_t, dtype)[0]
        dx = dw = db = None
        if ctx.needs_input_grad[1]:
            wd = mod.cache.get(("c3d", dtype), w, lambda: pack_conv(w, Cin, 0, dtype, 1))
            dxb = torch.empty((B, H, W, Cinp), dtype=dtype, device=dev)
            conv3x3(dzb, pd, Coutp, 0, 0, wd, dxb.data_ptr(), Cinp, 0, 0, B, H, W, dtype, alg=(Cout, Cin))
            dx = act_view(dxb, Cin)
        if ctx.needs_input_grad[2]:
            slabs, S = wgrad(pd, Coutp, px, Cinp, 0, 0, B, H, W, 0, dtype, dev, alg=(Cout, Cin))
            dw = wgrad_to_param(slabs, S, w.shape, Cout, Cin, 0, 9, dev, param=w)
        if ctx.has_bias and ctx.needs_input_grad[3]:
            db = channel_sum(pd, P, Cout, dtype, dev)
        return None, dx, dw, db


def _mse_operand(t, what):
    _require_cuda(t, what)
    t = t.detach()
    if t.dtype != torch.float32 or not t.is_contiguous():
        t = t.float().contiguous()
    return t


class MSELossFn(torch.autograd.Function):

    @staticmethod
    def forward(ctx, input, target, mean):
        if input.shape != target.shape:
            raise ValueError(f"MSELoss: input {tuple(input.shape)} and target {tuple(target.shape)} differ in shape")
        a, b = _mse_operand(input, "MSELoss input"), _mse_operand(target, "MSELoss target")
        n = a.numel()
        if n == 0:
            raise ValueError("MSELoss of empty tensors")
        dev = a.device
        part, out = _f32(_lib.MSE_PART_FLOATS, dev), _f32(1, dev)
        with _span("mse_fwd", 0.0, 8.0 * n):
            _lib.call("segk_mse_fwd", a.data_ptr(), b.data_ptr(), part.data_ptr(), part.numel(), out.data_ptr(), n, int(mean),
                      _stream())
        ctx.mean = int(mean)
        ctx.save_for_backward(a, b)
        return out.view(())

    @staticmethod
    def backward(ctx, gout):
        a, b = ctx.saved_tensors
        go = gout.detach().float().reshape(1).contiguous()
        da = torch.empty_like(a)
        db = torch.empty_like(b) if ctx.needs_input_grad[1] else None
        n = a.numel()
        with _span("mse_bwd", 0.0, (12.0 if db is None else 16.0) * n):
            _lib.call("segk_mse_bwd", a.data_ptr(), b.data_ptr(), go.data_ptr(), da.data_ptr(), _p(db), n, ctx.mean,
                      _stream())
        return da, db, None


class BilinearFn(torch.autograd.Function):

    @staticmethod
    def forward(ctx, x, size, dtype):
        _require_cuda(x, "bilinear resize")
        x_t, px, Cp = _raw(x, dtype)
        B, C, IH, IW = x.shape
        OH, OW = int(size[0]), int(size[1])
        y = torch.empty((B, OH, OW, Cp), dtype=dtype, device=x.device)
        with _span("bilinear_fwd", 0.0, B * (IH * IW + OH * OW) * C * _es(dtype)):
            _lib.call("segk_bilinear_fwd", px, y.data_ptr(), B, IH, IW, OH, OW, Cp, _DT[dtype], _stream())
        ctx.cfg = (B, C, IH, IW, OH, OW, Cp, dtype)
        return act_view(y, C)

    @staticmethod
    def backward(ctx, dy):
        B, C, IH, IW, OH, OW, Cp, dtype = ctx.cfg
        d_t, pd, _ = _raw(dy, dtype)
        dx = torch.empty((B, IH, IW, Cp), dtype=dtype, device=dy.device)
        with _span("bilinear_bwd", 0.0, B * (IH * IW + OH * OW) * C * _es(dtype)):
            tmp = _f32(B * OH * IW * Cp, dy.device) if OH * OW > 4 * IH * IW else None
            _lib.call("segk_bilinear_bwd", pd, dx.data_ptr(), _p(tmp), B, IH, IW, OH, OW, Cp, _DT[dtype], _stream())
        return act_view(dx, C), None, None


class HeadFn(torch.autograd.Function):

    @staticmethod
    def forward(ctx, mod, x, w, b):
        dtype = mod.compute_dtype or _compute_dtype
        _require_cuda(x, "output Conv2d")
        B, C, H, W = x.shape
        x_t, px, Cp = _raw(x, dtype)
        logits = _head_fwd(px, Cp, w, b, B, C, H, W, dtype, x.device)
        ctx.dtype, ctx.dims = dtype, (B, C, H, W)
        ctx.save_for_backward(x_t, w)
        return logits

    @staticmethod
    def backward(ctx, dlogits):
        x_t, w = ctx.saved_tensors
        dtype = ctx.dtype
        B, C, H, W = ctx.dims
        px, Cp = act_info(x_t, dtype)
        dy, dw, db, _ = _head_bwd(dlogits, px, Cp, w, B, C, H, W, dtype, x_t.device)
        return None, act_view(dy, C), dw, db


class SegLossFn(torch.autograd.Function):

    @staticmethod
    def forward(ctx, logits, target, class_weights, ignore_index, smooth, dice_weight, ce_weight):
        _require_cuda(logits, "segmentation loss")
        if logits.dim() != 4:
            raise ValueError(f"expected logits [N,C,H,W], got {tuple(logits.shape)}")
        N, C, H, W = logits.shape
        if C > _lib.MAX_CLASSES:
            raise RuntimeError(f"fused loss supports up to {_lib.MAX_CLASSES} classes, got {C}")
        lg = logits.detach()
        if lg.dtype != torch.float32 or not lg.is_contiguous():
            lg = lg.float().contiguous()
        tg = target.detach()
        if tg.dtype != torch.int64 or not tg.is_contiguous():
            tg = tg.long().contiguous()
        if tg.numel() != N * H * W:
            raise ValueError(f"target shape {tuple(target.shape)} does not match logits {tuple(logits.shape)}")
        dev = logits.device
        cw = None
        if class_weights is not None:
            cw = class_weights.detach().to(device=dev, dtype=torch.float32).contiguous()
            if cw.numel() != C:
                raise ValueError("class_weights must have one entry per class")
        ign = -1 if ignore_index is None else int(ignore_index)
        part = _f32(_lib.query("segk_loss_part_floats", N * H * W), dev)
        state = _f32(_lib.query("segk_loss_state_floats"), dev)
        out = _f32(1, dev)
        with _span("loss_fwd", 0.0, N * H * W * (4.0 * C + 8)):
            _lib.call("segk_loss_fwd", lg.data_ptr(), tg.data_ptr(), _p(cw), N, C, H * W, ign, float(smooth),
                      float(dice_weight), float(ce_weight), part.data_ptr(), state.data_ptr(), out.data_ptr(), _stream())
        ctx.cfg = (N, C, H, W, ign, float(dice_weight), float(ce_weight))
        ctx.save_for_backward(lg, tg, cw, state)
        return out.view(())

    @staticmethod
    def backward(ctx, gout):
        lg, tg, cw, state = ctx.saved_tensors
        N, C, H, W, ign, dw, cew = ctx.cfg
        go = gout.detach().float().reshape(1).contiguous()
        dl = torch.empty_like(lg)
        with _span("loss_bwd", 0.0, N * H * W * (8.0 * C + 8)):
            _lib.call("segk_loss_bwd", lg.data_ptr(), tg.data_ptr(), _p(cw), state.data_ptr(), go.data_ptr(), N, C,
                      H * W, ign, dw, cew, dl.data_ptr(), _stream())
        return dl, None, None, None, None, None, None


class ProbLossFn(torch.autograd.Function):

    @staticmethod
    def forward(ctx, probs, target, class_weights, ignore_index, smooth, dice_weight, nll_weight, nll_log, eps):
        _require_cuda(probs, "probability loss")
        if probs.dim() != 4:
            raise ValueError(f"expected probabilities [N,C,H,W], got {tuple(probs.shape)}")
        N, C, H, W = probs.shape
        if C > _lib.MAX_CLASSES:
            raise RuntimeError(f"fused loss supports up to {_lib.MAX_CLASSES} classes, got {C}")
        pr = probs.detach()
        if pr.dtype != torch.float32 or not pr.is_contiguous():
            pr = pr.float().contiguous()
        tg = target.detach()
        if tg.dtype != torch.int64 or not tg.is_contiguous():
            tg = tg.long().contiguous()
        if tg.numel() != N * H * W:
            raise ValueError(f"target shape {tuple(target.shape)} does not match probabilities {tuple(probs.shape)}")
        dev = probs.device
        cw = None
        if class_weights is not None:
            cw = class_weights.detach().to(device=dev, dtype=torch.float32).contiguous()
            if cw.numel() != C:
                raise ValueError("class_weights must have one entry per class")
        ign = -1 if ignore_index is None else int(ignore_index)
        part = _f32(_lib.query("segk_loss_part_floats", N * H * W), dev)
        state = _f32(_lib.query("segk_loss_state_floats"), dev)
        out = _f32(1, dev)
        with _span("loss_fwd", 0.0, N * H * W * (4.0 * C + 8)):
            _lib.call("segk_prob_loss_fwd", pr.data_ptr(), tg.data_ptr(), _p(cw), N, C, H * W, ign, float(smooth),
                      float(dice_weight), float(nll_weight), int(nll_log), float(eps), part.data_ptr(), state.data_ptr(),
                      out.data_ptr(), _stream())
        ctx.cfg = (N, C, H, W, ign, float(dice_weight), float(nll_weight), int(nll_log), float(eps))
        ctx.save_for_backward(pr, tg, cw, state)
        return out.view(())

    @staticmethod
    def backward(ctx, gout):
        pr, tg, cw, state = ctx.saved_tensors
        N, C, H, W, ign, dw, nw, nll_log, eps = ctx.cfg
        go = gout.detach().float().reshape(1).contiguous()
        dp = torch.empty_like(pr)
        with _span("loss_bwd", 0.0, N * H * W * (8.0 * C + 8)):
            _lib.call("segk_prob_loss_bwd", pr.data_ptr(), tg.data_ptr(), _p(cw), state.data_ptr(), go.data_ptr(), N, C,
                      H * W, ign, dw, nw, nll_log, eps, dp.data_ptr(), _stream())
        return dp, None, None, None, None, None, None, None, None


class PromptMixFn(torch.autograd.Function):

    @staticmethod
    def forward(ctx, clip_logits, mask_logit):
        _require_cuda(clip_logits, "prompt remix")
        _require_cuda(mask_logit, "prompt remix")
        N, C, H, W = clip_logits.shape
        if C != 4 or tuple(mask_logit.shape) != (N, 1, H, W):
            raise ValueError(f"prompt remix expects [N,4,H,W] CLIP logits and a [N,1,H,W] mask logit, got "
                             f"{tuple(clip_logits.shape)} and {tuple(mask_logit.shape)}")
        if clip_logits.requires_grad:
            raise RuntimeError("prompt remix: the CLIP branch must be frozen (prompt.py:30-31); only the mask gets a gradient")
        cl = clip_logits.detach().float().contiguous()
        ml = mask_logit.detach().float().contiguous()
        out = torch.empty_like(cl)
        with _span("prompt_mix", 0.0, N * H * W * 36.0):
            _lib.call("segk_prompt_mix_fwd", cl.data_ptr(), ml.data_ptr(), out.data_ptr(), N, H * W, _stream())
        ctx.save_for_backward(cl, ml)
        return out

    @staticmethod
    def backward(ctx, dout):
        cl, ml = ctx.saved_tensors
        N, _, H, W = cl.shape
        d = dout.detach().float().contiguous()
        dm = torch.empty_like(ml)
        with _span("prompt_mix", 0.0, N * H * W * 40.0):
            _lib.call("segk_prompt_mix_bwd", cl.data_ptr(), ml.data_ptr(), d.data_ptr(), dm.data_ptr(), N, H * W, _stream())
        return None, dm


def confusion_matrix(logits, labels, num_classes, out=None):
    _require_cuda(logits, "confusion_matrix")
    if logits.dim() == 3:
        logits = logits.unsqueeze(0)
    N, C, H, W = logits.shape
    if C != num_classes or C > _lib.MAX_CLASSES:
        raise ValueError(f"expected {num_classes} (<= {_lib.MAX_CLASSES}) class channels, got {C}")
    lg = logits.detach()
    if lg.dtype != torch.float32 or not lg.is_contiguous():
        lg = lg.float().contiguous()
    tg = labels.detach()
    if tg.dtype != torch.int64 or not tg.is_contiguous():
        tg = tg.long().contiguous()
    if tg.numel() != N * H * W:
        raise ValueError("label shape does not match logits")
    M = out if out is not None else torch.zeros((_lib.MAX_CLASSES, _lib.MAX_CLASSES), dtype=torch.int64, device=logits.device)
    _lib.call("segk_confusion", lg.data_ptr(), tg.data_ptr(), N, C, H * W, M.data_ptr(), _stream())
    return M[:C, :C]
```

### include/segk.h

```cpp
#ifndef SEGK_H
#define SEGK_H
#include <stddef.h>
#include <stdint.h>
#ifdef __cplusplus
extern "C" {
#endif

#define SEGK_F32 0
#define SEGK_BF16 1
#define SEGK_MAX_CLASSES 8

typedef void* segk_stream_t;

#define SEGK_ABI_VERSION 312
#define SEGK_ENTRY_COUNT 75
int segk_version(void);
int segk_entry_count(void);
const char* segk_build_id(void);
const char* segk_last_error(void);

int segk_nchw_to_nhwc(const float* src, void* dst, int B, int C, int H, int W, int Cp, int dtype, segk_stream_t s);
int segk_nhwc_to_nchw(const void* src, float* dst, int B, int C, int H, int W, int Cp, int dtype, segk_stream_t s);

int segk_pack_conv_weight(const float* w, void* dst, int Cout, int CA, int CB, int Coutp, int CAp, int CBp,
                          int taps, int mode, int dtype, segk_stream_t s);
int segk_pack_conv3x3_both(const float* w, void* dst_fwd, void* dst_dgrad, int Cout, int CA, int CB, int Coutp, int CAp,
                           int CBp, int dtype, segk_stream_t s);
int segk_pack_multi(const void* table, int n, int total_blocks, int dtype, segk_stream_t s);
int segk_pack_convt_chunk(void);
int segk_pack_convt_weight(const float* w, void* dst, int Cin, int Cout, int Cinp, int Coutp, int mode, int dtype,
                           segk_stream_t s);

int segk_conv_writes_act_q(int Cin, int Cout, int dtype);
int segk_conv3x3_act(const void* srcA, const void* wpacked, const float* scale, const float* shift, void* out,
                     void* act_out, float* stats, int B, int H, int W, int CA, int CO, int dtype, segk_stream_t s);

int segk_stem3x3_rows(int B, int H, int W, int Cin, int Cout, int dtype);
int segk_stem3x3(const float* x_nchw, const float* w_oihw, void* z, void* x_nhwc, float* stats, int B, int H, int W, int Cin,
                 int Cout, int dtype, segk_stream_t s);
int segk_stem3x3_wgrad_slabs(int B, int H, int W, int Cin, int Cout, int dtype);
int segk_stem3x3_wgrad(const float* x_nchw, const void* dz, float* slabs, int B, int H, int W, int Cin, int Cout, int dtype,
                       segk_stream_t s);
int segk_conv_tiles(int B, int H, int W, int Cin, int Cout, int dtype);
int segk_bn_stats_floats(int tiles, int Cp);
int segk_conv3x3(const void* srcA, const void* srcB, const void* wpacked, const float* bias, const float* scale,
                 const float* shift, void* out, void* out2, float* stats, int B, int H, int W, int CA, int CB,
                 int CO1, int CO2, int dtype, segk_stream_t s);
int segk_conv1x1(const void* srcA, const void* wpacked, const float* bias, void* out, int B, int H, int W, int CA,
                 int CO, int dtype, segk_stream_t s);
int segk_convt2x2_fwd(const void* in, const void* wpacked, const float* bias4, void* out, int B, int H, int W,
                      int Cin, int Cout, int dtype, segk_stream_t s);
int segk_convt2x2_dgrad(const void* dout, const void* wpacked, void* din, int B, int H, int W, int Cin, int Cout,
                        int dtype, segk_stream_t s);

int segk_wgrad_tiles(int B, int H, int W, int geo, int dtype);
int segk_wgrad_split(int tiles, int CD, int CA, int CB, int geo, int dtype);
int segk_wgrad(const void* dz, const void* srcA, const void* srcB, const float* scale, const float* shift,
               float* slabs, const void* zeros64, int S, int B, int H, int W, int CD, int CA, int CB, int geo,
               int dtype, segk_stream_t s);
int segk_wgrad_reduce(const float* slabs, int S, float* grad, int N, int CA, int CB, int Np, int CAp, int CBp,
                      int taps, segk_stream_t s);
typedef struct segk_reduce_job {
  const float* src;
  float* dst;
  int kind, S, N, CA, CB, Np, CAp, CBp, taps, pad_;
} segk_reduce_job;
int segk_wgrad_reduce_multi(const segk_reduce_job* jobs, int n, segk_stream_t s);

int segk_bn_finalize(const float* stats, int tiles, int Cp, int C, double count, const float* conv_bias,
                     const float* gamma, const float* beta, float* running_mean, float* running_var, float momentum,
                     float eps, int training, float* scale, float* shift, float* mean, float* rstd, segk_stream_t s);
int segk_bn_relu_apply(const void* z, void* y, const float* scale, const float* shift, long P, int Cp, int dtype,
                       segk_stream_t s);
int segk_bn_relu_apply_pool(const void* z, void* y, void* pooled, const float* scale, const float* shift, int B, int H, int W,
                            int Cp, int dtype, segk_stream_t s);
int segk_bn_bwd_blocks(long P, int Cp, int dtype);
int segk_bn_relu_bwd(const void* dy, const void* z, void* dz, const float* scale, const float* shift,
                     const float* mean, const float* rstd, long P, int Cp, int C, float* part, float* dgamma,
                     float* dbeta, float* coef, int dtype, segk_stream_t s);

int segk_channel_sum(const void* x, long P, int Cp, int C, float* part, float* out, int dtype, segk_stream_t s);

int segk_maxpool2x2_fwd(const void* x, void* y, int B, int H, int W, int Cp, int dtype, segk_stream_t s);
int segk_maxpool2x2_bwd(const void* x, const void* dy, void* dx, int B, int H, int W, int Cp, int accumulate,
                        int dtype, segk_stream_t s);

int segk_maxpool_bwd_stat_blocks(int B, int H, int W, int Cp, int dtype);
int segk_maxpool2x2_bwd_bnstat(const void* x, const void* dy, void* dx, int B, int H, int W, int Cp, int accumulate,
                               const float* scale, const float* shift, const float* mean, const float* rstd, float* part,
                               const void* z, int dtype, segk_stream_t s);
int segk_bn_relu_bwd_from_part(const void* dy, const void* z, void* dz, const float* scale, const float* shift,
                               const float* mean, const float* rstd, long P, int Cp, int C, const float* part, int nb,
                               float* dgamma, float* dbeta, float* coef, int dtype, segk_stream_t s);

int segk_bilinear_fwd(const void* x, void* y, int B, int IH, int IW, int OH, int OW, int Cp, int dtype,
                      segk_stream_t s);
int segk_bilinear_bwd(const void* dy, void* dx, float* scratch, int B, int IH, int IW, int OH, int OW, int Cp, int dtype,
                      segk_stream_t s);

int segk_linear(const void* rows, const void* wpacked, const float* bias, void* out, long M, int K, int N, int act,
                int dtype, segk_stream_t s);
int segk_vit_patchify(const float* x, void* rows, int B, int C, int H, int W, int ps, int Kp, int dtype, segk_stream_t s);
int segk_vit_embed_ln(const void* proj, const float* cls, const float* pos, const float* gamma, const float* beta,
                      float eps, float* h, int B, int T, int D, int Dp, int dtype, segk_stream_t s);
int segk_add_layernorm(float* h, const void* delta, const float* gamma, const float* beta, float eps, void* out, long M,
                       int D, int Dp, int dtype, segk_stream_t s);
int segk_linear_splitk(const void* rows, const void* wpacked, const float* bias, void* out_parts, long M, int K, int N,
                       int ksplit, int dtype, segk_stream_t s);
int segk_add_layernorm_parts(float* h, const void* delta, int nparts, long part_stride, const float* gamma,
                             const float* beta, float eps, void* out, long M, int D, int Dp, int dtype, segk_stream_t s);
int segk_attention(const void* qkv, void* ctx, int B, int T, int heads, int head_dim, int ldq, int ldo, float scale,
                   int dtype, segk_stream_t s);
int segk_vit_tokens_to_grid(const float* h, void* out, int B, int T, int D, int Dp, int dtype, segk_stream_t s);

int segk_resize_pad(const void* img, void* out, int C, int H, int W, int nh, int nw, int T, int pad_top, int pad_left,
                    int mode, int elem, segk_stream_t s);
int segk_crop_resize(const float* slot, float* out, int C, int T, int pad_top, int pad_left, int nh, int nw, int oh,
                     int ow, int mode, segk_stream_t s);
int segk_resize_pad_u8(const uint8_t* img_hwc, float* out, int Cin, int H, int W, int nh, int nw, int T, int pad_top,
                       int pad_left, int mode, segk_stream_t s);
int segk_predict_mask(const float* slot, uint8_t* mask, uint8_t* color, const uint8_t* palette, uint64_t* counts,
                      const int64_t* labels, uint64_t* M, int C, int T, int pad_top, int pad_left, int nh, int nw, int oh,
                      int ow, int mode, segk_stream_t s);

int segk_head_fwd(const void* y, const float* w, const float* bias, float* logits, int B, int H, int W, int Cp,
                  int C, int ncls, int dtype, segk_stream_t s);
int segk_head_part_floats(long P, int Cp);
int segk_head_bwd(const float* dlogits, const void* y, const float* w, void* dy, float* part, float* dw, float* db,
                  int B, int H, int W, int Cp, int C, int ncls, int dtype, segk_stream_t s);

int segk_head_bwd_blocks(long P);
int segk_head_bwd_bnstat(const float* dlogits, const void* y, const float* w, void* dy, float* part, float* dw, float* db,
                         int B, int H, int W, int Cp, int C, int ncls, const float* scale, const float* shift,
                         const float* mean, const float* rstd, float* bnpart, int dtype, segk_stream_t s);

int segk_head_fwd_bn(const void* z, const float* scale, const float* shift, const float* w, const float* bias, float* logits,
                     int B, int H, int W, int Cp, int C, int ncls, int dtype, segk_stream_t s);
int segk_head_bwd_bn(const float* dlogits, const void* z, const float* w, void* dy, float* part, float* dw, float* db,
                     int B, int H, int W, int Cp, int C, int ncls, const float* scale, const float* shift,
                     const float* mean, const float* rstd, float* bnpart, int dtype, segk_stream_t s);

int segk_loss_part_floats(long P);
int segk_loss_state_floats(void);
int segk_loss_fwd(const float* logits, const int64_t* labels, const float* class_weights, int N, int C, long HW,
                  int ignore_index, float smooth, float dice_weight, float ce_weight, float* part, float* state,
                  float* loss_out, segk_stream_t s);
int segk_loss_bwd(const float* logits, const int64_t* labels, const float* class_weights, const float* state,
                  const float* grad_out, int N, int C, long HW, int ignore_index, float dice_weight, float ce_weight,
                  float* dlogits, segk_stream_t s);

int segk_prompt_mix_fwd(const float* clip_logits, const float* mask_logit, float* final_probs, int N, long HW,
                        segk_stream_t s);
int segk_prompt_mix_bwd(const float* clip_logits, const float* mask_logit, const float* dfinal, float* dmask_logit, int N,
                        long HW, segk_stream_t s);
int segk_prob_loss_fwd(const float* probs, const int64_t* labels, const float* class_weights, int N, int C, long HW,
                       int ignore_index, float smooth, float dice_weight, float nll_weight, int nll_log, float eps,
                       float* part, float* state, float* loss_out, segk_stream_t s);
int segk_prob_loss_bwd(const float* probs, const int64_t* labels, const float* class_weights, const float* state,
                       const float* grad_out, int N, int C, long HW, int ignore_index, float dice_weight,
                       float nll_weight, int nll_log, float eps, float* dprobs, segk_stream_t s);

int segk_recon_head_fwd(const void* x, const float* w, const float* bias, float* rec, int B, int H, int W, int Cp, int Cin,
                        int Cout, int dtype, segk_stream_t s);
int segk_recon_sigmoid_bwd(const float* drec, const float* rec, void* dz, int B, int H, int W, int C, int Cp, int dtype,
                           segk_stream_t s);
#define SEGK_MSE_PART_FLOATS 1024
int segk_mse_fwd(const float* a, const float* b, float* part, int part_floats, float* out, long n, int mean, segk_stream_t s);
int segk_mse_bwd(const float* a, const float* b, const float* grad_out, float* da, float* db, long n, int mean,
                 segk_stream_t s);

int segk_clock_probe(uint64_t* out, int blocks, int iters, int shape, segk_stream_t s);
int segk_debug_poison_tickets(uint64_t pattern, segk_stream_t s);

int segk_confusion(const float* logits, const int64_t* labels, int N, int C, long HW, uint64_t* M, segk_stream_t s);

#ifdef __cplusplus
}
#endif
#endif
```

Before: 2699 images/sec.

## Fuse stem BN-ReLU backward apply into stem weight-gradient kernel

For the first (stem) conv, when no input gradient is needed, the BN-ReLU backward is split: only the statistics/finalize kernels run, and the per-element dz computation is folded into the stem wgrad kernel, which reads dy and z and applies the BN backward formula using per-channel constants staged in LDS. This removes a full read-modify-write pass over the 256x256x64 activation gradient. The wgrad kernel now loads twice as much input per block and does extra ALU work. The generic bn apply kernel's multi-flight loop is also replaced with a reversed single-step loop.

```diff
diff --git a/image_segmentation_amd/_lib.py b/image_segmentation_amd/_lib.py
--- a/image_segmentation_amd/_lib.py
+++ b/image_segmentation_amd/_lib.py
@@ -5,7 +5,7 @@
 LIB_PATH = os.path.join(_HERE, "csrc", "libsegk.so")
 
 F32, BF16 = 0, 1
-ABI_VERSION = 312
+ABI_VERSION = 313
 MAX_CLASSES = 8
 MSE_PART_FLOATS = 1024
 
@@ -34,6 +34,7 @@
     "segk_stem3x3": (_i, [_fp, _fp, _vp, _vp, _fp, _i, _i, _i, _i, _i, _i, _vp]),
     "segk_stem3x3_wgrad_slabs": (_i, [_i, _i, _i, _i, _i, _i]),
     "segk_stem3x3_wgrad": (_i, [_fp, _vp, _fp, _i, _i, _i, _i, _i, _i, _vp]),
+    "segk_stem3x3_wgrad_bn": (_i, [_fp, _vp, _vp, _fp, _fp, _fp, _fp, _fp, _fp, _i, _i, _i, _i, _i, _i, _vp]),
     "segk_conv1x1": (_i, [_vp, _vp, _fp, _vp, _i, _i, _i, _i, _i, _i, _vp]),
     "segk_convt2x2_fwd": (_i, [_vp, _vp, _fp, _vp, _i, _i, _i, _i, _i, _i, _vp]),
     "segk_convt2x2_dgrad": (_i, [_vp, _vp, _vp, _i, _i, _i, _i, _i, _i, _vp]),
@@ -47,6 +48,7 @@
     "segk_bn_relu_apply_pool": (_i, [_vp, _vp, _vp, _fp, _fp, _i, _i, _i, _i, _i, _vp]),
     "segk_bn_bwd_blocks": (_i, [_l, _i, _i]),
     "segk_bn_relu_bwd": (_i, [_vp, _vp, _vp, _fp, _fp, _fp, _fp, _l, _i, _i, _fp, _fp, _fp, _fp, _i, _vp]),
+    "segk_bn_relu_bwd_stats": (_i, [_vp, _vp, _fp, _fp, _fp, _fp, _l, _i, _i, _fp, _fp, _fp, _fp, _i, _vp]),
     "segk_channel_sum": (_i, [_vp, _l, _i, _i, _fp, _fp, _i, _vp]),
     "segk_maxpool2x2_fwd": (_i, [_vp, _vp, _i, _i, _i, _i, _i, _vp]),
     "segk_maxpool2x2_bwd": (_i, [_vp, _vp, _vp, _i, _i, _i, _i, _i, _i, _vp]),
diff --git a/image_segmentation_amd/csrc/api.hip b/image_segmentation_amd/csrc/api.hip
--- a/image_segmentation_amd/csrc/api.hip
+++ b/image_segmentation_amd/csrc/api.hip
@@ -10,6 +10,8 @@
 int segk_bn_relu_apply_pool_impl(const void*, void*, void*, const float*, const float*, int, int, int, int, int, hipStream_t);
 int segk_bn_bwd_impl(const void*, const void*, void*, const float*, const float*, const float*, const float*, long, int,
                      int, float*, float*, float*, float*, int, hipStream_t);
+int segk_bn_bwd_stats_impl(const void*, const void*, const float*, const float*, const float*, const float*, long, int, int,
+                           float*, float*, float*, float*, int, hipStream_t);
 int segk_channel_sum_impl(const void*, long, int, int, float*, float*, int, hipStream_t);
 int segk_maxpool_fwd_impl(const void*, void*, int, int, int, int, int, hipStream_t);
 int segk_maxpool_bwd_impl(const void*, const void*, void*, int, int, int, int, int, int, hipStream_t);
@@ -141,6 +143,12 @@
   SEGK_REQUIRE(dtype == SEGK_DT_BF16, "stem3x3_wgrad: bf16 only (dtype %d)", dtype);
   return segk_stem_wgrad_launch(x_nchw, dz, slabs, B, H, W, Cin, Cout, (hipStream_t)s);
 }
+int segk_stem3x3_wgrad_bn(const float* x_nchw, const void* g, const void* z, const float* scale, const float* shift,
+                          const float* mean, const float* rstd, const float* coef, float* slabs, int B, int H, int W, int Cin,
+                          int Cout, int dtype, segk_stream_t s) {
+  SEGK_REQUIRE(dtype == SEGK_DT_BF16, "stem3x3_wgrad_bn: bf16 only (dtype %d)", dtype);
+  return segk_stem_wgrad_bn_launch(x_nchw, g, z, scale, shift, mean, rstd, coef, slabs, B, H, W, Cin, Cout, (hipStream_t)s);
+}
 int segk_stem3x3(const float* x_nchw, const float* w_oihw, void* z, void* x_nhwc, float* stats, int B, int H, int W, int Cin,
                  int Cout, int dtype, segk_stream_t s) {
   SEGK_REQUIRE(dtype == SEGK_DT_BF16, "stem3x3: bf16 only (dtype %d)", dtype);
@@ -259,6 +267,12 @@
   return segk_bn_bwd_impl(dy, z, dz, scale, shift, mean, rstd, P, Cp, C, part, dgamma, dbeta, coef, dtype,
                           (hipStream_t)s);
 }
+int segk_bn_relu_bwd_stats(const void* dy, const void* z, const float* scale, const float* shift, const float* mean,
+                           const float* rstd, long P, int Cp, int C, float* part, float* dgamma, float* dbeta, float* coef,
+                           int dtype, segk_stream_t s) {
+  SEGK_REQUIRE(dtype == SEGK_DT_F32 || dtype == SEGK_DT_BF16, "bn_relu_bwd_stats: bad dtype %d", dtype);
+  return segk_bn_bwd_stats_impl(dy, z, scale, shift, mean, rstd, P, Cp, C, part, dgamma, dbeta, coef, dtype, (hipStream_t)s);
+}
 int segk_channel_sum(const void* x, long P, int Cp, int C, float* part, float* out, int dtype, segk_stream_t s) {
   SEGK_REQUIRE(dtype == SEGK_DT_F32 || dtype == SEGK_DT_BF16, "channel_sum: bad dtype %d", dtype);
   return segk_channel_sum_impl(x, P, Cp, C, part, out, dtype, (hipStream_t)s);
diff --git a/image_segmentation_amd/csrc/bn_pool.hip b/image_segmentation_amd/csrc/bn_pool.hip
--- a/image_segmentation_amd/csrc/bn_pool.hip
+++ b/image_segmentation_amd/csrc/bn_pool.hip
@@ -322,33 +322,14 @@
     unpack16<T>(rz, fz);
     unpack16<T>(rd, fd);
 #pragma unroll
-    for (int j = 0; j < E::VEC; ++j) {
-      const float g = (fmaf(fz[j], sc[j], sh[j]) > 0.f) ? fd[j] : 0.f;
-      const float xh = (fz[j] - mu[j]) * rs[j];
-      fd[j] = sc[j] * (g - c1[j] - xh * c2[j]);
-    }
+    for (int j = 0; j < E::VEC; ++j) fd[j] = bn_relu_bwd_dz(fz[j], fd[j], sc[j], sh[j], mu[j], rs[j], c1[j], c2[j]);
     *(uint4*)(dz + off) = pack16<T>(fd);
   };
-#ifndef SEGK_BN_APPLY_FLIGHT
-#define SEGK_BN_APPLY_FLIGHT 1
-#endif
-  constexpr int APF = SEGK_BN_APPLY_FLIGHT;
   const long step = (long)gridDim.x * rows;
   const size_t cofs = (size_t)l.cv * E::VEC;
-  long p = (long)blockIdx.x * rows + l.ry;
-  for (; p + (APF - 1) * step < P; p += APF * step) {
-    size_t o[APF];
-    uint4 rz[APF], rd[APF];
-#pragma unroll
-    for (int u = 0; u < APF; ++u) {
-      o[u] = (size_t)(p + u * step) * C + cofs;
-      rz[u] = *(const uint4*)(z + o[u]);
-      rd[u] = *(const uint4*)(dy + o[u]);
-    }
-#pragma unroll
-    for (int u = 0; u < APF; ++u) one(rz[u], rd[u], o[u]);
-  }
-  for (; p < P; p += step) {
+  const long p0 = (long)blockIdx.x * rows + l.ry;
+  if (p0 >= P) return;
+  for (long p = p0 + (P - 1 - p0) / step * step; p >= p0; p -= step) {
     const size_t o0 = (size_t)p * C + cofs;
     one(*(const uint4*)(z + o0), *(const uint4*)(dy + o0), o0);
   }
@@ -715,9 +696,9 @@
 }
 
 template <typename T>
-static int bn_bwd_t(const void* dy, const void* z, void* dz, const float* scale, const float* shift, const float* mean,
-                    const float* rstd, long P, int C, int C_real, float* part, float* dgamma, float* dbeta,
-                    float* coef, hipStream_t st) {
+static int bn_bwd_stats_t(const void* dy, const void* z, const float* scale, const float* shift, const float* mean,
+                          const float* rstd, long P, int C, int C_real, float* part, float* dgamma, float* dbeta,
+                          float* coef, hipStream_t st) {
   using E = ET<T>;
   int cvb, rows, gy;
   lane_geometry(C, E::VEC, &cvb, &rows, &gy);
@@ -729,6 +710,17 @@
   hipLaunchKernelGGL(bn_bwd_finalize_kernel, dim3(C / 32), dim3(1024), 0, st, part, gx, C, C_real, (double)P, dgamma,
                      dbeta, coef);
   SEGK_CHECK_LAUNCH("bn_bwd_finalize");
+  return 0;
+}
+template <typename T>
+static int bn_bwd_t(const void* dy, const void* z, void* dz, const float* scale, const float* shift, const float* mean,
+                    const float* rstd, long P, int C, int C_real, float* part, float* dgamma, float* dbeta,
+                    float* coef, hipStream_t st) {
+  using E = ET<T>;
+  int cvb, rows, gy;
+  lane_geometry(C, E::VEC, &cvb, &rows, &gy);
+  const int rc = bn_bwd_stats_t<T>(dy, z, scale, shift, mean, rstd, P, C, C_real, part, dgamma, dbeta, coef, st);
+  if (rc != 0) return rc;
   long ga = (P + rows - 1) / rows;
   if (ga > 4096) ga = 4096;
   hipLaunchKernelGGL(bn_bwd_apply_kernel<T>, dim3((int)ga, gy), dim3(256), 0, st, (const T*)dy, (const T*)z, (T*)dz,
@@ -773,6 +765,16 @@
   return dtype == SEGK_DT_BF16
              ? bn_bwd_t<bf16_t>(dy, z, dz, scale, shift, mean, rstd, P, C, C_real, part, dgamma, dbeta, coef, st)
              : bn_bwd_t<float>(dy, z, dz, scale, shift, mean, rstd, P, C, C_real, part, dgamma, dbeta, coef, st);
+}
+
+int segk_bn_bwd_stats_impl(const void* dy, const void* z, const float* scale, const float* shift, const float* mean,
+                           const float* rstd, long P, int C, int C_real, float* part, float* dgamma, float* dbeta, float* coef,
+                           int dtype, hipStream_t st) {
+  SEGK_REQUIRE(dy && z && scale && shift && mean && rstd && part && dgamma && dbeta && coef, "bn_bwd_stats: null pointer");
+  SEGK_REQUIRE(P > 0 && C > 0 && C % 32 == 0 && C_real > 0 && C_real <= C, "bn_bwd_stats: bad shape");
+  return dtype == SEGK_DT_BF16
+             ? bn_bwd_stats_t<bf16_t>(dy, z, scale, shift, mean, rstd, P, C, C_real, part, dgamma, dbeta, coef, st)
+             : bn_bwd_stats_t<float>(dy, z, scale, shift, mean, rstd, P, C, C_real, part, dgamma, dbeta, coef, st);
 }
 
 int segk_maxpool_fwd_impl(const void* x, void* y, int B, int H, int W, int C, int dtype, hipStream_t st) {
diff --git a/image_segmentation_amd/csrc/common.hpp b/image_segmentation_amd/csrc/common.hpp
--- a/image_segmentation_amd/csrc/common.hpp
+++ b/image_segmentation_amd/csrc/common.hpp
@@ -69,6 +69,12 @@
   return make_uint4(pack_bf16x2(f[0], f[1]), pack_bf16x2(f[2], f[3]), pack_bf16x2(f[4], f[5]),
                     pack_bf16x2(f[6], f[7]));
 }
+__device__ __forceinline__ float bn_relu_bwd_dz(float z, float dy, float sc, float sh, float mu, float rs, float c1,
+                                                float c2) {
+  const float g = (fmaf(z, sc, sh) > 0.f) ? dy : 0.f;
+  const float xh = (z - mu) * rs;
+  return sc * (g - c1 - xh * c2);
+}
 template <typename T> __device__ __forceinline__ T from_float(float f);
 template <> __device__ __forceinline__ float from_float<float>(float f) { return f; }
 template <> __device__ __forceinline__ bf16_t from_float<bf16_t>(float f) { return (bf16_t)f; }
diff --git a/image_segmentation_amd/csrc/segk_internal.h b/image_segmentation_amd/csrc/segk_internal.h
--- a/image_segmentation_amd/csrc/segk_internal.h
+++ b/image_segmentation_amd/csrc/segk_internal.h
@@ -37,6 +37,9 @@
 int segk_stem_wgrad_slabs(int B, int H, int W, int Cin, int Cout, int dtype);
 int segk_stem_wgrad_launch(const float* x, const void* dz, float* slabs, int B, int H, int W, int Cin, int Cout,
                            hipStream_t st);
+int segk_stem_wgrad_bn_launch(const float* x, const void* g, const void* z, const float* scale, const float* shift,
+                              const float* mean, const float* rstd, const float* coef, float* slabs, int B, int H, int W,
+                              int Cin, int Cout, hipStream_t st);
 int segk_convt_stream_ok(int B, int H, int W, int Cin, int Cout, int dtype);
 int segk_convt_stream_launch(const void* x, const void* wp, const float* bias4, void* out, int B, int H, int W, int Cin,
                              int Cout, hipStream_t st);
diff --git a/image_segmentation_amd/csrc/stem.hip b/image_segmentation_amd/csrc/stem.hip
--- a/image_segmentation_amd/csrc/stem.hip
+++ b/image_segmentation_amd/csrc/stem.hip
@@ -152,10 +152,17 @@
 
 struct __attribute__((packed, aligned(4))) F4U { float v[4]; };
 
+struct StemBn {
+  const bf16_t* z;
+  const float *scale, *shift, *mean, *rstd, *coef;
+};
+
+template <bool BN>
 __global__ __launch_bounds__(STEM_WAVES * 64, 2) void stem_wgrad_kernel(const float* __restrict__ x, const bf16_t* __restrict__ dz,
-                                                                        float* __restrict__ slabs, int B, int H, int W, int Cin,
-                                                                        long nblk) {
-  __shared__ __attribute__((aligned(16))) char lds[4 * 64 * 32 * 4];
+                                                                        const StemBn bn, float* __restrict__ slabs, int B,
+                                                                        int H, int W, int Cin, long nblk) {
+  constexpr int RED_BYTES = 4 * 64 * 32 * 4, TAB_BYTES = BN ? 8 * 6 * 8 * 4 : 0;
+  __shared__ __attribute__((aligned(16))) char lds[RED_BYTES + TAB_BYTES];
   typedef __attribute__((address_space(3))) s16x4* lds_v4;
   const int lane = threadIdx.x & 63;
   const int wave = __builtin_amdgcn_readfirstlane(threadIdx.x >> 6);
@@ -170,6 +177,16 @@
   const int g = lane >> 4, i16 = lane & 15, q = i16 >> 2, p = i16 & 3;
   const int coff = (16 * (g & 1) + 4 * p) * 2, xa = 8 * (g >> 1) + q;
   const int lp = lane >> 2, lc4 = lane & 3;
+  const int px = lane >> 3, pc = lane & 7;
+  const float4* const tab = (const float4*)(lds + RED_BYTES) + pc * 12;
+  if constexpr (BN) {
+    for (int i = threadIdx.x; i < 6 * 64; i += STEM_WAVES * 64) {
+      const int k = i >> 6, c = i & 63;
+      const float v = k == 0 ? bn.scale[c] : k == 1 ? bn.shift[c] : k == 2 ? bn.mean[c] : k == 3 ? bn.rstd[c] : bn.coef[2 * c + (k - 4)];
+      ((float*)(lds + RED_BYTES))[(c >> 3) * 48 + k * 8 + (c & 7)] = v;
+    }
+    __syncthreads();
+  }
 
   f32x16 acc[2];
 #pragma unroll
@@ -184,8 +201,15 @@
     const int x0 = (int)(blk - row * W16) * 16;
     const long b = row / H;
     const int y = (int)(row - b * H);
-    const bf16_t* dp = dz + ((size_t)row * W + x0 + lp) * 64 + lc4 * 8;
-    const uint4 d0 = *(const uint4*)dp, d1 = *(const uint4*)(dp + 32);
+    uint4 d0, d1, z0, z1;
+    if constexpr (BN) {
+      const size_t e0 = ((size_t)row * W + x0 + px) * 64 + pc * 8;
+      d0 = *(const uint4*)(dz + e0); d1 = *(const uint4*)(dz + e0 + 8 * 64);
+      z0 = *(const uint4*)(bn.z + e0); z1 = *(const uint4*)(bn.z + e0 + 8 * 64);
+    } else {
+      const bf16_t* dp = dz + ((size_t)row * W + x0 + lp) * 64 + lc4 * 8;
+      d0 = *(const uint4*)dp; d1 = *(const uint4*)(dp + 32);
+    }
     float v[8];
     const int xs = x0 + 8 * hh + dx;
     const bool rok = jok & ((unsigned)(y + dy) < (unsigned)H);
@@ -198,8 +222,29 @@
 #pragma unroll
       for (int e = 0; e < 8; ++e) v[e] = (rok && (unsigned)(xs + e) < (unsigned)W) ? src[e] : 0.f;
     }
-    *(uint4*)(slot + lp * 64 + lc4 * 16) = d0;
-    *(uint4*)(slot + 1024 + lp * 64 + lc4 * 16) = d1;
+    if constexpr (BN) {
+      float fg0[8], fg1[8], fz0[8], fz1[8];
+      unpack16<bf16_t>(d0, fg0); unpack16<bf16_t>(d1, fg1);
+      unpack16<bf16_t>(z0, fz0); unpack16<bf16_t>(z1, fz1);
+#pragma unroll
+      for (int h = 0; h < 2; ++h) {
+        const float4 k0 = tab[h], k1 = tab[2 + h], k2 = tab[4 + h], k3 = tab[6 + h], k4 = tab[8 + h], k5 = tab[10 + h];
+        const float sc[4] = {k0.x, k0.y, k0.z, k0.w}, sh[4] = {k1.x, k1.y, k1.z, k1.w}, mu[4] = {k2.x, k2.y, k2.z, k2.w};
+        const float rs[4] = {k3.x, k3.y, k3.z, k3.w}, c1[4] = {k4.x, k4.y, k4.z, k4.w}, c2[4] = {k5.x, k5.y, k5.z, k5.w};
+#pragma unroll
+        for (int e = 0; e < 4; ++e) {
+          const int c = 4 * h + e;
+          fg0[c] = bn_relu_bwd_dz(fz0[c], fg0[c], sc[e], sh[e], mu[e], rs[e], c1[e], c2[e]);
+          fg1[c] = bn_relu_bwd_dz(fz1[c], fg1[c], sc[e], sh[e], mu[e], rs[e], c1[e], c2[e]);
+        }
+      }
+      char* const dst = slot + (pc >> 2) * 1024 + px * 64 + (pc & 3) * 16;
+      *(uint4*)dst = pack16<bf16_t>(fg0);
+      *(uint4*)(dst + 8 * 64) = pack16<bf16_t>(fg1);
+    } else {
+      *(uint4*)(slot + lp * 64 + lc4 * 16) = d0;
+      *(uint4*)(slot + 1024 + lp * 64 + lc4 * 16) = d1;
+    }
     const u32x4 fbv = {pk_bf16(v[0], v[1]), pk_bf16(v[2], v[3]), pk_bf16(v[4], v[5]), pk_bf16(v[6], v[7])};
     const bf16x8 fb = __builtin_bit_cast(bf16x8, fbv);
     __builtin_amdgcn_fence(__ATOMIC_RELEASE, "wavefront");
@@ -274,8 +319,23 @@
   const int g = segk_stem_wgrad_slabs(B, H, W, Cin, Cout, SEGK_DT_BF16);
   SEGK_REQUIRE(g > 0, "stem_wgrad: shape not served (bf16, 1..3 input channels, 64 output channels, W a multiple of 16)");
   const long nblk = (long)B * H * (W / 16);
-  hipLaunchKernelGGL(stem_wgrad_kernel, dim3(g), dim3(STEM_WAVES * 64), 0, st, x, (const bf16_t*)dz, slabs, B, H, W, Cin, nblk);
+  hipLaunchKernelGGL(stem_wgrad_kernel<false>, dim3(g), dim3(STEM_WAVES * 64), 0, st, x, (const bf16_t*)dz, StemBn{}, slabs, B, H,
+                     W, Cin, nblk);
   SEGK_CHECK_LAUNCH("stem_wgrad");
+  return 0;
+}
+
+int segk_stem_wgrad_bn_launch(const float* x, const void* g, const void* z, const float* scale, const float* shift,
+                              const float* mean, const float* rstd, const float* coef, float* slabs, int B, int H, int W,
+                              int Cin, int Cout, hipStream_t st) {
+  SEGK_REQUIRE(x && g && z && scale && shift && mean && rstd && coef && slabs, "stem_wgrad_bn: null pointer");
+  const int nwg = segk_stem_wgrad_slabs(B, H, W, Cin, Cout, SEGK_DT_BF16);
+  SEGK_REQUIRE(nwg > 0, "stem_wgrad_bn: shape not served (bf16, 1..3 input channels, 64 output channels, W a multiple of 16)");
+  const long nblk = (long)B * H * (W / 16);
+  const StemBn bn{(const bf16_t*)z, scale, shift, mean, rstd, coef};
+  hipLaunchKernelGGL(stem_wgrad_kernel<true>, dim3(nwg), dim3(STEM_WAVES * 64), 0, st, x, (const bf16_t*)g, bn, slabs, B, H, W,
+                     Cin, nblk);
+  SEGK_CHECK_LAUNCH("stem_wgrad_bn");
   return 0;
 }
 
diff --git a/image_segmentation_amd/ops.py b/image_segmentation_amd/ops.py
--- a/image_segmentation_amd/ops.py
+++ b/image_segmentation_amd/ops.py
@@ -561,6 +561,18 @@
     return dgamma, dbeta
 
 
+def bn_relu_bwd_stats(dy_ptr, z_ptr, scale, shift, mean, rstd, P, C, dtype, dev):
+    Cp = pad32(C)
+    dgamma, dbeta = _f32(C, dev), _f32(C, dev)
+    nb = _lib.query("segk_bn_bwd_blocks", P, Cp, _DT[dtype])
+    part, coef = _f32(nb * Cp * 2, dev), _f32(2 * Cp, dev)
+    with _span("bn_relu_bwd", 0.0, 2.0 * P * C * _es(dtype)):
+        _lib.call("segk_bn_relu_bwd_stats", dy_ptr, z_ptr, scale.data_ptr(), shift.data_ptr(), mean.data_ptr(),
+                  rstd.data_ptr(), P, Cp, C, part.data_ptr(), dgamma.data_ptr(), dbeta.data_ptr(), coef.data_ptr(),
+                  _DT[dtype], _stream())
+    return dgamma, dbeta, coef
+
+
 def channel_sum(ptr, P, C, dtype, dev):
     Cp = pad32(C)
     nb = _lib.query("segk_bn_bwd_blocks", P, Cp, _DT[dtype])
@@ -934,13 +946,19 @@
         rb = ReduceBatch(dev)
         del slabs, dz2
 
-        dg1, dbe1 = bn_relu_bwd(da1.data_ptr(), z1.data_ptr(), da1.data_ptr(), sc1, sh1, mu1, rs1, P, Cout, dtype, dev,
-                                frozen=frozen)
+        has_up = ctx.up_dims is not None
+        need_dx = need[1] or need[2] or has_up
+        stem_bn = bool(ctx.stem_raw and not frozen and not need_dx
+                       and _lib.query("segk_stem3x3_wgrad_slabs", B, H, W, CA, Cout, _DT[dtype]) > 0)
+        if stem_bn:
+            dg1, dbe1, coef1 = bn_relu_bwd_stats(da1.data_ptr(), z1.data_ptr(), sc1, sh1, mu1, rs1, P, Cout, dtype, dev)
+        else:
+            dg1, dbe1 = bn_relu_bwd(da1.data_ptr(), z1.data_ptr(), da1.data_ptr(), sc1, sh1, mu1, rs1, P, Cout, dtype, dev,
+                                    frozen=frozen)
         dz1 = da1
         dxa = dxb = None
         dxb_buf, chan_sum = None, None
-        has_up = ctx.up_dims is not None
-        if need[1] or need[2] or has_up:
+        if need_dx:
             w1d = mod.cache.get(("w1d", dtype), w1, lambda: pack_conv(w1, CA, CB, dtype, 1))
             dxa_buf = torch.empty((B, H, W, CAp), dtype=dtype, device=dev)
             dxb_buf = torch.empty((B, H, W, CBp), dtype=dtype, device=dev) if CB else None
@@ -957,9 +975,15 @@
         if ctx.stem_raw:
             S = _lib.query("segk_stem3x3_wgrad_slabs", B, H, W, CA, Cout, _DT[dtype])
             slabs = _f32(S * 64 * 32, dev)
-            with _span("wgrad3x3", 2.0 * P * 9 * CA * Cout, P * (Cout * _es(dtype) + 4 * CA) + 4.0 * 9 * CA * Cout):
-                _lib.call("segk_stem3x3_wgrad", xa_t.data_ptr(), dz1.data_ptr(), slabs.data_ptr(), B, H, W, CA, Cout,
-                          _DT[dtype], _stream())
+            if stem_bn:
+                with _span("wgrad3x3", 2.0 * P * 9 * CA * Cout, P * (2 * Cout * _es(dtype) + 4 * CA) + 4.0 * 9 * CA * Cout):
+                    _lib.call("segk_stem3x3_wgrad_bn", xa_t.data_ptr(), da1.data_ptr(), z1.data_ptr(), sc1.data_ptr(),
+                              sh1.data_ptr(), mu1.data_ptr(), rs1.data_ptr(), coef1.data_ptr(), slabs.data_ptr(), B, H, W,
+                              CA, Cout, _DT[dtype], _stream())
+            else:
+                with _span("wgrad3x3", 2.0 * P * 9 * CA * Cout, P * (Cout * _es(dtype) + 4 * CA) + 4.0 * 9 * CA * Cout):
+                    _lib.call("segk_stem3x3_wgrad", xa_t.data_ptr(), dz1.data_ptr(), slabs.data_ptr(), B, H, W, CA, Cout,
+                              _DT[dtype], _stream())
             dw1 = wgrad_to_param(slabs, S, w1.shape, Cout, 9 * CA, 0, 1, dev, param=w1)
         else:
             slabs, S = wgrad(dz1.data_ptr(), Coutp, pA, CAp, pB, CBp, B, H, W, 0, dtype, dev, alg=(Cout, CA + CB))
diff --git a/include/segk.h b/include/segk.h
--- a/include/segk.h
+++ b/include/segk.h
@@ -12,8 +12,8 @@
 
 typedef void* segk_stream_t;
 
-#define SEGK_ABI_VERSION 312
-#define SEGK_ENTRY_COUNT 75
+#define SEGK_ABI_VERSION 313
+#define SEGK_ENTRY_COUNT 77
 int segk_version(void);
 int segk_entry_count(void);
 const char* segk_build_id(void);
@@ -41,6 +41,9 @@
 int segk_stem3x3_wgrad_slabs(int B, int H, int W, int Cin, int Cout, int dtype);
 int segk_stem3x3_wgrad(const float* x_nchw, const void* dz, float* slabs, int B, int H, int W, int Cin, int Cout, int dtype,
                        segk_stream_t s);
+int segk_stem3x3_wgrad_bn(const float* x_nchw, const void* g, const void* z, const float* scale, const float* shift,
+                          const float* mean, const float* rstd, const float* coef, float* slabs, int B, int H, int W, int Cin,
+                          int Cout, int dtype, segk_stream_t s);
 int segk_conv_tiles(int B, int H, int W, int Cin, int Cout, int dtype);
 int segk_bn_stats_floats(int tiles, int Cp);
 int segk_conv3x3(const void* srcA, const void* srcB, const void* wpacked, const float* bias, const float* scale,
@@ -78,6 +81,9 @@
 int segk_bn_relu_bwd(const void* dy, const void* z, void* dz, const float* scale, const float* shift,
                      const float* mean, const float* rstd, long P, int Cp, int C, float* part, float* dgamma,
                      float* dbeta, float* coef, int dtype, segk_stream_t s);
+int segk_bn_relu_bwd_stats(const void* dy, const void* z, const float* scale, const float* shift, const float* mean,
+                           const float* rstd, long P, int Cp, int C, float* part, float* dgamma, float* dbeta, float* coef,
+                           int dtype, segk_stream_t s);
 
 int segk_channel_sum(const void* x, long P, int Cp, int C, float* part, float* out, int dtype, segk_stream_t s);
 
```

Result: no change. 2717 images/sec (median of 6 runs) (+0.7%).
